# lez-s/Materialist

Measured on AMD Instinct MI355X. Metric: opt_iterations_per_sec_512x512, higher is better.
Workload: dtype f32; 1 GPU; BASELINE configs[1] synthetic: 1x512x512/GPU, --model_name pos_mlp --opt_order 'rm a' part rm, spp 64; mode=pos_mlp, height=512, width=512, spp=64, images_per_gpu=1, light=SH25, parallelism=dp1 (independent images, no data-path collective)

## Files before the change

include/matpbr.h:

```cpp
#ifndef MATPBR_H
#define MATPBR_H

#include <stddef.h>
#include <stdint.h>

#ifdef __cplusplus
extern "C" {
#endif

#define MATPBR_VERSION 311
#define MATPBR_MAX_SPP 128
#define MATPBR_NSH 25

enum {
    MATPBR_OK = 0,
    MATPBR_ERR_INVALID_ARG = -1,
    MATPBR_ERR_UNSUPPORTED = -2,
    MATPBR_ERR_LAUNCH = -3,
    MATPBR_ERR_WORKSPACE = -4,
};

enum { MATPBR_LIGHT_SH25 = 0, MATPBR_LIGHT_SH9 = 1, MATPBR_LIGHT_ENV_TEXELS = 2 };

#define MATPBR_FLAG_CLAMP_PARAMS 1u
// ... 13 lines not shown

typedef struct MatpbrCamera {
    float fov_x_deg;
} MatpbrCamera;

int matpbr_version(void);
const char* matpbr_strerror(int code);

int matpbr_shade_fwd(const float* a, const float* r, const float* m, const float* n, const float* light,
                     int light_kind, int n_light, float* out_rgb, int H, int W, int batch, int spp,
                     const MatpbrCamera* cam, uint32_t flags, void* stream);
size_t matpbr_plane9_bytes(int H, int W, int batch);
int matpbr_shade_fwd_ex(const float* a, const float* r, const float* m, const float* n, const float* light, int light_kind,
                        int n_light, const float* dcache, float* out_rgb, float* jac, int H, int W, int batch, int spp,
                        const MatpbrCamera* cam, uint32_t flags, void* stream);
int matpbr_diffuse_cache(const float* n, const float* light, int light_kind, int n_light, float* dcache, int H, int W, int batch,
                         int spp, const MatpbrCamera* cam, void* stream);
int matpbr_shade_fwd_keep(const float* a, const float* r, const float* m, const float* n, const float* light, int light_kind,
                          int n_light, const float* dcache, float* out_rgb, float* jac, float* s1, int H, int W, int batch, int spp,
                          const MatpbrCamera* cam, uint32_t flags, void* stream);
int matpbr_shade_fwd_cached(const float* a, const float* m, const float* jac, const float* s1, float* out_rgb, int H, int W, int batch,
                            uint32_t flags, void* stream);

size_t matpbr_lazy_state_bytes(int H, int W, int batch);
size_t matpbr_lazy_fold_bytes(int H, int W, int batch);
int matpbr_lazy_sums_count(int H, int W);
int matpbr_shade_fwd_lazy(const float* a, const float* r, const float* m, const float* n, const float* light, int light_kind, int n_light,
                          const float* dcache, void* lazy_state, float* out_rgb, void* jac16, const float* stats, float* sums, int H, int W,
                          int batch, int spp, const MatpbrCamera* cam, uint32_t flags, float floor, float tol, void* stream);
int matpbr_lazy_state_unpack(const void* lazy_state, float* state28, int* refreshed, int H, int W, int batch, void* stream);
int matpbr_jac16_unpack(const void* jac16, float* jac, int H, int W, int batch, void* stream);

int matpbr_shade_bwd(const float* a, const float* r, const float* m, const float* n, const float* light,
                     int light_kind, int n_light, const float* d_out_rgb, float* d_a, float* d_r, float* d_m,
                     float* d_n, float* d_light, void* workspace, size_t workspace_bytes, int H, int W, int batch,
                     int spp, const MatpbrCamera* cam, uint32_t flags, void* stream);
size_t matpbr_shade_bwd_workspace_bytes(int H, int W, int batch, int n_light);
int matpbr_shade_bwd_jac(const float* a, const float* r, const float* m, const float* jac, const float* d_out_rgb, float* d_a,
                         float* d_r, float* d_m, int H, int W, int batch, void* stream);

size_t matpbr_brdf_loss_workspace_bytes(int batch);
int matpbr_brdf_loss_stats(const float* pred, const float* gt, const float* gt_srgb, const float* pa, const float* pr,
                           const float* pm, const float* a0, const float* r0, const float* m0, float scale_delta,
                           float* stats, void* workspace, size_t workspace_bytes, int H, int W, int batch, uint32_t flags,
                           void* stream);
int matpbr_brdf_loss_stats_es(const float* pred, const float* gt, const float* gt_srgb, const float* pa, const float* pr, const float* pm,
                              const float* a0, const float* r0, const float* m0, float scale_delta, float* stats, void* workspace,
                              size_t workspace_bytes, int H, int W, int batch, uint32_t flags, int es_patience, float es_min_delta, float* history,
                              int hist_len, void* stream);
int matpbr_brdf_loss_bwd_jac(const float* pa, const float* pr, const float* pm, const float* jac, const float* pred,
                             const float* gt_srgb, const float* stats, const float* a0, const float* r0, const float* m0,
                             float scale_delta, float* d_a, float* d_r, float* d_m, float* best_a, float* best_r, float* best_m,
                             float* best_img, int H, int W, int batch, uint32_t flags, void* stream);
int matpbr_adam_step(float* p, const float* g, float* m, float* v, long n, float lr, float beta1, float beta2, float eps,
                     int step, void* stream);

typedef struct MatpbrBrdfPhase {
    float *pa, *pr, *pm;
    const float *n, *light;
    const float *gt_srgb;
    const float *a0, *r0, *m0;
    const float* dcache;
    float* pred;
    float* jac;
    float *d_a, *d_r, *d_m;
    float *adam_m[3], *adam_v[3];
    float *best_a, *best_r, *best_m, *best_img;
    float* stats;
    float* history;
    void* workspace;
    size_t workspace_bytes;
    int H, W, batch, spp;
    float fov_x_deg, scale_delta;
    uint32_t part_mask;
    int es_patience;
    float es_min_delta;
    int hist_len;
    float* s1cache;
    void* lazy_state;
    float lazy_tol;
    float* pred_next;
    uint32_t flags;
    void* lazy_fold;
} MatpbrBrdfPhase;
typedef struct MatpbrNormalStep {
    float *pa, *pr, *pm, *pn;
    float *ca, *cr, *cm, *cn;
    const float *d_a, *d_r, *d_m, *d_n;
    const float *a0, *r0, *m0, *n0;
    float *adam_m[4], *adam_v[4];
    float *best_a, *best_r, *best_m, *best_n, *best_img;
    const float *pred, *stats;
    float* ln_part;
    int H, W, batch;
    uint32_t part_mask;
    float scale_delta;
} MatpbrNormalStep;
int matpbr_brdf_loss_dpred(const float* pred, const float* gt_srgb, const float* stats, float* d_pred, int H, int W, int batch, void* stream);
int matpbr_brdf_normal_step(const MatpbrNormalStep* step, int t, float lr, void* stream);

size_t matpbr_brdf_phase_workspace_bytes(int H, int W, int batch);
int matpbr_brdf_phase_step(const MatpbrBrdfPhase* phase, int t, float lr, void* stream);
int matpbr_brdf_phase_resolve(const MatpbrBrdfPhase* phase, int t_done, void* stream);
#define MATPBR_STAGE_RENDER 1u
#define MATPBR_STAGE_STATS 2u
#define MATPBR_STAGE_BACKWARD 4u
// ... 53 lines not shown
```

include/matpbr_mlp.h:

```cpp
#ifndef MATPBR_MLP_H
#define MATPBR_MLP_H
#include <stddef.h>
#include <stdint.h>

#ifdef __cplusplus
extern "C" {
#endif

int matpbr_mlp_small_bwd_step(const float* g, int ldg, const float* w, int ldw, const float* c_prev, float* g_prev, int ldo, float* colsum_out,
                              int n_prev, const float* x, int ldx, float* d_w, int ldw_out, int K, const float* colsum_in, int colsum_stride,
                              int groups_in, float* d_bias, long M, int n_red, void* stream);

int matpbr_sin_bwd(const float* d_y, long ld_d, const float* pre, long ld_p, float* out, long M, int n, void* stream);
size_t matpbr_column_sum_workspace_bytes(int N);
int matpbr_column_sum(const float* x, float* out, long M, int N, void* workspace, size_t workspace_bytes, void* stream);

int matpbr_mlp_layer_fwd(const float* x, int ldx, const float* w, int ldw, const float* bias, float* s_out, float* c_out, int ldo, long M,
                         int N, int K, void* stream);
size_t matpbr_mlp_bwd_input_workspace_bytes(long M);
int matpbr_mlp_layer_bwd_input(const float* g, int ldg, const float* wt, int ldwt, const float* c_prev, float* g_prev, int ldo,
                               float* d_bias_prev, void* workspace, size_t workspace_bytes, long M, int n_prev, int n_red, void* stream);
size_t matpbr_mlp_bwd_weight_workspace_bytes(long M);
int matpbr_mlp_layer_bwd_weight(const float* g, int ldg, const float* x, int ldx, float* d_w, int ldw, void* workspace,
                                size_t workspace_bytes, long M, int N, int K, void* stream);
// ... 24 lines not shown
                                      int nprod, void* stream);
int matpbr_mlp_layer_bwd_weight_bx(const float* g, int ldg, const float* x, int ldx, float* d_w, int ldw, void* workspace,
                                   size_t workspace_bytes, long M, int N, int K, int nprod, void* stream);

#define MATPBR_WSPLIT_TRANSPOSED 1
#define MATPBR_WSPLIT_F16X2 2
int matpbr_mlp_split_weights_fmt(const float* w, int ldw, int N, int K, int flags, void* wsplit, void* stream);
size_t matpbr_mlp_chain_images_bytes(void);
int matpbr_mlp_chain_prep(const float* const* w, const int* ldw, const int* n, const float* const* bias, int d0, void* images, void* const* bwd_images,
                          void* zero, long zero_words, void* stream);
int matpbr_mlp_chain_fwd(const float* x0, int ldx0, const void* images, float* const* s_out, int ldo, const int* n, const float* start, int lds, float* th,
                         float* map_a, float* map_r, float* map_m, int n_head, long M, void* stream);
#define MATPBR_REDUCE_NONE (-1)
#define MATPBR_REDUCE_WGRAD 0
#define MATPBR_REDUCE_COLSUM 1
#define MATPBR_REDUCE_SKINNY 2
typedef struct MatpbrReduceJob {
    int kind, groups;
    const float *src, *src_b, *src_g;
    float *dst, *dst_b, *dst_g;
    int n0, n1, n2, n3;
    long ld_j, ld_c;
} MatpbrReduceJob;
int matpbr_mlp_reduce_jobs(const MatpbrReduceJob* jobs, int n_jobs, void* stream);
int matpbr_mlp_out_layer_bwd_tmax(const float* d_x, int ldd, const float* s_prev, const float* c_prev, int lds, const float* w_out, int ldw, float* g_prev,
                                  int ldg, void* g_tile_max, float* d_w, long ld_j, long ld_c, float* d_bias, float* d_bias_prev, void* workspace,
                                  size_t workspace_bytes, long M, int J, int n_prev, MatpbrReduceJob* defer, void* stream);
int matpbr_mlp_layer_bwd_input_blk(const float* g, int ldg, const void* g_tile_max, const void* wtsplit, const float* s_prev, float* g_prev, int ldo,
                                   void* out_tile_max, float* d_bias_prev, void* workspace, size_t workspace_bytes, long M, int n_prev, int n_red,
                                   MatpbrReduceJob* defer, void* stream);
int matpbr_mlp_first_layer_bwd_blk(const float* g, int ldg, const void* g_tile_max, const void* wtsplit, const float* s_prev, int lds, const float* x0,
                                   int ldx0, float* d_w0, long ld_j, long ld_c, int d0, float* d_bias0, void* workspace, size_t workspace_bytes,
                                   void* workspace2, size_t workspace2_bytes, long M, int n0, int n_red, MatpbrReduceJob* defer2, void* stream);
int matpbr_mlp_layer_bwd_weight_blk(const float* g, int ldg, const void* g_tile_max, const float* x, int ldx, float* d_w, int ldw, void* workspace,
                                    size_t workspace_bytes, long M, int N, int K, MatpbrReduceJob* defer, void* stream);
int matpbr_mlp_set_wgrad_kernel(int kernel);
int matpbr_mlp_split_weights_multi(const float* const* w, const int* ldw, const int* N, const int* K, const int* transposed,
                                   void* const* wsplit, int n_jobs, void* stream);
int matpbr_mlp_skinny_fwd(const float* x, int ldx, const float* w, int ldw, const float* bias, float* out, int ldo, long M, int J, int K,
                          void* stream);
int matpbr_mlp_arm_head_fwd(const float* x, int ldx, const float* w, int ldw, const float* bias, const float* start, int lds, float* th,
                            float* map_a, float* map_r, float* map_m, long M, int K, void* stream);
int matpbr_mlp_arm_head_bwd(const float* g_a, const float* g_r, const float* g_m, const float* th, float* d_x, long M, void* stream);
size_t matpbr_mlp_skinny_workspace_bytes(int J);
int matpbr_mlp_out_layer_bwd(const float* d_x, int ldd, const float* s_prev, const float* c_prev, int lds, const float* w_out, int ldw, float* g_prev,
                             int ldg, float* d_w, long ld_j, long ld_c, float* d_bias, float* d_bias_prev, void* workspace, size_t workspace_bytes,
                             long M, int J, int n_prev, void* stream);
int matpbr_mlp_skinny_bwd_weight(const float* s, int lds, const float* b, int ldb, float* d_w, long ld_j, long ld_c, float* d_bias,
                                 void* workspace, size_t workspace_bytes, long M, int J, int C, void* stream);
int matpbr_adamw_step_dev(float* p, const float* g, float* m, float* v, long n, float* hyper, float beta1, float beta2, float eps,
                          float weight_decay, void* stream);
int matpbr_adamw_step_snapshot_dev(float* p, const float* g, float* m, float* v, long n, float* hyper, float beta1, float beta2,
                                   float eps, float weight_decay, float* best, const float* stats, void* stream);

#ifdef __cplusplus
}
#endif
#endif
```

materialist_amd/_lib.py:

```python
from __future__ import annotations

import ctypes
import os
import threading

from . import build as _build

_c_f = ctypes.c_void_p


class MatpbrCamera(ctypes.Structure):
    _fields_ = [("fov_x_deg", ctypes.c_float)]


class MatpbrBrdfPhase(ctypes.Structure):
    _fields_ = ([(k, ctypes.c_void_p) for k in ("pa", "pr", "pm", "n", "light", "gt_srgb", "a0", "r0", "m0", "dcache", "pred", "jac", "d_a",
                                                "d_r", "d_m")] +
                [("adam_m", ctypes.c_void_p * 3), ("adam_v", ctypes.c_void_p * 3)] +
                [(k, ctypes.c_void_p) for k in ("best_a", "best_r", "best_m", "best_img", "stats", "history", "workspace")] +
                [("workspace_bytes", ctypes.c_size_t), ("H", ctypes.c_int), ("W", ctypes.c_int), ("batch", ctypes.c_int), ("spp", ctypes.c_int),
                 ("fov_x_deg", ctypes.c_float), ("scale_delta", ctypes.c_float), ("part_mask", ctypes.c_uint32), ("es_patience", ctypes.c_int),
                 ("es_min_delta", ctypes.c_float), ("hist_len", ctypes.c_int), ("s1cache", ctypes.c_void_p), ("lazy_state", ctypes.c_void_p),
                 ("lazy_tol", ctypes.c_float), ("pred_next", ctypes.c_void_p), ("flags", ctypes.c_uint32), ("lazy_fold", ctypes.c_void_p)])

# ... 6 lines not shown


class MatpbrError(RuntimeError):
    pass


class ReduceJob(ctypes.Structure):
    _fields_ = [("kind", ctypes.c_int), ("groups", ctypes.c_int), ("src", ctypes.c_void_p), ("src_b", ctypes.c_void_p), ("src_g", ctypes.c_void_p),
                ("dst", ctypes.c_void_p), ("dst_b", ctypes.c_void_p), ("dst_g", ctypes.c_void_p), ("n0", ctypes.c_int), ("n1", ctypes.c_int),
                ("n2", ctypes.c_int), ("n3", ctypes.c_int), ("ld_j", ctypes.c_long), ("ld_c", ctypes.c_long)]


SIGNATURES = {
    "matpbr_version": (ctypes.c_int, []),
    "matpbr_strerror": (ctypes.c_char_p, [ctypes.c_int]),
    "matpbr_shade_fwd": (ctypes.c_int, [_c_f] * 5 + [ctypes.c_int, ctypes.c_int, _c_f, ctypes.c_int, ctypes.c_int, ctypes.c_int,
                                       ctypes.c_int, ctypes.POINTER(MatpbrCamera), ctypes.c_uint32, ctypes.c_void_p]),
    "matpbr_shade_bwd": (ctypes.c_int, [_c_f] * 5 + [ctypes.c_int, ctypes.c_int] + [_c_f] * 6 + [ctypes.c_void_p, ctypes.c_size_t,
                                       ctypes.c_int, ctypes.c_int, ctypes.c_int, ctypes.c_int, ctypes.POINTER(MatpbrCamera),
                                       ctypes.c_uint32, ctypes.c_void_p]),
    "matpbr_shade_bwd_workspace_bytes": (ctypes.c_size_t, [ctypes.c_int] * 4),
    "matpbr_plane9_bytes": (ctypes.c_size_t, [ctypes.c_int] * 3),
    "matpbr_shade_fwd_ex": (ctypes.c_int, [_c_f] * 5 + [ctypes.c_int, ctypes.c_int, _c_f, _c_f, _c_f, ctypes.c_int, ctypes.c_int, ctypes.c_int,
                                          ctypes.c_int, ctypes.POINTER(MatpbrCamera), ctypes.c_uint32, ctypes.c_void_p]),
    "matpbr_shade_fwd_keep": (ctypes.c_int, [_c_f] * 5 + [ctypes.c_int, ctypes.c_int, _c_f, _c_f, _c_f, _c_f, ctypes.c_int, ctypes.c_int, ctypes.c_int,
                                            ctypes.c_int, ctypes.POINTER(MatpbrCamera), ctypes.c_uint32, ctypes.c_void_p]),
    "matpbr_shade_fwd_cached": (ctypes.c_int, [_c_f] * 5 + [ctypes.c_int, ctypes.c_int, ctypes.c_int, ctypes.c_uint32, ctypes.c_void_p]),
    "matpbr_diffuse_cache": (ctypes.c_int, [_c_f, _c_f, ctypes.c_int, ctypes.c_int, _c_f, ctypes.c_int, ctypes.c_int, ctypes.c_int, ctypes.c_int,
                                           ctypes.POINTER(MatpbrCamera), ctypes.c_void_p]),
    "matpbr_lazy_state_bytes": (ctypes.c_size_t, [ctypes.c_int] * 3),
    "matpbr_lazy_fold_bytes": (ctypes.c_size_t, [ctypes.c_int] * 3),
    "matpbr_env_texel_phase_step": (ctypes.c_int, [_c_f] * 6 + [ctypes.c_int, ctypes.c_int, ctypes.c_float, ctypes.c_void_p, ctypes.c_size_t, ctypes.c_int,
                                                   ctypes.c_int, _c_f, ctypes.c_int] + [_c_f] * 8 + [ctypes.c_float] * 3 + [ctypes.c_int, ctypes.c_int,
                                                                                                                          ctypes.c_void_p]),
    "matpbr_brdf_loss_dpred": (ctypes.c_int, [_c_f] * 4 + [ctypes.c_int, ctypes.c_int, ctypes.c_int, ctypes.c_void_p]),
    "matpbr_brdf_normal_step": (ctypes.c_int, [ctypes.POINTER(MatpbrNormalStep), ctypes.c_int, ctypes.c_float, ctypes.c_void_p]),
    "matpbr_env_mlp_phase_step": (ctypes.c_int, [_c_f] * 7 + [ctypes.c_int, ctypes.c_int, ctypes.c_float, ctypes.c_void_p, ctypes.c_size_t, ctypes.c_int,
                                                 ctypes.c_int, _c_f, ctypes.c_int] + [_c_f] * 4 + [ctypes.c_int, ctypes.c_int, ctypes.c_void_p]),
    "matpbr_brdf_phase_stages_timed": (ctypes.c_int, [ctypes.POINTER(MatpbrBrdfPhase), ctypes.c_int, ctypes.c_float, ctypes.c_uint32, ctypes.c_void_p,
                                                      ctypes.c_void_p, ctypes.c_void_p]),
    "matpbr_lazy_sums_count": (ctypes.c_int, [ctypes.c_int] * 2),
    "matpbr_shade_fwd_lazy": (ctypes.c_int, [_c_f] * 5 + [ctypes.c_int, ctypes.c_int] + [_c_f] * 6 + [ctypes.c_int, ctypes.c_int, ctypes.c_int, ctypes.c_int,
                                            ctypes.POINTER(MatpbrCamera), ctypes.c_uint32, ctypes.c_float, ctypes.c_float, ctypes.c_void_p]),
    "matpbr_lazy_state_unpack": (ctypes.c_int, [_c_f, _c_f, _c_f, ctypes.c_int, ctypes.c_int, ctypes.c_int, ctypes.c_void_p]),
    "matpbr_jac16_unpack": (ctypes.c_int, [_c_f, _c_f, ctypes.c_int, ctypes.c_int, ctypes.c_int, ctypes.c_void_p]),
    "matpbr_shade_bwd_jac": (ctypes.c_int, [_c_f] * 8 + [ctypes.c_int, ctypes.c_int, ctypes.c_int, ctypes.c_void_p]),
    "matpbr_brdf_loss_workspace_bytes": (ctypes.c_size_t, [ctypes.c_int]),
    "matpbr_brdf_loss_stats": (ctypes.c_int, [_c_f] * 9 + [ctypes.c_float, _c_f, ctypes.c_void_p, ctypes.c_size_t, ctypes.c_int, ctypes.c_int,
                                             ctypes.c_int, ctypes.c_uint32, ctypes.c_void_p]),
    "matpbr_brdf_loss_stats_es": (ctypes.c_int, [_c_f] * 9 + [ctypes.c_float, _c_f, ctypes.c_void_p, ctypes.c_size_t, ctypes.c_int, ctypes.c_int,
                                                ctypes.c_int, ctypes.c_uint32, ctypes.c_int, ctypes.c_float, _c_f, ctypes.c_int, ctypes.c_void_p]),
    "matpbr_brdf_loss_bwd_jac": (ctypes.c_int, [_c_f] * 10 + [ctypes.c_float] + [_c_f] * 7 + [ctypes.c_int, ctypes.c_int, ctypes.c_int,
                                                                                              ctypes.c_uint32, ctypes.c_void_p]),
    "matpbr_brdf_phase_workspace_bytes": (ctypes.c_size_t, [ctypes.c_int] * 3),
    "matpbr_brdf_phase_step": (ctypes.c_int, [ctypes.POINTER(MatpbrBrdfPhase), ctypes.c_int, ctypes.c_float, ctypes.c_void_p]),
    "matpbr_brdf_phase_stages": (ctypes.c_int, [ctypes.POINTER(MatpbrBrdfPhase), ctypes.c_int, ctypes.c_float, ctypes.c_uint32, ctypes.c_void_p]),
    "matpbr_brdf_phase_resolve": (ctypes.c_int, [ctypes.POINTER(MatpbrBrdfPhase), ctypes.c_int, ctypes.c_void_p]),
    "matpbr_env_phase_workspace_bytes": (ctypes.c_size_t, [ctypes.c_int] * 3),
    "matpbr_env_phase_step": (ctypes.c_int, [_c_f] * 7 + [ctypes.c_int, ctypes.c_int, ctypes.c_float, ctypes.c_void_p, ctypes.c_size_t,
                                            ctypes.c_int, ctypes.c_int, ctypes.c_int, ctypes.c_void_p]),
    "matpbr_env_project": (ctypes.c_int, [_c_f, ctypes.c_int, _c_f, _c_f, _c_f, ctypes.c_int, ctypes.c_void_p]),
    "matpbr_env_project_bwd": (ctypes.c_int, [_c_f, ctypes.c_int, _c_f, _c_f, _c_f, ctypes.c_int, ctypes.c_int, ctypes.c_void_p]),
    "matpbr_select_improved": (ctypes.c_int, [_c_f, _c_f, _c_f, ctypes.c_int, ctypes.c_long, ctypes.c_void_p]),
    "matpbr_mlp_wsplit_bytes": (ctypes.c_size_t, [ctypes.c_int]),
    "matpbr_mlp_split_weights": (ctypes.c_int, [_c_f, ctypes.c_int, ctypes.c_int, ctypes.c_int, _c_f, ctypes.c_void_p]),
    "matpbr_mlp_layer_fwd_bx": (ctypes.c_int, [_c_f, ctypes.c_int, _c_f, _c_f, _c_f, _c_f, ctypes.c_int, ctypes.c_long, ctypes.c_int, ctypes.c_int,
                                              ctypes.c_int, ctypes.c_void_p]),
    "matpbr_mlp_layer_bwd_input_bx": (ctypes.c_int, [_c_f, ctypes.c_int, _c_f, _c_f, _c_f, ctypes.c_int, _c_f, ctypes.c_void_p, ctypes.c_size_t,
                                                    ctypes.c_long, ctypes.c_int, ctypes.c_int, ctypes.c_int, ctypes.c_void_p]),
    "matpbr_sin_bwd": (ctypes.c_int, [_c_f, ctypes.c_long, _c_f, ctypes.c_long, _c_f, ctypes.c_long, ctypes.c_int, ctypes.c_void_p]),
    "matpbr_mlp_layer_fwd": (ctypes.c_int, [_c_f, ctypes.c_int, _c_f, ctypes.c_int, _c_f, _c_f, _c_f, ctypes.c_int, ctypes.c_long, ctypes.c_int,
                                           ctypes.c_int, ctypes.c_void_p]),
    "matpbr_mlp_bwd_input_workspace_bytes": (ctypes.c_size_t, [ctypes.c_long]),
    "matpbr_mlp_layer_bwd_input": (ctypes.c_int, [_c_f, ctypes.c_int, _c_f, ctypes.c_int, _c_f, _c_f, ctypes.c_int, _c_f, ctypes.c_void_p,
                                                 ctypes.c_size_t, ctypes.c_long, ctypes.c_int, ctypes.c_int, ctypes.c_void_p]),
    "matpbr_mlp_bwd_weight_workspace_bytes": (ctypes.c_size_t, [ctypes.c_long]),
    "matpbr_mlp_layer_bwd_weight": (ctypes.c_int, [_c_f, ctypes.c_int, _c_f, ctypes.c_int, _c_f, ctypes.c_int, ctypes.c_void_p, ctypes.c_size_t,
                                                  ctypes.c_long, ctypes.c_int, ctypes.c_int, ctypes.c_void_p]),
    "matpbr_mlp_layer_fwd_sgn": (ctypes.c_int, [_c_f, ctypes.c_int, _c_f, ctypes.c_int, _c_f, _c_f, ctypes.c_int, _c_f, ctypes.c_int, ctypes.c_long,
                                               ctypes.c_int, ctypes.c_int, ctypes.c_void_p]),
    "matpbr_mlp_layer_bwd_input_sgn": (ctypes.c_int, [_c_f, ctypes.c_int, _c_f, ctypes.c_int, _c_f, _c_f, ctypes.c_int, _c_f, ctypes.c_void_p,
                                                     ctypes.c_size_t, ctypes.c_long, ctypes.c_int, ctypes.c_int, ctypes.c_void_p]),
    "matpbr_mlp_layer_bwd_input_bx_sgn": (ctypes.c_int, [_c_f, ctypes.c_int, _c_f, _c_f, _c_f, ctypes.c_int, _c_f, ctypes.c_void_p, ctypes.c_size_t,
                                                        ctypes.c_long, ctypes.c_int, ctypes.c_int, ctypes.c_int, ctypes.c_void_p]),
    "matpbr_mlp_layer_bwd_weight_bx": (ctypes.c_int, [_c_f, ctypes.c_int, _c_f, ctypes.c_int, _c_f, ctypes.c_int, ctypes.c_void_p, ctypes.c_size_t,
                                                     ctypes.c_long, ctypes.c_int, ctypes.c_int, ctypes.c_int, ctypes.c_void_p]),
    "matpbr_mlp_out_layer_bwd_tmax": (ctypes.c_int, [_c_f, ctypes.c_int, _c_f, _c_f, ctypes.c_int, _c_f, ctypes.c_int, _c_f, ctypes.c_int, ctypes.c_void_p, _c_f,
                                                     ctypes.c_long, ctypes.c_long, _c_f, _c_f, ctypes.c_void_p, ctypes.c_size_t, ctypes.c_long, ctypes.c_int,
                                                     ctypes.c_int, ctypes.c_void_p, ctypes.c_void_p]),
    "matpbr_mlp_reduce_jobs": (ctypes.c_int, [ctypes.c_void_p, ctypes.c_int, ctypes.c_void_p]),
    "matpbr_mlp_layer_bwd_input_blk": (ctypes.c_int, [_c_f, ctypes.c_int, ctypes.c_void_p, ctypes.c_void_p, _c_f, _c_f, ctypes.c_int, ctypes.c_void_p, _c_f,
                                                      ctypes.c_void_p, ctypes.c_size_t, ctypes.c_long, ctypes.c_int, ctypes.c_int, ctypes.c_void_p, ctypes.c_void_p]),
    "matpbr_mlp_first_layer_bwd_blk": (ctypes.c_int, [_c_f, ctypes.c_int, ctypes.c_void_p, ctypes.c_void_p, _c_f, ctypes.c_int, _c_f, ctypes.c_int, _c_f,
                                                      ctypes.c_long, ctypes.c_long, ctypes.c_int, _c_f, ctypes.c_void_p, ctypes.c_size_t, ctypes.c_void_p,
                                                      ctypes.c_size_t, ctypes.c_long, ctypes.c_int, ctypes.c_int, ctypes.c_void_p, ctypes.c_void_p]),
    "matpbr_mlp_layer_bwd_weight_blk": (ctypes.c_int, [_c_f, ctypes.c_int, ctypes.c_void_p, _c_f, ctypes.c_int, _c_f, ctypes.c_int, ctypes.c_void_p,
                                                       ctypes.c_size_t, ctypes.c_long, ctypes.c_int, ctypes.c_int, ctypes.c_void_p, ctypes.c_void_p]),
    "matpbr_mlp_set_wgrad_kernel": (ctypes.c_int, [ctypes.c_int]),
    "matpbr_mlp_chain_images_bytes": (ctypes.c_size_t, []),
    "matpbr_mlp_chain_prep": (ctypes.c_int, [ctypes.c_void_p, ctypes.c_void_p, ctypes.c_void_p, ctypes.c_void_p, ctypes.c_int, ctypes.c_void_p, ctypes.c_void_p,
                                             ctypes.c_void_p, ctypes.c_long, ctypes.c_void_p]),
    "matpbr_mlp_chain_fwd": (ctypes.c_int, [_c_f, ctypes.c_int, ctypes.c_void_p, ctypes.c_void_p, ctypes.c_int, ctypes.c_void_p, _c_f, ctypes.c_int, _c_f, _c_f, _c_f,
                                            _c_f, ctypes.c_int, ctypes.c_long, ctypes.c_void_p]),
    "matpbr_mlp_split_weights_fmt": (ctypes.c_int, [_c_f, ctypes.c_int, ctypes.c_int, ctypes.c_int, ctypes.c_int, ctypes.c_void_p, ctypes.c_void_p]),
    "matpbr_mlp_skinny_fwd": (ctypes.c_int, [_c_f, ctypes.c_int, _c_f, ctypes.c_int, _c_f, _c_f, ctypes.c_int, ctypes.c_long, ctypes.c_int, ctypes.c_int,
                                            ctypes.c_void_p]),
    "matpbr_mlp_arm_head_fwd": (ctypes.c_int, [_c_f, ctypes.c_int, _c_f, ctypes.c_int, _c_f, _c_f, ctypes.c_int, _c_f, _c_f, _c_f, _c_f, ctypes.c_long,
                                              ctypes.c_int, ctypes.c_void_p]),
    "matpbr_mlp_arm_head_bwd": (ctypes.c_int, [_c_f, _c_f, _c_f, _c_f, _c_f, ctypes.c_long, ctypes.c_void_p]),
    "matpbr_mlp_skinny_workspace_bytes": (ctypes.c_size_t, [ctypes.c_int]),
    "matpbr_mlp_set_lds_dma": (ctypes.c_int, [ctypes.c_int]),
    "matpbr_mlp_skinny_bwd_weight": (ctypes.c_int, [_c_f, ctypes.c_int, _c_f, ctypes.c_int, _c_f, ctypes.c_long, ctypes.c_long, _c_f, ctypes.c_void_p,
                                                   ctypes.c_size_t, ctypes.c_long, ctypes.c_int, ctypes.c_int, ctypes.c_void_p]),
    "matpbr_adamw_step_dev": (ctypes.c_int, [_c_f] * 4 + [ctypes.c_long, _c_f, ctypes.c_float, ctypes.c_float, ctypes.c_float, ctypes.c_float,
                                                         ctypes.c_void_p]),
    "matpbr_light_to_sh25": (ctypes.c_int, [_c_f, ctypes.c_int, ctypes.c_int, _c_f, ctypes.c_int, ctypes.c_void_p]),
    "matpbr_light_to_sh25_bwd": (ctypes.c_int, [_c_f, ctypes.c_int, ctypes.c_int, _c_f, ctypes.c_int, ctypes.c_void_p]),
    "matpbr_mlp_split_weights_multi": (ctypes.c_int, [ctypes.c_void_p] * 6 + [ctypes.c_int, ctypes.c_void_p]),
    "matpbr_adamw_step_snapshot_dev": (ctypes.c_int, [_c_f] * 4 + [ctypes.c_long, _c_f, ctypes.c_float, ctypes.c_float, ctypes.c_float, ctypes.c_float,
                                                                  _c_f, _c_f, ctypes.c_void_p]),
    "matpbr_mlp_layer_fwd_tail": (ctypes.c_int, [_c_f, ctypes.c_int, _c_f, ctypes.c_int, _c_f, _c_f, _c_f, ctypes.c_int, _c_f, ctypes.c_int, ctypes.c_long,
                                                ctypes.c_int, ctypes.c_int, ctypes.c_void_p]),
    "matpbr_mlp_layer_fwd_bx_tail": (ctypes.c_int, [_c_f, ctypes.c_int, _c_f, _c_f, _c_f, _c_f, ctypes.c_int, _c_f, ctypes.c_int, ctypes.c_long,
                                                   ctypes.c_int, ctypes.c_int, ctypes.c_int, ctypes.c_void_p]),
    "matpbr_sample_brdf_dr": (ctypes.c_int, [_c_f] * 10 + [ctypes.c_long, ctypes.c_void_p]),
    "matpbr_mlp_layer_fwd_bx_head": (ctypes.c_int, [_c_f, ctypes.c_int, _c_f, _c_f, _c_f, _c_f, ctypes.c_int, _c_f, ctypes.c_int, _c_f, _c_f, ctypes.c_int,
                                                   _c_f, _c_f, _c_f, _c_f, ctypes.c_long, ctypes.c_int, ctypes.c_int, ctypes.c_void_p]),
    "matpbr_column_sum_workspace_bytes": (ctypes.c_size_t, [ctypes.c_int]),
    "matpbr_column_sum": (ctypes.c_int, [_c_f, _c_f, ctypes.c_long, ctypes.c_int, ctypes.c_void_p, ctypes.c_size_t, ctypes.c_void_p]),
    "matpbr_shade_transfer": (ctypes.c_int, [_c_f] * 5 + [ctypes.c_int, ctypes.c_int, ctypes.c_int, ctypes.c_int, ctypes.POINTER(MatpbrCamera),
                                            ctypes.c_uint32, ctypes.c_void_p]),
    "matpbr_transfer_bytes": (ctypes.c_size_t, [ctypes.c_int] * 3),
    "matpbr_relight": (ctypes.c_int, [_c_f] * 3 + [ctypes.c_int, ctypes.c_int, ctypes.c_int, ctypes.c_void_p]),
    "matpbr_adam_step": (ctypes.c_int, [_c_f] * 4 + [ctypes.c_long, ctypes.c_float, ctypes.c_float, ctypes.c_float, ctypes.c_float, ctypes.c_int,
                                       ctypes.c_void_p]),
    "matpbr_eval_brdf": (ctypes.c_int, [_c_f] * 8 + [ctypes.c_long, ctypes.c_void_p]),
    "matpbr_eval_brdf_bwd": (ctypes.c_int, [_c_f] * 11 + [ctypes.c_long, ctypes.c_void_p]),
    "matpbr_brdf_terms": (ctypes.c_int, [_c_f] * 5 + [ctypes.c_long, ctypes.c_void_p]),
    "matpbr_sample_brdf": (ctypes.c_int, [_c_f] * 10 + [ctypes.c_long, ctypes.c_void_p]),
    "matpbr_sh_eval": (ctypes.c_int, [_c_f] * 3 + [ctypes.c_long, ctypes.c_void_p]),
    "matpbr_depth_to_mesh_host": (ctypes.c_int, [ctypes.c_void_p, ctypes.c_int, ctypes.c_int, ctypes.c_float, ctypes.c_float] + [ctypes.c_void_p] * 6),
    "matpbr_mlp_small_bwd_step": (ctypes.c_int, [_c_f, ctypes.c_int, _c_f, ctypes.c_int, _c_f, _c_f, ctypes.c_int, _c_f, ctypes.c_int, _c_f, ctypes.c_int,
                                                 _c_f, ctypes.c_int, ctypes.c_int, _c_f, ctypes.c_int, ctypes.c_int, _c_f, ctypes.c_long, ctypes.c_int,
# ... 54 lines not shown
```

materialist_amd/armhead.py:

```python
from __future__ import annotations

import types
from typing import Dict, Optional

import torch

from . import _lib, ops
from . import loss as _loss
from . import render as _render
from .posmlp import _PosMlpHipFn

_al4 = lambda n: (n + 3) // 4 * 4


def flat_state(net: torch.nn.Module, dev) -> dict:
    L = net.n_layers
    lins = [(getattr(net, f"lin{l}").linear if l < L - 1 else getattr(net, f"lin{l}")) for l in range(L)]
    st = getattr(net, "_flat_state", None)
    if (st is not None and "spans" in st and st["flat"].device == torch.device(dev)
            and all(lin.weight.data_ptr() == wp.data_ptr() and lin.bias.data_ptr() == bp.data_ptr() for lin, (wp, bp) in zip(lins, st["views"]))):
        return st
    total = sum(lin.weight.shape[0] * _al4(lin.weight.shape[1]) + _al4(lin.weight.shape[0]) for lin in lins)
    flat = torch.zeros(total, dtype=torch.float32, device=dev)
    off, views, spans = 0, [], {}
    for l, lin in enumerate(lins):
        n, k = lin.weight.shape
        wp = flat[off:off + n * _al4(k)].view(n, _al4(k))
        wp[:, :k].copy_(lin.weight.detach())
        lin.weight.data = wp[:, :k]
        off += n * _al4(k)
        bp = flat[off:off + n]
        bp.copy_(lin.bias.detach())
        lin.bias.data = bp
        off += _al4(n)
        views.append((wp, bp))
    names = {id(p): name for name, p in net.named_parameters()}
    for lin, (wp, bp) in zip(lins, views):
        spans[names[id(lin.weight)]] = (wp, lin.weight.shape[1])
        spans[names[id(lin.bias)]] = (bp, None)
    st = net._flat_state = {"flat": flat, "views": views, "spans": spans}
    return st


class ArmMlpPhase:

    PACKED = True
    FUSED_OUT_BWD = True
    FUSED_FIRST_BWD = True
    BWD_F16 = True
    FWD_CHAIN = True
    DEFER_REDUCE = True
    FWD_PRODUCTS = 3

    @staticmethod
    def why_not(scene: _render.Scene, gt_image: torch.Tensor, net: torch.nn.Module, optimize_part: str, mask) -> Optional[str]:
        if gt_image.ndim != 3:
            return "a batch of images (the network optimises one image per process, as the reference does)"
        if not gt_image.is_cuda:
            return "the image is not on a GPU"
        if not scene.use_mesh_normal or "n" in optimize_part:
            return "predicted normals / a part that moves the normal map (the eight-output 'armn' network and the render under a normal map: loop.PosMlpNormalPhase with armhead.MlpEngine)"
        if getattr(net, "output_type", None) != "arm" or not _PosMlpHipFn.PRODUCTS:
            return "not the five-output 'arm' network on the split-operand kernels"
        M = gt_image.shape[0] * gt_image.shape[1]
        if M % 128 or M < _PosMlpHipFn.MIN_ROWS:
            return f"{M} pixels: the layer kernels take whole 128-row tiles of at least {_PosMlpHipFn.MIN_ROWS} rows"
        L = net.n_layers
        d0 = getattr(net, "lin0").linear.weight.shape[1]
        for l in range(L - 1):
            n = getattr(net, f"lin{l}").linear.weight.shape[0]
            if (n + d0 if (l + 1) in net.skip else n) != 256:
                return "hidden layers that are not 256 wide"
        if getattr(net, f"lin{L - 1}").weight.shape != (5, 256) or d0 > 16:
            return "an output layer that is not 256 -> 5, or more than 16 inputs"
        return None

    @staticmethod
    def supported(scene: _render.Scene, gt_image: torch.Tensor, net: torch.nn.Module, optimize_part: str, mask) -> bool:
        return ArmMlpPhase.why_not(scene, gt_image, net, optimize_part, mask) is None

    def __init__(self, scene: _render.Scene, gt_image: torch.Tensor, net: torch.nn.Module, start_arm: torch.Tensor, fixed: Dict[str, torch.Tensor],
                 optimize_part: str = "arm", spp: int = 64, lr: float = 3e-4, scale_delta: float = 0.1, patience: int = 0,
                 min_delta: float = 0.0, best_mse: Optional[torch.Tensor] = None, history_len: int = 5000, weight_decay: float = 0.01,
                 mask: Optional[torch.Tensor] = None):
        from .loop import _lib_ws

        if not ArmMlpPhase.supported(scene, gt_image, net, optimize_part, None):
            raise NotImplementedError("ArmMlpPhase: 'arm' network with 256-wide layers on one image of at least 8192 pixels (a multiple of 128)")
        self.ops, self.scene, self.net, self.part = ops, scene, net, optimize_part
        self.spp, self.scale_delta = int(spp), float(scale_delta)
        self.gt = gt_image.contiguous()
        dev = self.dev = self.gt.device
        H, W = self.H, self.W = self.gt.shape[0], self.gt.shape[1]
        M = self.M = H * W
        self.gt_srgb = _loss.linear_to_srgb(self.gt).contiguous()
        self.start_arm = start_arm.detach().to(dev, torch.float32).contiguous()
        self.fixed = {k: v.detach().contiguous() for k, v in fixed.items()}
        self.orig = {"albedo": self.start_arm[:, 0:3].reshape(H, W, 3).contiguous(),
                     "roughness": self.start_arm[:, 3:4].reshape(H, W, 1).contiguous(),
                     "metallic": self.start_arm[:, 4:5].reshape(H, W, 1).contiguous()}
        self.products = int(_PosMlpHipFn.PRODUCTS)
        self.fwd_products = int(self.FWD_PRODUCTS) or self.products
        self.bwd_f16 = bool(self.BWD_F16 and self.PACKED and self.FUSED_OUT_BWD and self.FUSED_FIRST_BWD)
        st = flat_state(net, dev)
# ... 82 lines not shown
        self.dcache = ops.diffuse_cache(self._n, self._light, self.spp, scene.fov)
        self.jac = ops.plane9(self.gt)
        self.s1 = None if "roughness" in self.live else torch.empty((3, 1, H, W), dtype=torch.float32, device=dev)
        self._bg_mask = scene.bg_mask
        if self._bg_mask is not None:
            self._bg_rgb = (scene.bg_basis @ self._light.reshape(25, 3)).contiguous()
            self._bg_idx = ops.background_index(self._bg_mask)
            self._bg_rows = self._bg_rgb.reshape(-1, 3)[self._bg_idx].contiguous()
            self._bg_rows_t = self._bg_rows.t().contiguous()
        self._mask_u8 = None if mask is None else mask.to(dev).reshape(H, W).to(torch.uint8).contiguous()
        self._fed = {k: E(H, W, 1) for k in ("roughness", "metallic")} if mask is not None else None
        self.t = 0

    def set_lr(self, lr: float) -> None:
        self._lr = float(lr)
        self.hyper[0:1].fill_(self._lr)
        self.opt.param_groups[0]["lr"] = self._lr

    def forward(self) -> Dict[str, torch.Tensor]:
        o, P = ops, self.fwd_products
        if self._split_args[-1] > 0:
            with torch.cuda.device(self.dev):
                _lib.check(_lib.load().matpbr_mlp_split_weights_multi(*self._split_args, o._stream(self.flat)), "matpbr_mlp_split_weights_multi")
        if self.chain:
            live = self.live
            lib, st = _lib.load(), o._stream(self.flat)
            mp = [o._ptr(self.maps[k]) if k in live else None for k in ("albedo", "roughness", "metallic")]
            with torch.cuda.device(self.dev):
                _lib.check(lib.matpbr_mlp_chain_prep(*self._chain_prep, st), "matpbr_mlp_chain_prep")
                _lib.check(lib.matpbr_mlp_chain_fwd(o._ptr(self.x0p), self.x0p.stride(0), o._ptr(self._chain_images), self._chain_out, 256, self._chain_n,
                                                    o._ptr(self.start_arm), self.start_arm.stride(0), o._ptr(self.th), *mp, self.views[-1][0].shape[0], self.M, st),
                           "matpbr_mlp_chain_fwd")
            return {k: (self.maps[k] if k in live else self.fixed[k]) for k in self.maps}
        wp, bp = self.views[0]
        tail = lambda l: self.x0p if self.ns[l] != 256 else None
        if self.packed:
            o.mlp_layer_fwd(self.x0p, wp, bp, self.bufs[0], None, self.d0, packed=True)
        else:
            o.mlp_layer_fwd(self.x0p, wp, bp, self.bufs[0], self.cbufs[0], self.d0)
        live = self.live
        maps = [self.maps[k] if k in live else None for k in ("albedo", "roughness", "metallic")]
        wo, bo = self.views[-1]
        for l in range(1, self.L - 1):
            wp, bp = self.views[l]
            if l == self.L - 2 and self.ns[l] == 256:
                o.mlp_layer_fwd_bx_head(self.bufs[l - 1], self.wsplit_f[l], bp, self.bufs[l], self.cbufs[l], 256, P, wo, bo, self.start_arm, self.th,
                                        *maps)
            else:
                o.mlp_layer_fwd_bx(self.bufs[l - 1], self.wsplit_f[l], bp, self.bufs[l], self.cbufs[l], self.ns[l], 256, P, tail=tail(l))
        if self.ns[-1] != 256:
            o.mlp_arm_head_fwd(self.bufs[-1], wo, bo, self.start_arm, self.th, *maps, 256)
        return {k: (self.maps[k] if k in live else self.fixed[k]) for k in self.maps}

    def backward(self) -> None:
        o, P, live = ops, self.products, self.live
        o.mlp_arm_head_bwd(self.g["albedo"] if "albedo" in live else None, self.g["roughness"] if "roughness" in live else None,
                           self.g["metallic"] if "metallic" in live else None, self.th, self.d_x)
        wp, _ = self.views[-1]
        gw, gb = self.gviews[-1]
        g_prev = self.gbufs[0]
        _, gb_prev = self.gviews[self.L - 2]
        f16 = self.bwd_f16
        import ctypes as _ct

        jobs, nj = (self._jobs, 0) if (f16 and self.DEFER_REDUCE) else (None, 0)
        slot = (lambda k: (_ct.cast(_ct.byref(jobs, k * _ct.sizeof(_lib.ReduceJob)), _ct.c_void_p), f"_d{k}")) if jobs is not None else (lambda k: None)
        if f16:
            if not self.prep_all:
                self.tmax.zero_()
            o.mlp_out_layer_bwd_tmax(self.d_x, self.bufs[-1], wp, g_prev, self.tmax[self.L - 2], gw, gb, gb_prev, 5, self.ns[-1], defer=slot(nj))
            nj += 1
        elif self.FUSED_OUT_BWD:
            o.mlp_out_layer_bwd(self.d_x, self.bufs[-1], None if self.packed else self.cbufs[-1], wp, g_prev, gw, gb, gb_prev, 5, self.ns[-1])
        else:
            o.mlp_skinny_bwd_weight(self.d_x, self.bufs[-1], gw, 5, 256, d_bias=gb)
            self.w_out_t[:, :5].copy_(wp.t())
            o.mlp_layer_bwd_input(self.d_x, self.w_out_t, self.bufs[-1] if self.packed else self.cbufs[-1], g_prev, self.ns[-1], 5, gb_prev,
                                  packed=self.packed)
        g, n_red = g_prev, self.ns[-1]
        for l in range(self.L - 2, 0, -1):
            wp, _ = self.views[l]
            gw, _ = self.gviews[l]
            if f16:
                o.mlp_layer_bwd_weight_blk(g, self.tmax[l], self.bufs[l - 1], n_red, 256, out=gw, defer=slot(nj))
                nj += 1
            else:
                o.mlp_layer_bwd_weight_bx(g, self.bufs[l - 1], n_red, 256, P, out=gw)
            n_prev = self.ns[l - 1]
            _, gb = self.gviews[l - 1]
            c_prev = self.bufs[l - 1] if self.packed else self.cbufs[l - 1]
            if f16:
                if l == 1:
                    o.mlp_first_layer_bwd_blk(g, self.tmax[l], self.wsplit_b[l], c_prev, self.x0p, self.gviews[0][0], self.d0, n_prev, n_red, gb, defer=slot(nj))
                    nj += 2
                    if jobs is not None:
                        o.mlp_reduce_jobs(jobs, nj, self.flat)
                    return
                g_prev = self.gbufs[0] if g is self.gbufs[1] else self.gbufs[1]
                o.mlp_layer_bwd_input_blk(g, self.tmax[l], self.wsplit_b[l], c_prev, g_prev, n_prev, n_red, gb, self.tmax[l - 1], defer=slot(nj))
                nj += 1
                g, n_red = g_prev, n_prev
                continue
            if l == 1 and self.FUSED_FIRST_BWD:
                o.mlp_first_layer_bwd_bx(g, self.wsplit_b[l], c_prev, self.x0p, self.gviews[0][0], self.d0, n_prev, n_red, gb, P, packed=self.packed)
                return
            g_prev = self.gbufs[0] if g is self.gbufs[1] else self.gbufs[1]
            o.mlp_layer_bwd_input_bx(g, self.wsplit_b[l], c_prev, g_prev, n_prev, n_red, gb, P, packed=self.packed)
            g, n_red = g_prev, n_prev
        gw, _ = self.gviews[0]
        o.mlp_skinny_bwd_weight(self.x0p, g, gw, self.d0, n_red, transposed_out=True)

    def step(self) -> None:
        o, sc = ops, self.scene
        d = self.forward()
        if self._mask_u8 is not None:
            d = dict(d)
            for k in ("roughness", "metallic"):
                lo, hi = (0.0, 1.0) if k in self.live else (-3.0e38, 3.0e38)
                d[k] = o.masked_mean_fill(d[k], self._mask_u8, out=self._fed[k], lo=lo, hi=hi)
        if self.s1 is not None and self.t > 0:
            o.shade_fwd_cached(d["albedo"], d["metallic"], self.jac, self.s1, clamp_params=True, out=self.pred)
        else:
            o.shade_fwd(d["albedo"], d["roughness"], d["metallic"], self._n, self._light, self.spp, sc.fov, clamp_params=True, out=self.pred,
                        dcache=self.dcache, jac=self.jac, s1=self.s1)
        if self._bg_mask is not None and not (self.s1 is not None and self.t > 0):
            self.pred.view(-1, 3).index_copy_(0, self._bg_idx, self._bg_rows)
            o.background_into_jac(self.jac, self.s1, self._bg_mask, self._bg_rgb, self._bg_idx, self._bg_rows_t)
        o.brdf_loss_stats(self.pred, self.gt, self.gt_srgb, d["albedo"], d["roughness"], d["metallic"], self.orig["albedo"],
                          self.orig["roughness"], self.orig["metallic"], self.scale_delta, self.stats, self.ws, optimize_part=self.part,
                          es_patience=self.patience, es_min_delta=self.min_delta, history=self.hist)
        o.brdf_loss_bwd_jac(d["albedo"], d["roughness"], d["metallic"], self.jac, self.pred, self.gt_srgb, self.stats,
                            self.orig["albedo"], self.orig["roughness"], self.orig["metallic"], self.scale_delta,
                            self.g["albedo"], self.g["roughness"], self.g["metallic"], self.best["albedo"], self.best["roughness"],
                            self.best["metallic"], self.best_img, optimize_part=self.part)
        if self._mask_u8 is not None:
            for k in ("roughness", "metallic"):
                if k in self.live:
                    o.masked_mean_fill(self.g[k], self._mask_u8, out=self.g[k], gate=self.maps[k])
        self.backward()
        lib = _lib.load()
        with torch.cuda.device(self.dev):
            _lib.check(lib.matpbr_adamw_step_snapshot_dev(o._ptr(self.flat), o._ptr(self.gflat), o._ptr(self.adam_m), o._ptr(self.adam_v),
                                                          self.flat.numel(), o._ptr(self.hyper), 0.9, 0.999, 1e-8, self.weight_decay,
                                                          o._ptr(self._best_flat), o._ptr(self.stats), o._stream(self.flat)),
                       "matpbr_adamw_step_snapshot_dev")
        if self._lr > 1.5e-4:
            self._sched_epoch += 1
            if self._sched_epoch % 100 == 0:
                self.set_lr(self._lr * 0.8)
        self.t += 1

    @property
    def best_weights(self) -> Dict[str, torch.Tensor]:
        out, off = {}, 0
        order = []
        for wp, bp in self.views:
            order += [(off, wp), (off + wp.numel(), bp)]
            off += wp.numel() + _al4(bp.numel())
        by_ptr = {t.data_ptr(): o_ for o_, t in order}
        for name, (view, k) in self._spans.items():
            o_ = by_ptr[view.data_ptr()]
            best = self._best_flat[o_:o_ + view.numel()].view_as(view)
            out[name] = (best[:, :k] if k is not None else best).clone()
        return out

    def current_maps(self) -> Dict[str, torch.Tensor]:
        d = self.forward()
        if self._mask_u8 is not None:
            d = dict(d)
            for k in ("roughness", "metallic"):
                lo, hi = (0.0, 1.0) if k in self.live else (-3.0e38, 3.0e38)
                d[k] = self.ops.masked_mean_fill(d[k], self._mask_u8, lo=lo, hi=hi)
        return {"albedo": d["albedo"].clamp(0, 1), "roughness": d["roughness"].clamp(0.07, 1), "metallic": d["metallic"].clamp(0, 1)}

    def step_and_check(self) -> bool:
        self.step()
        if self.patience <= 0 or self.t % self.sync_every:
            return False
        return bool(self.stats[0, ops.STAT_STOPPED] > 0.5)

    @property
    def iterations_run(self) -> int:
        return int(self.stats[0, ops.STAT_ITERS])

    def lr_at(self, t0: int) -> float:
        lr, k = self.base_lr, 0
        while lr > 1.5e-4 and (k + 1) * 100 <= t0:
            lr *= 0.8
            k += 1
        return lr

    def history(self) -> torch.Tensor:
        return self.hist[: self.t]


class MlpEngine:

    @staticmethod
# ... 137 lines not shown
```

materialist_amd/build.py:

```python
from __future__ import annotations

import os
import shutil
import subprocess

_HERE = os.path.dirname(os.path.abspath(__file__))
CSRC = os.path.join(_HERE, "csrc")
LIB_PATH = os.path.join(_HERE, "libmatpbr.so")
SOURCES = ["matpbr_kernels.hip", "posmlp_kernels.hip", "posmlp_chain.hip", "mesh_host.cpp"]
HEADERS = [os.path.join("..", "..", "include", "matpbr_experimental.h"), "posmlp_device.hpp", "matpbr_device.hpp", "matpbr_shade.hpp", "matpbr_lazy.hpp", "matpbr_pstep.hpp", os.path.join("..", "..", "include", "matpbr.h"), os.path.join("..", "..", "include", "matpbr_mlp.h")]
HIPCC_FLAGS = ["-O3", "--offload-arch=gfx950", "-std=c++17", "-shared", "-fPIC", "-fno-gpu-rdc", "-Wall", "-Wno-unused-function"]


def _hipcc() -> str:
    for cand in (os.environ.get("HIPCC"), shutil.which("hipcc"), "/opt/rocm/bin/hipcc"):
        if cand and os.path.exists(cand):
            return cand
    raise RuntimeError("hipcc not found: libmatpbr.so can only be built with the ROCm toolchain")


def sources_digest() -> str:
    import hashlib

    h = hashlib.sha256()
    for name in sorted(SOURCES + HEADERS):
        with open(os.path.normpath(os.path.join(CSRC, name)), "rb") as f:
            h.update(f.read())
    return h.hexdigest()[:16]


def is_stale() -> bool:
    if not os.path.exists(LIB_PATH):
        return True
    t = os.path.getmtime(LIB_PATH)
    deps = [os.path.join(CSRC, s) for s in SOURCES] + [os.path.normpath(os.path.join(CSRC, h)) for h in HEADERS]
    return any(os.path.getmtime(d) > t for d in deps)


EXTRA_FLAGS = {"posmlp_chain.hip": ["-fno-slp-vectorize"]}
OBJ_DIR = os.path.join(_HERE, "_build")


def build_library(force: bool = False, verbose: bool = False) -> str:
    if not force and not is_stale():
        return LIB_PATH
    os.makedirs(OBJ_DIR, exist_ok=True)
    hdr_t = max(os.path.getmtime(os.path.normpath(os.path.join(CSRC, h))) for h in HEADERS)
    flags = [f for f in HIPCC_FLAGS if f != "-shared"]
    objs, procs = [], []
    for src in SOURCES:
        sp = os.path.join(CSRC, src)
        obj = os.path.join(OBJ_DIR, os.path.splitext(src)[0] + ".o")
        objs.append(obj)
        if force or not os.path.exists(obj) or os.path.getmtime(obj) < max(os.path.getmtime(sp), hdr_t, os.path.getmtime(__file__)):
            cmd = [_hipcc(), *flags, *EXTRA_FLAGS.get(src, []), "-c", sp, "-o", obj]
            procs.append((cmd, subprocess.Popen(cmd, stdout=subprocess.PIPE, stderr=subprocess.PIPE, text=True)))
    for cmd, pr in procs:
        out, err = pr.communicate()
        if pr.returncode != 0:
            raise RuntimeError("hipcc failed:\n" + " ".join(cmd) + "\n" + out + err)
        if verbose:
            print(err)
    cmd = [_hipcc(), "--offload-arch=gfx950", "-shared", "-fPIC", "-fno-gpu-rdc", "-o", LIB_PATH, *objs]
# ... 37 lines not shown
```

materialist_amd/csrc/matpbr_kernels.hip:

```cpp
#include <hip/hip_runtime.h>
#include <hip/hip_ext.h>
#include <cstdlib>

#include <algorithm>
#include <cmath>
#include <cstdint>
#include <cstring>

#include "../../include/matpbr.h"
#include "../../include/matpbr_experimental.h"
#include "matpbr_device.hpp"
#include "matpbr_shade.hpp"
#include "matpbr_lazy.hpp"
#include "matpbr_pstep.hpp"

using namespace matpbr;

namespace {

constexpr int kRedBlocks = 768;

__global__ __launch_bounds__(kBlock) void loss_sums1_kernel(const float* __restrict__ pred, const float* __restrict__ gt,
                                                            float* __restrict__ part, long n3) {
    __shared__ float s_buf[4];
    const int b = blockIdx.y;
    const float* p = pred + b * n3;
    const float* q = gt + b * n3;
    float sp = 0.0f, sg = 0.0f;
    for (long i = (long)blockIdx.x * kBlock + threadIdx.x; i < n3; i += (long)gridDim.x * kBlock) { sp += p[i]; sg += q[i]; }
    sp = block_sum(sp, s_buf);
    sg = block_sum(sg, s_buf);
    if (threadIdx.x == 0) { part[((long)b * gridDim.x + blockIdx.x) * 2] = sp; part[((long)b * gridDim.x + blockIdx.x) * 2 + 1] = sg; }
}
__global__ __launch_bounds__(kBlock) void loss_final1_kernel(const float* __restrict__ part, float* __restrict__ stats, int nblk) {
    __shared__ float s_buf[4];
    const int b = blockIdx.x;
    float sp = 0.0f, sg = 0.0f;
    for (int i = threadIdx.x; i < nblk; i += kBlock) { sp += part[((long)b * nblk + i) * 2]; sg += part[((long)b * nblk + i) * 2 + 1]; }
    sp = block_sum(sp, s_buf);
    sg = block_sum(sg, s_buf);
    if (threadIdx.x == 0) stats[b * kStatsStride + 0] = sg / sp;
}
__global__ __launch_bounds__(kBlock) void step_state_init_kernel(const float* __restrict__ stats, float* __restrict__ state, int batch) {
    for (int i = threadIdx.x; i < batch * kStateStride; i += kBlock) {
        const int b = i / kStateStride, k = i - b * kStateStride;
        state[i] = k < kStatsStride ? stats[b * kStatsStride + k] : (k == kStBestRatio ? -1.0f : 0.0f);
    }
}
struct ResolveArgs {
    float *x0[3], *x1[3];
    float *p0, *p1, *best_img;
    const float* state;
    long n1;
};
__global__ __launch_bounds__(kBlock) void phase_resolve_kernel(const ResolveArgs q) {
    const int b = blockIdx.y;
    const long i = (long)blockIdx.x * kBlock + threadIdx.x;
    if (i >= q.n1) return;
    const bool swap = q.state[b * kStateStride + kStSel] > 0.5f;
    const float bratio = q.state[b * kStateStride + kStBestRatio];
    const long o1 = b * q.n1 + i, o3 = o1 * 3;
    if (swap || bratio >= 0.0f) {
#pragma unroll
        for (int z = 0; z < 3; ++z) {
            if (q.x0[z] == nullptr) continue;
            const int w = z == 0 ? 3 : 1;
            const float lo = z == 1 ? 0.07f : 0.0f;
            for (int c = 0; c < w; ++c) {
                const long o = (z == 0 ? o3 : o1) + c;
                float u = q.x0[z][o], v = q.x1[z][o];
                if (swap) { const float t = u; u = v; v = t; q.x0[z][o] = u; }
                q.x1[z][o] = bratio >= 0.0f ? fminf(fmaxf(v, lo), 1.0f) : v;
            }
        }
    }
    if (q.p0 == nullptr) return;
#pragma unroll
    for (int c = 0; c < 3; ++c) {
        float u = q.p0[o3 + c], v = q.p1[o3 + c];
        if (swap) { const float t = u; u = v; v = t; q.p0[o3 + c] = u; q.p1[o3 + c] = v; }
        if (bratio >= 0.0f && q.best_img) q.best_img[o3 + c] = pow_inv_gamma(fmaxf(v * bratio, kLossEps));
    }
}
__global__ __launch_bounds__(kBlock) void phase_resolve_done_kernel(float* __restrict__ state2, int batch) {
    for (int i = threadIdx.x; i < 2 * batch; i += kBlock) state2[(long)i * kStateStride + kStSel] = 0.0f;
}

template <int MODE>
__global__ __launch_bounds__(kBlock) void loss_sums2_kernel(const float* __restrict__ pred, const float* __restrict__ gt_srgb,
                                                            const float* __restrict__ stats, const float* __restrict__ pa,
                                                            const float* __restrict__ a0, const float* __restrict__ pr,
                                                            const float* __restrict__ r0, const float* __restrict__ pm,
                                                            const float* __restrict__ m0, float* __restrict__ part, long n3, long n1,
                                                            const float* __restrict__ fwd_sums, int n_fwd, unsigned part_mask,
                                                            const float* __restrict__ reg_sums = nullptr, const float* __restrict__ pred_alt = nullptr,
                                                            const float* __restrict__ state = nullptr, int n_reg = 0,
                                                            const long long* __restrict__ walk_fix = nullptr) {
    __shared__ float s_buf[4];
    const int b = blockIdx.y;
    float ratio = 1.0f;
    const bool vec4 = MODE == 4 && (n3 & 3) == 0 && ((reinterpret_cast<uintptr_t>(pred) | reinterpret_cast<uintptr_t>(pred_alt) | reinterpret_cast<uintptr_t>(gt_srgb)) & 15) == 0;
    const long stride4 = (long)gridDim.x * kBlock, first4 = (long)blockIdx.x * kBlock + threadIdx.x;
    float4 pre_p[2], pre_g[2];
    if (vec4) {
#pragma unroll
        for (int u = 0; u < 2; ++u) {
            const long i = first4 + u * stride4;
            pre_g[u] = reinterpret_cast<const float4*>(gt_srgb + b * n3)[i < (n3 >> 2) ? i : 0];
        }
    }
    if (MODE >= 1 && img_stopped(stats, b)) return;
    if (MODE >= 3 && state != nullptr && state[b * kStateStride + kStSel] > 0.5f) pred = pred_alt;
    if (vec4) {
#pragma unroll
        for (int u = 0; u < 2; ++u) {
            const long i = first4 + u * stride4;
            pre_p[u] = reinterpret_cast<const float4*>(pred + b * n3)[i < (n3 >> 2) ? i : 0];
        }
    }
    float sp_total = 0.0f;
    if (MODE == 1 || MODE >= 3) {
        float sp = 0.0f;
        for (int i = threadIdx.x; i < n_fwd; i += kBlock)
            sp += fwd_sums[(long)b * n_fwd + i] + (MODE == 4 && walk_fix ? (float)((double)walk_fix[(long)b * n_fwd + i] * (1.0 / kWalkFix)) : 0.0f);
        sp_total = block_sum(sp, s_buf);
        ratio = stats[b * kStatsStride + kStGtSum] / sp_total;
    } else if (MODE == 0) {
        ratio = stats[b * kStatsStride + kStRatio];
    }
    float s[5] = {0.0f, 0.0f, 0.0f, 0.0f, 0.0f};
    if (vec4) {
        const float4* p4 = reinterpret_cast<const float4*>(pred + b * n3);
        const float4* g4 = reinterpret_cast<const float4*>(gt_srgb + b * n3);
        auto word = [&](const float4 pv, const float4 gv) {
            const float px[4] = {pv.x, pv.y, pv.z, pv.w}, gx[4] = {gv.x, gv.y, gv.z, gv.w};
#pragma unroll
            for (int e = 0; e < 4; ++e) {
                const float d = pow_inv_gamma(fmaxf(px[e] * ratio, kLossEps)) - gx[e];
                s[0] = fmaf(d, d, s[0]);
                s[1] += fabsf(d);
            }
        };
#pragma unroll
        for (int u = 0; u < 2; ++u)
            if (first4 + u * stride4 < (n3 >> 2)) word(pre_p[u], pre_g[u]);
        for (long i = first4 + 2 * stride4; i < (n3 >> 2); i += stride4) word(p4[i], g4[i]);
    } else
    for (long i = (long)blockIdx.x * kBlock + threadIdx.x; i < n3; i += (long)gridDim.x * kBlock) {
        float xs = pow_inv_gamma(fmaxf(pred[b * n3 + i] * ratio, kLossEps));
        float d = xs - gt_srgb[b * n3 + i];
        s[0] = fmaf(d, d, s[0]);
        s[1] += fabsf(d);
        if (MODE != 4 && (part_mask & MATPBR_PART_A)) s[2] += fabsf(fminf(fmaxf(pa[b * n3 + i], 0.0f), 1.0f) - a0[b * n3 + i]);
    }
    if (MODE != 4 && (part_mask & (MATPBR_PART_R | MATPBR_PART_M)))
        for (long i = (long)blockIdx.x * kBlock + threadIdx.x; i < n1; i += (long)gridDim.x * kBlock) {
            if (part_mask & MATPBR_PART_R) s[3] += fabsf(fminf(fmaxf(pr[b * n1 + i], 0.07f), 1.0f) - r0[b * n1 + i]);
            if (part_mask & MATPBR_PART_M) s[4] += fabsf(fminf(fmaxf(pm[b * n1 + i], 0.0f), 1.0f) - m0[b * n1 + i]);
        }
    float* rows = part + (long)b * (MODE >= 3 ? step_part_stride((int)gridDim.x) : (long)gridDim.x * 5);
#pragma unroll
    for (int k = 0; k < 5; ++k) {
        if (MODE == 4 && k >= 2) {
            if (threadIdx.x == 0) rows[(long)blockIdx.x * 5 + k] = 0.0f;
            continue;
        }
        float v = block_sum(s[k], s_buf);
        if (threadIdx.x == 0) rows[(long)blockIdx.x * 5 + k] = v;
    }
    if (MODE >= 3 && blockIdx.x == 0 && threadIdx.x == 0) rows[(long)gridDim.x * 5] = sp_total;
    if (MODE == 4 && blockIdx.x == 0) {
        float rg[3] = {0.0f, 0.0f, 0.0f};
        for (int i = threadIdx.x; i < n_reg; i += kBlock) {
#pragma unroll
            for (int k = 0; k < 3; ++k) rg[k] += reg_sums[((long)b * n_reg + i) * 3 + k];
        }
#pragma unroll
        for (int k = 0; k < 3; ++k) {
            const float v = block_sum(rg[k], s_buf);
            if (threadIdx.x == 0) rows[(long)gridDim.x * 5 + 1 + k] = v;
        }
// ... 278 lines not shown
    float acc[kNSH][3];
#pragma unroll
    for (int k = 0; k < kNSH; ++k) acc[k][0] = acc[k][1] = acc[k][2] = 0.0f;
    for (int t = threadIdx.x; t < n_light; t += 64) {
        float Yw[kNSH];
        texel_basis(t, He, Yw);
        const float e0 = src[t * 3], e1 = src[t * 3 + 1], e2 = src[t * 3 + 2];
#pragma unroll
        for (int k = 0; k < kNSH; ++k) {
            acc[k][0] = fmaf(Yw[k], e0, acc[k][0]);
            acc[k][1] = fmaf(Yw[k], e1, acc[k][1]);
            acc[k][2] = fmaf(Yw[k], e2, acc[k][2]);
        }
    }
#pragma unroll
    for (int k = 0; k < kNSH; ++k)
#pragma unroll
        for (int c = 0; c < 3; ++c) {
            const float v = wave_sum_to_lane63(acc[k][c]);
            if (threadIdx.x == 63) dst[k * 3 + c] = v;
        }
}
__global__ __launch_bounds__(kBlock) void light_to_sh25_bwd_kernel(const float* __restrict__ d_sh25, int kind, int n_light, float* __restrict__ d_light,
                                                                   int batch) {
    const long i = (long)blockIdx.x * kBlock + threadIdx.x;
    if (i >= (long)batch * n_light) return;
    const int b = (int)(i / n_light), t = (int)(i % n_light);
    const float* g = d_sh25 + (long)b * kNL;
    float* dst = d_light + i * 3;
    if (kind == MATPBR_LIGHT_SH9) {
        dst[0] = g[t * 3]; dst[1] = g[t * 3 + 1]; dst[2] = g[t * 3 + 2];
        return;
    }
    const int He = (int)(sqrtf((float)(n_light / 2)) + 0.5f);
    float Yw[kNSH];
    texel_basis(t, He, Yw);
    float a0 = 0.0f, a1 = 0.0f, a2 = 0.0f;
#pragma unroll
    for (int k = 0; k < kNSH; ++k) {
        a0 = fmaf(Yw[k], g[k * 3], a0);
        a1 = fmaf(Yw[k], g[k * 3 + 1], a1);
        a2 = fmaf(Yw[k], g[k * 3 + 2], a2);
    }
    dst[0] = a0; dst[1] = a1; dst[2] = a2;
}
__global__ __launch_bounds__(kBlock) void select_copy_kernel(float* __restrict__ dst, const float* __restrict__ src, const float* __restrict__ stats,
                                                             int first, long n) {
    if (!(first || stats[kStImproved] > 0.5f)) return;
    for (long i = (long)blockIdx.x * kBlock + threadIdx.x; i < n; i += (long)gridDim.x * kBlock) dst[i] = src[i];
}
__global__ __launch_bounds__(kBlock) void adam_dev_kernel(float* __restrict__ p, const float* __restrict__ g, float* __restrict__ m,
                                                          float* __restrict__ v, long n, float* __restrict__ hyper, float b1, float b2,
                                                          float eps, float wd, float* __restrict__ best, const float* __restrict__ stats) {
    if (stats != nullptr && stats[kStStopped] > 1.5f) return;
    const bool snap = best != nullptr && stats[kStImproved] > 0.5f;
    const float t = stats != nullptr ? fmaxf(stats[kStIters], 1.0f) : hyper[1] + 1.0f, lr = hyper[0];
    if (stats != nullptr && blockIdx.x == 0 && threadIdx.x == 0) hyper[1] = t;
    const float keep = 1.0f - lr * wd;
    const float bc1 = 1.0f - powf(b1, t), bc2 = 1.0f - powf(b2, t);
    const float lr_over_bc1 = lr / bc1, inv_sqrt_bc2 = 1.0f / sqrtf(bc2);
    for (long i = (long)blockIdx.x * kBlock + threadIdx.x; i < n; i += (long)gridDim.x * kBlock) {
        float gi = g[i];
        float mi = fmaf(b1, m[i], (1.0f - b1) * gi);
        float vi = fmaf(b2, v[i], (1.0f - b2) * gi * gi);
        m[i] = mi; v[i] = vi;
        const float pi = p[i];
        if (snap) best[i] = pi;
        p[i] = pi * keep - lr_over_bc1 * mi / fmaf(fsqrt(vi), inv_sqrt_bc2, eps);
    }
}
__global__ void adam_dev_tick_kernel(float* __restrict__ hyper, const float* __restrict__ stats) {
    if (stats != nullptr && stats[kStStopped] > 1.5f) return;
    hyper[1] += 1.0f;
}

__global__ __launch_bounds__(kBlock) void colsum_pass1_kernel(const float* __restrict__ x, float* __restrict__ part, long M, int N,
                                                              long rows_per) {
    const long r0 = (long)blockIdx.x * rows_per, r1 = r0 + rows_per < M ? r0 + rows_per : M;
    for (int c = threadIdx.x; c < N; c += kBlock) {
        float a0 = 0.0f, a1 = 0.0f, a2 = 0.0f, a3 = 0.0f;
        long r = r0;
        for (; r + 3 < r1; r += 4) {
            a0 += x[r * N + c]; a1 += x[(r + 1) * N + c]; a2 += x[(r + 2) * N + c]; a3 += x[(r + 3) * N + c];
        }
        for (; r < r1; ++r) a0 += x[r * N + c];
        part[(long)blockIdx.x * N + c] = (a0 + a1) + (a2 + a3);
    }
}
__global__ __launch_bounds__(kBlock) void colsum_pass2_kernel(const float* __restrict__ part, float* __restrict__ out, int nblk, int N) {
    __shared__ float s_acc[8][33];
    const int cx = threadIdx.x & 31, cy = threadIdx.x >> 5;
    const int c = blockIdx.x * 32 + cx;
    float a = 0.0f;
    if (c < N)
        for (int b = cy; b < nblk; b += 8) a += part[(long)b * N + c];
    s_acc[cy][cx] = a;
    __syncthreads();
    if (cy == 0 && c < N) {
        float t = 0.0f;
#pragma unroll
        for (int k = 0; k < 8; ++k) t += s_acc[k][cx];
        out[c] = t;
    }
}

__global__ __launch_bounds__(kBlock) void colsum_small_kernel(const float* __restrict__ x, float* __restrict__ out, int M, int N) {
    const int slice = threadIdx.x & 63, cx = threadIdx.x >> 6;
    const int c = blockIdx.x * 4 + cx;
    float a = 0.0f;
    if (c < N)
        for (int r = slice; r < M; r += 64) a += x[(long)r * N + c];
    a = wave_sum_to_lane63(a);
    if (slice == 63 && c < N) out[c] = a;
}

__global__ __launch_bounds__(kBlock) void sin_bwd_kernel(const float* __restrict__ d_y, long ld_d, const float* __restrict__ pre, long ld_p,
                                                         float* __restrict__ out, long M, int n) {
    const long total = M * n;
    for (long i = (long)blockIdx.x * kBlock + threadIdx.x; i < total; i += (long)gridDim.x * kBlock) {
        const long r = i / n;
        const int c = (int)(i - r * n);
        out[i] = d_y[r * ld_d + c] * cosf(pre[r * ld_p + c]);
// ... 628 lines not shown
    else
        hipLaunchKernelGGL(lazy_refresh_kernel<8>, dim3((unsigned)lb.ngrp, (unsigned)batch), dim3(kBlock), 0, st, ra, light, g, tab);
    return launch_status();
}
static int lazy_forward(const float* a, const float* r, const float* m, const float* n, const float* light, const float* dcache, void* lazy_state,
                        float* out_rgb, void* jac16, const float* stats, float* sums, const Geom& g, const RuleTable& tab, int batch, int clamp,
                        int force, float floor_, float tol, hipStream_t st, int jac32 = 0) {
    const long P = (long)g.H * g.W;
    const LazyBuffers lb = lazy_buffers(lazy_state, P, batch);
    if (lb.nblk > kLazyMaxBlocks) return MATPBR_ERR_UNSUPPORTED;
    LazyFwdArgs fa{};
    fa.a = a; fa.r = r; fa.m = m; fa.state = lb.planes; fa.out = out_rgb; fa.jac16 = (uint32_t*)jac16; fa.stats = stats; fa.block_sums = sums;
    fa.counts = lb.counts; fa.lists = lb.lists; fa.clamp = clamp; fa.force = force; fa.n_sums = lb.nblk + lb.ngrp; fa.jac32 = jac32;
    hipLaunchKernelGGL(lazy_fwd_kernel, dim3((unsigned)lb.nblk, (unsigned)batch), dim3(kBlock), 0, st, fa, (int)P);
    return lazy_refresh(a, r, m, n, light, dcache, lazy_state, out_rgb, jac16, stats, sums, g, tab, batch, clamp, force, floor_, tol, st, jac32);
}

int matpbr_shade_fwd_lazy(const float* a, const float* r, const float* m, const float* n, const float* light, int light_kind, int n_light,
                          const float* dcache, void* lazy_state, float* out_rgb, void* jac16, const float* stats, float* sums, int H, int W,
                          int batch, int spp, const MatpbrCamera* cam, uint32_t flags, float floor_, float tol, void* stream) {
    if (!a || !r || !m || !n || !light || !dcache || !lazy_state || !out_rgb || !jac16 || batch <= 0) return MATPBR_ERR_INVALID_ARG;
    if (!sh25(light_kind, n_light)) return MATPBR_ERR_INVALID_ARG;
    if (!valid_spp(spp)) return MATPBR_ERR_UNSUPPORTED;
    if (!stats && !(floor_ > 0.0f)) return MATPBR_ERR_INVALID_ARG;
    Geom g;
    RuleTable tab;
    if (!make_geom(H, W, cam, g)) return MATPBR_ERR_INVALID_ARG;
    if (!fill_rule_table(spp, tab)) return MATPBR_ERR_UNSUPPORTED;
    return lazy_forward(a, r, m, n, light, dcache, lazy_state, out_rgb, jac16, stats, sums, g, tab, batch, (flags & MATPBR_FLAG_CLAMP_PARAMS) ? 1 : 0,
                        (flags & MATPBR_FLAG_LAZY_FORCE) ? 1 : 0, floor_, tol, (hipStream_t)stream, (flags & MATPBR_FLAG_JAC32) ? 1 : 0);
}

int matpbr_lazy_state_unpack(const void* lazy_state, float* state28, int* refreshed, int H, int W, int batch, void* stream) {
    if (!lazy_state || (!state28 && !refreshed) || H <= 0 || W <= 0 || batch <= 0) return MATPBR_ERR_INVALID_ARG;
    const long P = (long)H * W, BP = P * batch;
    const uint32_t* counts = (const uint32_t*)((const char*)lazy_state + lazy_planes_bytes(P, batch));
    const uint16_t* lists = (const uint16_t*)((const char*)counts + lazy_counts_bytes(P, batch));
    if (state28)
        hipLaunchKernelGGL(lazy_unpack_kernel, dim3((unsigned)((BP + kBlock - 1) / kBlock)), dim3(kBlock), 0, (hipStream_t)stream,
                           (const uint32_t*)lazy_state, state28, BP);
    if (refreshed)
        hipLaunchKernelGGL(lazy_refreshed_kernel, dim3((unsigned)lazy_fwd_blocks(P), (unsigned)batch), dim3(kBlock), 0, (hipStream_t)stream, counts, lists,
                           refreshed, (int)P, lazy_fwd_blocks(P));
    return launch_status();
}

int matpbr_jac16_unpack(const void* jac16, float* jac, int H, int W, int batch, void* stream) {
    if (!jac16 || !jac || H <= 0 || W <= 0 || batch <= 0) return MATPBR_ERR_INVALID_ARG;
    const long BP = (long)H * W * batch;
    hipLaunchKernelGGL(jac16_unpack_kernel, dim3((unsigned)((BP + kBlock - 1) / kBlock)), dim3(kBlock), 0, (hipStream_t)stream, (const uint32_t*)jac16, jac, BP);
    return launch_status();
}

size_t matpbr_brdf_loss_workspace_bytes(int batch) { return batch > 0 ? (size_t)batch * kRedBlocks * 5 * sizeof(float) : 0; }

static unsigned part_mask_of(uint32_t flags) {
    const unsigned all = MATPBR_PART_A | MATPBR_PART_R | MATPBR_PART_M;
    if (flags & MATPBR_PART_N) return flags & all;
    return (flags & all) ? (flags & all) : all;
}

int matpbr_brdf_loss_stats_es(const float* pred, const float* gt, const float* gt_srgb, const float* pa, const float* pr, const float* pm,
                              const float* a0, const float* r0, const float* m0, float scale_delta, float* stats, void* workspace,
                              size_t workspace_bytes, int H, int W, int batch, uint32_t flags, int es_patience, float es_min_delta, float* history,
                              int hist_len, void* stream) {
    if (!pred || !gt || !gt_srgb || !pa || !pr || !pm || !a0 || !r0 || !m0 || !stats || H <= 0 || W <= 0 || batch <= 0)
        return MATPBR_ERR_INVALID_ARG;
    if (!workspace || workspace_bytes < matpbr_brdf_loss_workspace_bytes(batch)) return MATPBR_ERR_WORKSPACE;
    const long n1 = (long)H * W, n3 = n1 * 3;
    float* part = (float*)workspace;
    hipStream_t st = (hipStream_t)stream;
    dim3 grid(kRedBlocks, (unsigned)batch);
    hipLaunchKernelGGL(loss_sums1_kernel, grid, dim3(kBlock), 0, st, pred, gt, part, n3);
    hipLaunchKernelGGL(loss_final1_kernel, dim3((unsigned)batch), dim3(kBlock), 0, st, part, stats, kRedBlocks);
    hipLaunchKernelGGL(loss_sums2_kernel<0>, grid, dim3(kBlock), 0, st, pred, gt_srgb, stats, pa, a0, pr, r0, pm, m0, part, n3, n1,
                       (const float*)nullptr, 0, part_mask_of(flags));
    hipLaunchKernelGGL(loss_final2_kernel<2>, dim3((unsigned)batch), dim3(kBlock), 0, st, part, stats, kRedBlocks, 1.0f / (float)n3,
                       1.0f / (float)n1, scale_delta, part_mask_of(flags), es_patience, es_min_delta,
                       (const float*)nullptr, 0, history, hist_len, batch);
    return launch_status();
}

int matpbr_brdf_loss_stats(const float* pred, const float* gt, const float* gt_srgb, const float* pa, const float* pr, const float* pm,
                           const float* a0, const float* r0, const float* m0, float scale_delta, float* stats, void* workspace,
                           size_t workspace_bytes, int H, int W, int batch, uint32_t flags, void* stream) {
    return matpbr_brdf_loss_stats_es(pred, gt, gt_srgb, pa, pr, pm, a0, r0, m0, scale_delta, stats, workspace, workspace_bytes, H, W, batch, flags, -1,
                                     0.0f, nullptr, 0, stream);
}


int matpbr_brdf_loss_bwd_jac(const float* pa, const float* pr, const float* pm, const float* jac, const float* pred, const float* gt_srgb,
                             const float* stats, const float* a0, const float* r0, const float* m0, float scale_delta, float* d_a,
                             float* d_r, float* d_m, float* best_a, float* best_r, float* best_m, float* best_img, int H, int W, int batch,
                             uint32_t flags, void* stream) {
    if (!pa || !pr || !pm || !jac || !pred || !gt_srgb || !stats || !a0 || !r0 || !m0 || !d_a || !d_r || !d_m || H <= 0 || W <= 0 ||
        batch <= 0)
        return MATPBR_ERR_INVALID_ARG;
    JacBwdArgs q{};
    q.a = pa; q.r = pr; q.m = pm; q.jac = jac; q.d_a = d_a; q.d_r = d_r; q.d_m = d_m;
    q.pred = pred; q.gt_srgb = gt_srgb; q.stats = stats; q.a0 = a0; q.r0 = r0; q.m0 = m0;
    q.best_a = best_a; q.best_r = best_r; q.best_m = best_m; q.best_img = best_img;
    q.scale_delta = scale_delta;
    q.inv_n3 = 1.0f / (3.0f * (float)H * (float)W);
    q.inv_n1 = 1.0f / ((float)H * (float)W);
    q.part_mask = part_mask_of(flags);
    const long P = (long)H * W;
    if (flags & MATPBR_FLAG_JAC16)
        hipLaunchKernelGGL((jac_bwd_kernel<true, true>), dim3((unsigned)((P + kBlock - 1) / kBlock), (unsigned)batch), dim3(kBlock), 0, (hipStream_t)stream, q, P);
    else
        hipLaunchKernelGGL((jac_bwd_kernel<true, false>), dim3((unsigned)((P + kBlock - 1) / kBlock), (unsigned)batch), dim3(kBlock), 0, (hipStream_t)stream, q, P);
    return launch_status();
}

namespace {
__global__ __launch_bounds__(kBlock) void loss_dpred_kernel(const float* __restrict__ pred, const float* __restrict__ gt_srgb,
                                                            const float* __restrict__ stats, float* __restrict__ d_pred, long P, float inv_n3) {
    const int b = blockIdx.y;
    if (img_stopped_before(stats, b)) return;
    const long p = (long)blockIdx.x * kBlock + threadIdx.x;
    if (p >= P) return;
    const long i = (long)b * P + p;
    const float ratio = stats[b * kStatsStride + kStRatio], sr = stats[b * kStatsStride + kStSr];
#pragma unroll
    for (int c = 0; c < 3; ++c) {
        const float x = pred[i * 3 + c] * ratio;
        const float xc = fmaxf(x, kLossEps);
        const float xs = pow_inv_gamma(xc);
        const float d = xs - gt_srgb[i * 3 + c];
        const float dxs = x > kLossEps ? xs * rcp(xc) * (1.0f / 2.2f) : 0.0f;
        d_pred[i * 3 + c] = ratio * dxs * fmaf(6.0f * sr, d, fsign(d)) * inv_n3;
    }
}
struct NormalStepArgs {
    MatpbrNormalStep s;
    float inv_n3, inv_n1, lr_over_bc1, b1, b2, eps, inv_sqrt_bc2;
};
__device__ __forceinline__ float adam_one(float p, float gi, float* m, float* v, long i, const NormalStepArgs& q) {
    const float mi = fmaf(q.b1, m[i], (1.0f - q.b1) * gi);
    const float vi = fmaf(q.b2, v[i], (1.0f - q.b2) * gi * gi);
    m[i] = mi; v[i] = vi;
    return p - q.lr_over_bc1 * mi / fmaf(fsqrt(vi), q.inv_sqrt_bc2, q.eps);
}
__global__ __launch_bounds__(kBlock) void normal_step_kernel(const NormalStepArgs q, long P) {
    __shared__ float s_buf[4];
    const MatpbrNormalStep& s = q.s;
    const int b = blockIdx.y;
    if (img_stopped_before(s.stats, b)) return;
    const long p = (long)blockIdx.x * kBlock + threadIdx.x;
    const bool live = p < P;
    const long i = (long)b * P + (live ? p : P - 1);
    const bool improved = s.stats[b * kStatsStride + kStImproved] > 0.5f;
    const float ratio = s.stats[b * kStatsStride + kStRatio];
    const unsigned part = s.part_mask;
    float ln = 0.0f;
    if (live) {
#pragma unroll
        for (int c = 0; c < 3; ++c) {
            const float ra = s.pa[i * 3 + c], a = fminf(fmaxf(ra, 0.0f), 1.0f);
            if (improved && s.best_a) s.best_a[i * 3 + c] = a;
            if (improved && s.best_img) s.best_img[i * 3 + c] = pow_inv_gamma(fmaxf(s.pred[i * 3 + c] * ratio, kLossEps));
            if ((part & MATPBR_PART_A) && s.d_a) {
                float g = s.d_a[i * 3 + c] + s.scale_delta * q.inv_n3 * fsign(a - s.a0[i * 3 + c]);
                g = (ra >= 0.0f && ra <= 1.0f) ? g : 0.0f;
                const float pn = adam_one(ra, g, s.adam_m[0], s.adam_v[0], i * 3 + c, q);
// ... 565 lines not shown
```

materialist_amd/csrc/matpbr_shade.hpp:

```cpp
#pragma once
#include <hip/hip_runtime.h>

#include <cmath>
#include <cstdint>
#include <cstring>

#include "matpbr_device.hpp"

namespace matpbr {

constexpr int kBlock = 256;
constexpr int kNL = kNSH * 3;

constexpr int kMaxRings = 8, kMaxAz = 8;
struct RuleTable {
    int nu_d, nphi_d, nu_s, nphi_s;
    float4 dring[kMaxRings];
    float4 dring2[kMaxRings];
    float2 daz[kMaxRings][kMaxAz];
    float4 sring[kMaxRings];
    float2 saz[kMaxRings][kMaxAz];
};

struct RuleRegs { float2 daz, saz; };
__device__ __forceinline__ void load_rule_regs(const RuleTable& tab, RuleRegs& rr) {
    static_assert(kMaxRings * kMaxAz == 64, "one table entry per lane of a wave64");
    const int lane = threadIdx.x & 63;
    rr.daz = (&tab.daz[0][0])[lane];
    rr.saz = (&tab.saz[0][0])[lane];
}
__device__ __forceinline__ float2 rule_entry(float2 v, int idx) {
    return make_float2(__builtin_bit_cast(float, __builtin_amdgcn_readlane(__builtin_bit_cast(int, v.x), idx)),
                       __builtin_bit_cast(float, __builtin_amdgcn_readlane(__builtin_bit_cast(int, v.y), idx)));
}

inline double vdc2_host(uint32_t i) {
    i = (i << 16) | (i >> 16);
    i = ((i & 0x55555555u) << 1) | ((i & 0xAAAAAAAAu) >> 1);
    i = ((i & 0x33333333u) << 2) | ((i & 0xCCCCCCCCu) >> 2);
    i = ((i & 0x0F0F0F0Fu) << 4) | ((i & 0xF0F0F0F0u) >> 4);
    i = ((i & 0x00FF00FFu) << 8) | ((i & 0xFF00FF00u) >> 8);
    return (double)i * 2.3283064365386963e-10;
}
inline void gauss_legendre01(int n, double* x, double* w) {
    for (int i = 0; i < n; ++i) {
        double z = std::cos(M_PI * (i + 0.75) / (n + 0.5)), pp = 1.0;
        for (int it = 0; it < 100; ++it) {
            double p1 = 1.0, p2 = 0.0;
            for (int j = 0; j < n; ++j) {
                double p3 = p2;
                p2 = p1;
                p1 = ((2.0 * j + 1.0) * z * p2 - j * p3) / (j + 1.0);
            }
            pp = n * (z * p1 - p2) / (z * z - 1.0);
            double z1 = z;
            z = z1 - p1 / pp;
            if (std::fabs(z - z1) < 1e-15) break;
        }
        x[n - 1 - i] = 0.5 * (z + 1.0);
        w[n - 1 - i] = 1.0 / ((1.0 - z * z) * pp * pp);
// ... 261 lines not shown
    const f2 d2 = sm.d + sm.d;
    sm.wlx = vfma(d2, sm.whx, -px.vx); sm.wly = vfma(d2, sm.why, -px.vy); sm.wlz = vfma(d2, R.ct, -px.vz);
    to_world(px.s, px.t, px.n, sm.wlx, sm.wly, sm.wlz, sm.wi);
    sm.NoL = vmax(sm.wlz, 0.0f);
    sm.dpos = vmax(sm.d, 0.0f);
    sm.g1l = rcp(vfma(sm.NoL, px.omk, px.kpe));
    sm.x5 = pow5(1.0f - sm.dpos);
}

template <bool JAC>
struct SpecAcc { f2 S0[3], S1[3], dS0[JAC ? 3 : 1], dS1[JAC ? 3 : 1]; };

template <bool JAC>
__device__ __forceinline__ void spec_accumulate(const Pixel& px, const LightRegs& lr, const RuleTable& tab, const RuleRegs& rr,
                                                SpecAcc<JAC>& A) {
#pragma unroll
    for (int c = 0; c < 3; ++c) {
        A.S0[c] = A.S1[c] = f2{0.0f, 0.0f};
        if (JAC) A.dS0[c] = A.dS1[c] = f2{0.0f, 0.0f};
    }
    const f2 four_over_r = 4.0f * rcp(px.r);
    const f2 cv = px.dk_dr * px.g1v * (1.0f - px.NoV);
    for (int k = 0; k < tab.nu_s; ++k) {
        const float4 rg = tab.sring[k];
        SpecRing R;
        spec_ring<JAC>(px, rg, R);
        f2 lam0 = f2{0.0f, 0.0f};
        if (JAC) lam0 = vfma(four_over_r, vfma(R.q * R.idq, -2.0f * rg.y, 1.0f), -cv);
        for (int j = 0; j < tab.nphi_s; ++j) {
            SpecSample sm;
            spec_sample(px, R, rule_entry(rr.saz, k * kMaxAz + j), sm);
            const f2 wgt = (R.ringw * sm.g1l) * (sm.NoL * sm.dpos);
            f2 L[3];
            sh_radiance(lr, sm.wi, L);
            const f2 wx = wgt * sm.x5;
#pragma unroll
            for (int c = 0; c < 3; ++c) {
                A.S0[c] = vfma(wgt, L[c], A.S0[c]);
                A.S1[c] = vfma(wx, L[c], A.S1[c]);
            }
            if (JAC) {
                const f2 lam = vfma(px.dk_dr * sm.g1l, sm.NoL - 1.0f, lam0);
                const f2 wl = wgt * lam, wlx = wl * sm.x5;
#pragma unroll
                for (int c = 0; c < 3; ++c) {
                    A.dS0[c] = vfma(wl, L[c], A.dS0[c]);
                    A.dS1[c] = vfma(wlx, L[c], A.dS1[c]);
                }
            }
        }
    }
}

constexpr int kStatsStride = 16;
enum { kStRatio = 0, kStMse, kStL1, kStSr, kStLa, kStLr, kStLm, kStLoss, kStImproved, kStBest, kStEsCounter, kStEsBest, kStEsHas,
       kStStopped, kStIters, kStGtSum };
constexpr int kStateStride = 20;
enum { kStSel = 16, kStBestRatio = 17, kStSelOld = 18  };
__device__ __forceinline__ bool img_stopped(const float* stats, int b) { return stats[b * kStatsStride + kStStopped] > 0.5f; }
__device__ __forceinline__ bool img_stopped_before(const float* stats, int b) { return stats[b * kStatsStride + kStStopped] > 1.5f; }

__device__ __forceinline__ bool stats_enter(float* st) {
    if (st[kStStopped] > 0.5f) {
        st[kStStopped] = 2.0f;
        st[kStImproved] = 0.0f;
        return true;
    }
    return false;
}
__device__ __forceinline__ void stats_commit(float* st, float mse, float l1, float sr, float la, float lr, float lm, float scale_delta,
                                             int es_patience, float es_min_delta, float* history, int hist_len, int batch, int b) {
    st[kStMse] = mse; st[kStL1] = l1; st[kStSr] = sr; st[kStLa] = la; st[kStLr] = lr; st[kStLm] = lm;
    st[kStLoss] = 3.0f * sr * mse + l1 + scale_delta * (la + lr + lm);
    float best = st[kStBest];
    bool improved = mse < best;
    st[kStImproved] = improved ? 1.0f : 0.0f;
    st[kStBest] = improved ? mse : best;
    const int it = (int)st[kStIters];
    if (history && it < hist_len) history[(long)it * batch + b] = mse;
    st[kStIters] = (float)(it + 1);
    if (es_patience > 0) {
        if (st[kStEsHas] < 0.5f) { st[kStEsBest] = mse; st[kStEsHas] = 1.0f; }
        else if (mse > st[kStEsBest] * (1.0f - es_min_delta)) {
            float cnt = st[kStEsCounter] + 1.0f;
            st[kStEsCounter] = cnt;
            if (cnt >= (float)es_patience) st[kStStopped] = 1.0f;
        } else { st[kStEsBest] = mse; st[kStEsCounter] = 0.0f; }
    }
}
constexpr int kStepRows = 384;
__host__ __device__ inline long step_part_stride(int rows) { return (long)rows * 5 + 4; }

struct ShadeArgs {
    const float *a, *r, *m, *n;
    const float* dcache;
    float* out;
    float* jac;
    const float* d_out;
    float *d_a, *d_r, *d_m;
    const float* stats;
    float* block_sums;
    int clamp;
    float* s1;
};

template <bool JAC>
__global__ __launch_bounds__(kBlock, 2) void shade_kernel(const ShadeArgs q, const float* __restrict__ light, const Geom g,
                                                          const RuleTable tab) {
    __shared__ float s_sum[4];
// ... 117 lines not shown
}

__global__ __launch_bounds__(kBlock, 2) void diffuse_cache_kernel(const float* __restrict__ n, const float* __restrict__ light,
                                                                  float* __restrict__ dcache, const Geom g, const RuleTable tab) {
    RuleRegs rr;
    load_rule_regs(tab, rr);
    const int b = blockIdx.y;
    const int P = g.H * g.W;
    const long BP = (long)gridDim.y * P;
    const int q0 = 2 * (blockIdx.x * kBlock + threadIdx.x);
    const bool act0 = q0 < P, two = q0 + 1 < P;
    const int p0 = act0 ? q0 : P - 1, p1 = two ? q0 + 1 : p0;
    const long i0 = (long)b * P + p0, i1 = (long)b * P + p1;
    Pixel px;
    f2 nv[3];
#pragma unroll
    for (int c = 0; c < 3; ++c) nv[c] = f2{n[i0 * 3 + c], n[i1 * 3 + c]};
    px.inv_len = rsq(vmax(dot3v(nv, nv), 1e-30f));
#pragma unroll
    for (int c = 0; c < 3; ++c) px.n[c] = nv[c] * px.inv_len;
    f2 fi = f2{(float)(p0 / g.W), (float)(p1 / g.W)}, fj = f2{(float)(p0 % g.W), (float)(p1 % g.W)};
    f2 x = (g.cx - fj) * g.inv_f, y = (fi - g.cy) * g.inv_f;
    f2 il = rsq(vfma(x, x, vfma(y, y, 1.0f)));
    f2 wo[3] = {x * il, y * il, il};
    frame(px.n, px.s, px.t);
    px.vx = dot3v(px.s, wo); px.vy = dot3v(px.t, wo); px.vz = dot3v(px.n, wo);
    px.NoV = vmax(px.vz, 0.0f);
    px.po = pow5(1.0f - px.NoV);
    LightRegs lr;
    load_light_regs(lr, light + (long)b * kNL);
    DiffuseCoef A;
    diffuse_coef(px, lr, tab, rr, A);
#pragma unroll
    for (int c = 0; c < 3; ++c) {
        if (act0) { dcache[c * BP + i0] = A.A0[c].x; dcache[(3 + c) * BP + i0] = A.A1[c].x; dcache[(6 + c) * BP + i0] = A.A2[c].x; }
        if (two) { dcache[c * BP + i1] = A.A0[c].y; dcache[(3 + c) * BP + i1] = A.A1[c].y; dcache[(6 + c) * BP + i1] = A.A2[c].y; }
    }
}

struct JacBwdArgs {
    const float *a, *r, *m;
    const float* jac;
    const float* d_out;
    float *d_a, *d_r, *d_m;
    const float *pred, *gt_srgb, *stats;
    const float *a0, *r0, *m0;
    float *best_a, *best_r, *best_m, *best_img;
    float *pa, *pr, *pm;
    float *am[3], *av[3];
    float scale_delta, inv_n3, inv_n1;
    unsigned part_mask;
    float lr_over_bc1, b1, b2, eps, inv_sqrt_bc2;
    int check_stop;
};
constexpr float kLossEps = 1e-8f;
__device__ __forceinline__ float fsign(float x) { return x > 0.0f ? 1.0f : (x < 0.0f ? -1.0f : 0.0f); }
__device__ __forceinline__ float pow_inv_gamma(float x) { return __builtin_amdgcn_exp2f(__builtin_amdgcn_logf(x) * (1.0f / 2.2f)); }
__device__ __forceinline__ float adam_update(float p, float gi, float* m, float* v, long i, const JacBwdArgs& q) {
    const unsigned off = (unsigned)i * 4u;
    float* mp = (float*)((char*)m + off);
    float* vp = (float*)((char*)v + off);
    const float mi = fmaf(q.b1, *mp, (1.0f - q.b1) * gi);
    const float vi = fmaf(q.b2, *vp, (1.0f - q.b2) * gi * gi);
    *mp = mi; *vp = vi;
    return p - q.lr_over_bc1 * mi / fmaf(fsqrt(vi), q.inv_sqrt_bc2, q.eps);
}

typedef _Float16 jac_h2 __attribute__((ext_vector_type(2)));
template <bool FUSED, bool J16 = false>
__global__ __launch_bounds__(kBlock) void jac_bwd_kernel(const JacBwdArgs q, long P) {
    const int b = blockIdx.y;
    if (FUSED && q.check_stop && img_stopped_before(q.stats, b)) return;
    const long p = (long)blockIdx.x * kBlock + threadIdx.x;
    if (p >= P) return;
    const long BP = (long)gridDim.y * P, i = (long)b * P + p;
    float a[3] = {q.a[i * 3], q.a[i * 3 + 1], q.a[i * 3 + 2]}, r = q.r[i], m = q.m[i];
    float ra[3] = {a[0], a[1], a[2]}, rr = r, rm = m;
    if (FUSED) {
#pragma unroll
        for (int c = 0; c < 3; ++c) a[c] = fminf(fmaxf(a[c], 0.0f), 1.0f);
        r = fminf(fmaxf(r, 0.07f), 1.0f);
        m = fminf(fmaxf(m, 0.0f), 1.0f);
    }
    float go[3], xs_keep[3];
    if (FUSED) {
        const float ratio = q.stats[b * kStatsStride + kStRatio], sr = q.stats[b * kStatsStride + kStSr];
#pragma unroll
        for (int c = 0; c < 3; ++c) {
            const float x = q.pred[i * 3 + c] * ratio;
            const float xc = fmaxf(x, kLossEps);
            const float xs = pow_inv_gamma(xc);
            const float d = xs - q.gt_srgb[i * 3 + c];
            const float dxs = x > kLossEps ? xs * rcp(xc) * (1.0f / 2.2f) : 0.0f;
            go[c] = ratio * dxs * fmaf(6.0f * sr, d, fsign(d)) * q.inv_n3;
            xs_keep[c] = xs;
        }
    } else {
#pragma unroll
        for (int c = 0; c < 3; ++c) go[c] = q.d_out[i * 3 + c];
    }
    float da[3], dr = 0.0f, dm = 0.0f;
    const float omm = 1.0f - m;
    float jrv[3] = {0.0f, 0.0f, 0.0f};
    if (J16) {
        const jac_h2 u3 = __builtin_bit_cast(jac_h2, q.jac[3 * BP + i]), u4 = __builtin_bit_cast(jac_h2, q.jac[4 * BP + i]);
        jrv[0] = (float)u3.x; jrv[1] = (float)u3.y; jrv[2] = (float)u4.x;
    }
#pragma unroll
    for (int c = 0; c < 3; ++c) {
        float Pc, SD, JR;
        if (J16) {
            const jac_h2 u = __builtin_bit_cast(jac_h2, q.jac[c * BP + i]);
            Pc = (float)u.x; SD = (float)u.y; JR = jrv[c];
        } else {
            Pc = q.jac[c * BP + i]; SD = q.jac[(3 + c) * BP + i]; JR = q.jac[(6 + c) * BP + i];
        }
        da[c] = go[c] * fmaf(m, SD, omm * Pc);
        dm = fmaf(go[c], fmaf(a[c] - 0.04f, SD, -(a[c] * Pc)), dm);
        dr = fmaf(go[c], JR, dr);
    }
    if (!FUSED) {
#pragma unroll
        for (int c = 0; c < 3; ++c) q.d_a[i * 3 + c] = da[c];
        q.d_r[i] = dr;
        q.d_m[i] = dm;
        return;
    }
    const bool improved = q.stats[b * kStatsStride + kStImproved] > 0.5f;
#pragma unroll
    for (int c = 0; c < 3; ++c) {
        float gsum = da[c] + ((q.part_mask & MATPBR_PART_A) ? q.scale_delta * q.inv_n3 * fsign(a[c] - q.a0[i * 3 + c]) : 0.0f);
        gsum = (ra[c] >= 0.0f && ra[c] <= 1.0f) ? gsum : 0.0f;
        if (q.d_a) q.d_a[i * 3 + c] = gsum;
        if (improved && q.best_a) q.best_a[i * 3 + c] = a[c];
        if (improved && q.best_img) q.best_img[i * 3 + c] = xs_keep[c];
        if ((q.part_mask & MATPBR_PART_A) && q.am[0]) q.pa[i * 3 + c] = adam_update(ra[c], gsum, q.am[0], q.av[0], i * 3 + c, q);
    }
    float gr = dr + ((q.part_mask & MATPBR_PART_R) ? q.scale_delta * q.inv_n1 * fsign(r - q.r0[i]) : 0.0f);
    float gm = dm + ((q.part_mask & MATPBR_PART_M) ? q.scale_delta * q.inv_n1 * fsign(m - q.m0[i]) : 0.0f);
    gr = (rr >= 0.07f && rr <= 1.0f) ? gr : 0.0f;
    gm = (rm >= 0.0f && rm <= 1.0f) ? gm : 0.0f;
    if (q.d_r) q.d_r[i] = gr;
    if (q.d_m) q.d_m[i] = gm;
    if (improved && q.best_r) q.best_r[i] = r;
    if (improved && q.best_m) q.best_m[i] = m;
    if ((q.part_mask & MATPBR_PART_R) && q.am[1]) q.pr[i] = adam_update(rr, gr, q.am[1], q.av[1], i, q);
    if ((q.part_mask & MATPBR_PART_M) && q.am[2]) q.pm[i] = adam_update(rm, gm, q.am[2], q.av[2], i, q);
}

struct LightGradUse {
    const f2* gw;
    float* dc;
    template <int K> __device__ __forceinline__ void operator()(f2 Bk) {
#pragma unroll
        for (int c = 0; c < 3; ++c) dc[K * 3 + c] = fmaf(gw[c].y, Bk.y, fmaf(gw[c].x, Bk.x, dc[K * 3 + c]));
    }
};
template <int K0, int K1>
struct TransferUse {
    const f2* w;
    f2* acc;
    template <int K> __device__ __forceinline__ void operator()(f2 Bk) {
        if (K >= K0 && K < K1) {
#pragma unroll
            for (int c = 0; c < 3; ++c) acc[(K - K0) * 3 + c] = vfma(w[c], Bk, acc[(K - K0) * 3 + c]);
        }
    }
};

template <bool WANT_N, bool WANT_W, class Use>
__device__ __forceinline__ void walk_samples(const Pixel& px, const LightRegs& lr, const RuleTable& tab, const RuleRegs& rr, const f2 go[3],
                                             Use&& use, f2& dnx, f2& dny) {
    const f2 omm = 1.0f - px.m;
    f2 kd[3], C0[3], ga[3], gC[3], gD[3];
#pragma unroll
    for (int c = 0; c < 3; ++c) {
        kd[c] = px.a[c] * omm;
        C0[c] = vfma(px.m, px.a[c], omm * 0.04f);
        if (WANT_N) { ga[c] = go[c] * kd[c]; gC[c] = go[c] * C0[c]; gD[c] = go[c] - gC[c]; }
    }
    f2 gvd = f2{0.0f, 0.0f}, scs = f2{0.0f, 0.0f};
    for (int k = 0; k < tab.nu_d; ++k) {
        const float4 rg = tab.dring[k];
        const float4 rg2 = tab.dring2[k];
        for (int j = 0; j < tab.nphi_d; ++j) {
            const float2 az = rule_entry(rr.daz, k * kMaxAz + j);
            f2 wi[3];
            to_world(px.s, px.t, px.n, az.x, az.y, rg.x, wi);
            const f2 u = vfma(px.vz, rg.x, vfma(px.vy, az.y, vfma(px.vx, az.x, 1.0f)));
            const f2 qq = vfma(px.r, u, -0.5f);
            const f2 Fo = vfma(qq, px.po, 1.0f), Fi = vfma(qq, rg2.x, 1.0f);
            if (WANT_W) {
                const f2 wff = (Fo * Fi) * rg.y;
                f2 wc[3] = {kd[0] * wff, kd[1] * wff, kd[2] * wff};
                use(wi, wc);
            }
// ... 287 lines not shown
```

materialist_amd/csrc/posmlp_kernels.hip:

```cpp
#include <hip/hip_runtime.h>
#include <stdint.h>
#include <atomic>
#include <type_traits>

#include "../../include/matpbr.h"
#include "../../include/matpbr_experimental.h"
#include "posmlp_device.hpp"

namespace {


constexpr int kBM = 128, kBN = 128, kBK = 32;
constexpr int kPersistent = 512;
constexpr int EPI_SINCOS = 0, EPI_MULC = 1, EPI_BIAS = 2;

struct HeadArgs {
  const float* w;
  int ldw;
  const float* bias;
  ArmHead h;
};

__global__ __launch_bounds__(256) void mlp_tail_copy_kernel(float* __restrict__ out, int ldo, const float* __restrict__ tail, int ldt, long M, int N) {
  const int w = 256 - N;
  const long total = M * w;
  for (long i = (long)blockIdx.x * 256 + threadIdx.x; i < total; i += (long)gridDim.x * 256) {
    const long m = i / w;
    const int j = (int)(i - m * w);
    out[m * ldo + N + j] = tail[m * ldt + j];
  }
}
__device__ __forceinline__ void store4_upto(float* dst, float4 v, int valid, bool all) {
  if (all) {
    *reinterpret_cast<float4*>(dst) = v;
    return;
  }
  if (valid >= 4) {
    *reinterpret_cast<float4*>(dst) = v;
  } else {
    if (valid > 0) dst[0] = v.x;
    if (valid > 1) dst[1] = v.y;
    if (valid > 2) dst[2] = v.z;
  }
}

struct NtArgs {
  const float* A;
  const float* B;
  const float* bias;
  const float* cmul;
  float* out0;
  float* out1;
  float* colsum;
  int M;
  int N, K, lda, ldb, ldo;
  const float* tail;
  int ldt;
  int cmul_sin;
  const float* x0;
  int ldx0;
// ... 610 lines not shown
#pragma unroll
    for (int q = 0; q < 8; ++q) *reinterpret_cast<float4*>(sX + (tid + 256 * q) * 4) = rx[q];
  };

  f32x16 acc[2][4];
#pragma unroll
  for (int mi = 0; mi < 2; ++mi)
#pragma unroll
    for (int ni = 0; ni < 4; ++ni)
#pragma unroll
      for (int r = 0; r < 16; ++r) acc[mi][ni][r] = 0.f;

  if (m_begin < m_end) {
    gload(m_begin);
    sstore();
    __syncthreads();
    const float* pa = sG + lh * 128 + wm * 64 + li;
    const float* pb = sX + lh * 256 + wn * 128 + li;
    for (long m0 = m_begin; m0 < m_end; m0 += kWM) {
      const bool more = m0 + kWM < m_end;
      if (more) gload(m0 + kWM);
#pragma unroll
      for (int kk = 0; kk < kWM / 2; ++kk) {
        float a[2], b[4];
#pragma unroll
        for (int mi = 0; mi < 2; ++mi) a[mi] = pa[2 * kk * 128 + mi * 32];
#pragma unroll
        for (int ni = 0; ni < 4; ++ni) b[ni] = pb[2 * kk * 256 + ni * 32];
#pragma unroll
        for (int mi = 0; mi < 2; ++mi)
#pragma unroll
          for (int ni = 0; ni < 4; ++ni) acc[mi][ni] = __builtin_amdgcn_mfma_f32_32x32x2f32(a[mi], b[ni], acc[mi][ni], 0, 0, 0);
      }
      __syncthreads();
      if (more) {
        sstore();
        __syncthreads();
      }
    }
  }
  float* out = partial + (long)blockIdx.x * 256 * 256;
#pragma unroll
  for (int mi = 0; mi < 2; ++mi)
#pragma unroll
    for (int ni = 0; ni < 4; ++ni)
#pragma unroll
      for (int r = 0; r < 16; ++r) {
        const int n = n0 + wm * 64 + mi * 32 + (r & 3) + 8 * (r >> 2) + 4 * lh;
        const int k = wn * 128 + ni * 32 + li;
        out[n * 256 + k] = acc[mi][ni][r];
      }
}

__device__ __forceinline__ void wgrad_reduce_body(float* red, const float* __restrict__ partial, int slabs, float* __restrict__ dW, int N, int K, int ldw,
                                                  int block) {
  const int t = threadIdx.x & 255, sl = threadIdx.x >> 8;
  const int idx = block * 256 + t;
  const int per = (slabs + 3) / 4, c0 = sl * per, c1 = c0 + per < slabs ? c0 + per : slabs;
  float s0 = 0.f, s1 = 0.f, s2 = 0.f, s3 = 0.f;
  int c = c0;
  for (; c + 3 < c1; c += 4) {
    s0 += partial[(long)(c + 0) * 65536 + idx];
    s1 += partial[(long)(c + 1) * 65536 + idx];
    s2 += partial[(long)(c + 2) * 65536 + idx];
    s3 += partial[(long)(c + 3) * 65536 + idx];
  }
  for (; c < c1; ++c) s0 += partial[(long)c * 65536 + idx];
  red[sl * 256 + t] = (s0 + s1) + (s2 + s3);
  __syncthreads();
  const int n = idx >> 8, k = idx & 255;
  if (sl == 0 && n < N && k < K) dW[(long)n * ldw + k] = (red[t] + red[256 + t]) + (red[512 + t] + red[768 + t]);
}
__global__ __launch_bounds__(1024) void mlp_wgrad_reduce(const float* __restrict__ partial, int slabs, float* __restrict__ dW, int N, int K,
                                                         int ldw) {
  __shared__ float red[1024];
  wgrad_reduce_body(red, partial, slabs, dW, N, K, ldw, (int)blockIdx.x);
}

__device__ __forceinline__ void colsum_reduce_body(float* red, const float* __restrict__ part, int groups, float* __restrict__ out, int col) {
  const bool act = threadIdx.x < 256;
  float s = 0.f;
  if (act) {
    for (int g = threadIdx.x; g < groups; g += 256) s += part[(long)g * 256 + col];
    red[threadIdx.x] = s;
  }
  __syncthreads();
#pragma unroll
  for (int w = 128; w > 0; w >>= 1) {
    if ((int)threadIdx.x < w) red[threadIdx.x] += red[threadIdx.x + w];
    __syncthreads();
  }
  if (threadIdx.x == 0) out[col] = red[0];
}
__global__ __launch_bounds__(256) void mlp_colsum_reduce(const float* __restrict__ part, int groups, float* __restrict__ out) {
  __shared__ float red[256];
  colsum_reduce_body(red, part, groups, out, (int)blockIdx.x);
}



constexpr long kSmallM = 1024;

__device__ __forceinline__ float4 ld4_masked(const float* p, int k, int K) {
  float4 v = *reinterpret_cast<const float4*>(p);
  v.x = k < K ? v.x : 0.f;
  v.y = k + 1 < K ? v.y : 0.f;
  v.z = k + 2 < K ? v.z : 0.f;
  v.w = k + 3 < K ? v.w : 0.f;
  return v;
}

template <int EPI, bool BKN = false>
__device__ __forceinline__ void small_nt_body(const NtArgs& p, int block) {
  __shared__ float s_part[4][16 * 64];
  __shared__ float s_col[4][32];
  const int wave = threadIdx.x >> 6, lane = threadIdx.x & 63, li = lane & 31, lh = lane >> 5;
  const int tiles_n = (p.N + 31) >> 5;
  const int tm = block / tiles_n, tn = block - tm * tiles_n;
  const int row = min(tm * 32 + li, p.M - 1), col = min(tn * 32 + li, p.N - 1);
  const float* pa = p.A + (size_t)row * p.lda;
  const float* pb = BKN ? p.B + col : p.B + (size_t)col * p.ldb;
  const int kpad = (p.K + 3) & ~3;
  const int kq = (((p.K + 3) / 4) + 7) & ~7;
  const int k_begin = wave * kq;
  f32x16 acc;
#pragma unroll
  for (int r = 0; r < 16; ++r) acc[r] = 0.f;
  {
    float4 a[8], b[8];
#pragma unroll
    for (int j = 0; j < 8; ++j) {
      const int k = k_begin + 8 * j + 4 * lh;
      const int kc = k < kpad ? k : kpad - 4;
      const bool mine = 8 * j < kq;
      a[j] = ld4_masked(pa + kc, k, mine ? p.K : 0);
      if (BKN) {
        const int K_ = mine ? p.K : 0;
        b[j].x = k < K_ ? pb[(size_t)min(k, p.K - 1) * p.ldb] : 0.f;
        b[j].y = k + 1 < K_ ? pb[(size_t)min(k + 1, p.K - 1) * p.ldb] : 0.f;
        b[j].z = k + 2 < K_ ? pb[(size_t)min(k + 2, p.K - 1) * p.ldb] : 0.f;
        b[j].w = k + 3 < K_ ? pb[(size_t)min(k + 3, p.K - 1) * p.ldb] : 0.f;
      } else {
        b[j] = ld4_masked(pb + kc, k, mine ? p.K : 0);
      }
    }
#pragma unroll
    for (int j = 0; j < 8; ++j) {
      if (8 * j < kq && k_begin + 8 * j < p.K) {
        acc = __builtin_amdgcn_mfma_f32_32x32x2f32(a[j].x, b[j].x, acc, 0, 0, 0);
// ... 1387 lines not shown
    float mine[J];
#pragma unroll
    for (int j = 0; j < J; ++j) mine[j] = 0.f;
    float4 x[R];
    auto load_rows = [&](int g) {
#pragma unroll
      for (int r = 0; r < R; ++r) {
        long m = row0 + g * R + r;
        m = m < M ? m : M - 1;
        x[r] = in ? *reinterpret_cast<const float4*>(X + m * ldx + k0) : make_float4(0.f, 0.f, 0.f, 0.f);
      }
    };
    load_rows(0);
    for (int g = 0; g < 64 / R; ++g) {
      float4 cur[R];
#pragma unroll
      for (int r = 0; r < R; ++r) cur[r] = x[r];
      if (g + 1 < 64 / R) load_rows(g + 1);
#pragma unroll
      for (int r = 0; r < R; ++r) {
        const int row = g * R + r;
#pragma unroll
        for (int j = 0; j < J; ++j) {
          const float t = wave_sum_lane63(fmaf(cur[r].x, w[j].x, fmaf(cur[r].y, w[j].y, fmaf(cur[r].z, w[j].z, cur[r].w * w[j].w))));
          const float total = __builtin_bit_cast(float, __builtin_amdgcn_readlane(__builtin_bit_cast(int, t), 63));
          mine[j] = lane == row ? total : mine[j];
        }
      }
    }
    const long m = row0 + lane;
    if (m < M) {
      float v[J];
#pragma unroll
      for (int j = 0; j < J; ++j) v[j] = mine[j] + bias[j];
      if (out != nullptr) {
#pragma unroll
        for (int j = 0; j < J; ++j) out[m * ldo + j] = v[j];
      }
      if (HEAD) arm_head_store(h, m, v);
    }
  }
}

template <int J, bool HEAD>
void launch_skinny_nt(const float* x, int ldx, const float* w, int ldw, const float* bias, float* out, int ldo, long M, int K, const ArmHead& h,
                      hipStream_t stream) {
  const long tiles = (M + 63) / 64;
  const unsigned grid = (unsigned)((tiles + 3) / 4 < 2048 ? (tiles + 3) / 4 : 2048);
  hipLaunchKernelGGL((mlp_skinny_nt_kernel<J, HEAD>), dim3(grid), dim3(256), 0, stream, x, ldx, w, ldw, bias, out, ldo, M, K, h);
}

__global__ __launch_bounds__(256) void arm_head_bwd_kernel(const float* __restrict__ g_a, const float* __restrict__ g_r, const float* __restrict__ g_m,
                                                           const float* __restrict__ th, float* __restrict__ d_x, long M) {
  for (long m = (long)blockIdx.x * 256 + threadIdx.x; m < M; m += (long)gridDim.x * 256) {
    const float4 t0 = *reinterpret_cast<const float4*>(th + m * 8);
    const float t4 = th[m * 8 + 4];
    float4 o = make_float4(0.f, 0.f, 0.f, 0.f);
    float o4 = 0.f;
    if (g_a) {
      o.x = (g_a[m * 3 + 0] * 1.3f) * (1.f - t0.x * t0.x);
      o.y = (g_a[m * 3 + 1] * 1.3f) * (1.f - t0.y * t0.y);
      o.z = (g_a[m * 3 + 2] * 1.3f) * (1.f - t0.z * t0.z);
    }
    if (g_r) o.w = ((g_r[m] * 0.93f) * 1.3f) * (1.f - t0.w * t0.w);
    if (g_m) o4 = (g_m[m] * 1.3f) * (1.f - t4 * t4);
    *reinterpret_cast<float4*>(d_x + m * 8) = o;
    *reinterpret_cast<float4*>(d_x + m * 8 + 4) = make_float4(o4, 0.f, 0.f, 0.f);
  }
}

constexpr int kSkinnySlabs = 1024;
constexpr int kOutJ = 5;
struct SkinnyDgrad {
  const float* W;
  int ldw, Jv;
  const float* cmul;
  float* G;
  int ldg;
  float* gsum_part;
  unsigned* tmax;
};
template <int J, bool DGRAD = false, int JV = kOutJ>
__global__ __launch_bounds__(256) void mlp_skinny_tn_kernel(const float* __restrict__ S, int lds, const float* __restrict__ B, int ldb,
                                                            float* __restrict__ partial, float* __restrict__ bpart, long M, long rows_per_slab,
                                                            const SkinnyDgrad dg) {
  __shared__ float red[3][8][256];
  __shared__ float bred[4][J];
  const int cq = threadIdx.x & 63, rs = __builtin_amdgcn_readfirstlane(threadIdx.x >> 6);
  const long m_begin = (long)blockIdx.x * rows_per_slab;
  const long m_end = (m_begin + rows_per_slab < M) ? m_begin + rows_per_slab : M;
  float4 acc[J];
  float bs[J];
#pragma unroll
  for (int j = 0; j < J; ++j) { acc[j] = make_float4(0.f, 0.f, 0.f, 0.f); bs[j] = 0.f; }
  float4 wv[DGRAD ? JV : 1], gsum = make_float4(0.f, 0.f, 0.f, 0.f);
  if (DGRAD) {
#pragma unroll
    for (int j = 0; j < JV; ++j) wv[j] = j < dg.Jv ? *reinterpret_cast<const float4*>(dg.W + (size_t)j * dg.ldw + 4 * cq) : make_float4(0.f, 0.f, 0.f, 0.f);
  }
  constexpr int U = 4;
  float tmx = 0.f;
  long tmx_tile = m_begin / kBM;
  auto tmx_flush = [&]() {
    if (DGRAD && dg.tmax != nullptr) {
      const float wmx = wave_max_lane63(tmx);
      if (cq == 63) atomicMax(dg.tmax + tmx_tile, __float_as_uint(wmx));
    }
    tmx = 0.f;
  };
  for (long m0 = m_begin + rs; m0 < m_end; m0 += 4 * U) {
    float4 b[U];
#pragma unroll
    for (int u = 0; u < U; ++u) {
      const long m = m0 + 4 * u;
      b[u] = m < m_end ? *reinterpret_cast<const float4*>(B + m * ldb + 4 * cq) : make_float4(0.f, 0.f, 0.f, 0.f);
    }
#pragma unroll
    for (int u = 0; u < U; ++u) {
      const long m = m0 + 4 * u < m_end ? m0 + 4 * u : m_end - 1;
      const float* srow = S + m * lds;
      const bool live = m0 + 4 * u < m_end;
// ... 19 lines not shown
        if (m / kBM != tmx_tile) {
          tmx_flush();
          tmx_tile = m / kBM;
        }
        tmx = __builtin_fmaxf(__builtin_fmaxf(tmx, __builtin_fmaxf(__builtin_fabsf(gv.x), __builtin_fabsf(gv.y))), __builtin_fmaxf(__builtin_fabsf(gv.z), __builtin_fabsf(gv.w)));
      }
    }
  }
  if (DGRAD) tmx_flush();
  if (DGRAD) {
    if (rs > 0) *reinterpret_cast<float4*>(&red[rs - 1][0][4 * cq]) = gsum;
    __syncthreads();
    if (rs == 0) {
#pragma unroll
      for (int q = 0; q < 3; ++q) {
        const float4 o = *reinterpret_cast<const float4*>(&red[q][0][4 * cq]);
        gsum.x += o.x; gsum.y += o.y; gsum.z += o.z; gsum.w += o.w;
      }
      *reinterpret_cast<float4*>(dg.gsum_part + (size_t)blockIdx.x * 256 + 4 * cq) = gsum;
    }
    __syncthreads();
  }
  if (cq == 0) {
#pragma unroll
    for (int j = 0; j < J; ++j) bred[rs][j] = bs[j];
  }
#pragma unroll
  for (int j0 = 0; j0 < J; j0 += 8) {
    if (j0 > 0) __syncthreads();
    if (rs > 0) {
#pragma unroll
      for (int j = 0; j < 8; ++j) *reinterpret_cast<float4*>(&red[rs - 1][j][4 * cq]) = acc[j0 + j];
    }
    __syncthreads();
    if (rs == 0) {
#pragma unroll
      for (int j = 0; j < 8; ++j) {
        float4 t = acc[j0 + j];
#pragma unroll
        for (int q = 0; q < 3; ++q) {
          const float4 o = *reinterpret_cast<const float4*>(&red[q][j][4 * cq]);
          t.x += o.x; t.y += o.y; t.z += o.z; t.w += o.w;
        }
        *reinterpret_cast<float4*>(partial + ((size_t)blockIdx.x * J + j0 + j) * 256 + 4 * cq) = t;
      }
    }
  }
  if (rs == 0 && bpart != nullptr && threadIdx.x < J)
    bpart[(size_t)blockIdx.x * J + threadIdx.x] = (bred[0][threadIdx.x] + bred[1][threadIdx.x]) + (bred[2][threadIdx.x] + bred[3][threadIdx.x]);
}

__device__ __forceinline__ void skinny_reduce_body(float* red_, int block, const float* __restrict__ partial, const float* __restrict__ bpart, int slabs, int J, int Jv,
                                                             int C, float* __restrict__ out, long ld_j, long ld_c, float* __restrict__ d_b,
                                                             const float* __restrict__ gsum_part, int C2, float* __restrict__ d_b2) {
  float (*red)[64] = reinterpret_cast<float (*)[64]>(red_);
  int j = block >> 2;
  const int cl = threadIdx.x & 63, c = (block & 3) * 64 + cl, sl = threadIdx.x >> 6;
  if (j == J) {
    partial = gsum_part; J = 1; j = 0; Jv = 1; C = C2; out = d_b2; ld_j = 0; ld_c = 1; d_b = nullptr;
  }
  if (j >= Jv) return;
  float a0 = 0.f, a1 = 0.f, a2 = 0.f, a3 = 0.f;
  int q = sl;
  for (; q + 48 < slabs; q += 64) {
    a0 += partial[((size_t)q * J + j) * 256 + c];
    a1 += partial[((size_t)(q + 16) * J + j) * 256 + c];
    a2 += partial[((size_t)(q + 32) * J + j) * 256 + c];
    a3 += partial[((size_t)(q + 48) * J + j) * 256 + c];
  }
  for (; q < slabs; q += 16) a0 += partial[((size_t)q * J + j) * 256 + c];
  red[sl][cl] = (a0 + a1) + (a2 + a3);
  __syncthreads();
  if (sl == 0 && c < C) {
    float t = 0.f;
#pragma unroll
    for (int u = 0; u < 16; ++u) t += red[u][cl];
    out[j * ld_j + c * ld_c] = t;
  }
  if (d_b != nullptr && bpart != nullptr && (block & 3) == 0) {
    __syncthreads();
    float t = 0.f;
    for (int q2 = threadIdx.x; q2 < slabs; q2 += 1024) t += bpart[(size_t)q2 * J + j];
    red[sl][cl] = t;
    __syncthreads();
    if (sl == 0) {
      float u = 0.f;
#pragma unroll
      for (int r = 0; r < 16; ++r) u += red[r][cl];
      red[0][cl] = u;
    }
    __syncthreads();
    if (threadIdx.x == 0) {
      float u = 0.f;
      for (int r = 0; r < 64; ++r) u += red[0][r];
      d_b[j] = u;
    }
  }
}
__global__ __launch_bounds__(1024) void mlp_skinny_tn_reduce(const float* __restrict__ partial, const float* __restrict__ bpart, int slabs, int J, int Jv,
                                                             int C, float* __restrict__ out, long ld_j, long ld_c, float* __restrict__ d_b,
                                                             const float* __restrict__ gsum_part, int C2, float* __restrict__ d_b2) {
  __shared__ float red[1024];
  skinny_reduce_body(red, (int)blockIdx.x, partial, bpart, slabs, J, Jv, C, out, ld_j, ld_c, d_b, gsum_part, C2, d_b2);
}

constexpr int kMaxReduceJobs = 16;
struct ReduceJobs {
  MatpbrReduceJob j[kMaxReduceJobs];
  int first[kMaxReduceJobs + 1];
  int n;
};
__global__ __launch_bounds__(1024) void mlp_reduce_jobs_kernel(const ReduceJobs js) {
  __shared__ float red[1024];
  int k = 0;
  while (k + 1 < js.n && (int)blockIdx.x >= js.first[k + 1]) ++k;
  const MatpbrReduceJob& q = js.j[k];
  const int block = (int)blockIdx.x - js.first[k];
  if (q.kind == MATPBR_REDUCE_WGRAD) wgrad_reduce_body(red, q.src, q.groups, q.dst, q.n0, q.n1, q.n2, block);
  else if (q.kind == MATPBR_REDUCE_COLSUM) colsum_reduce_body(red, q.src, q.groups, q.dst, block);
  else skinny_reduce_body(red, block, q.src, q.src_b, q.groups, q.n0, q.n1, q.n2, q.dst, q.ld_j, q.ld_c, q.dst_b, q.src_g, q.n3, q.dst_g);
}
inline int reduce_job_blocks(const MatpbrReduceJob& q) {
  if (q.kind == MATPBR_REDUCE_WGRAD) return 256;
  if (q.kind == MATPBR_REDUCE_COLSUM) return q.n0;
  return q.n0 * 4 + (q.dst_g ? 4 : 0);
}
inline void launch_reduce_job(const MatpbrReduceJob& q, hipStream_t st) {
  if (q.kind == MATPBR_REDUCE_WGRAD) hipLaunchKernelGGL(mlp_wgrad_reduce, dim3(256), dim3(1024), 0, st, q.src, q.groups, q.dst, q.n0, q.n1, q.n2);
  else if (q.kind == MATPBR_REDUCE_COLSUM) hipLaunchKernelGGL(mlp_colsum_reduce, dim3(q.n0), dim3(256), 0, st, q.src, q.groups, q.dst);
  else hipLaunchKernelGGL(mlp_skinny_tn_reduce, dim3(reduce_job_blocks(q)), dim3(1024), 0, st, q.src, q.src_b, q.groups, q.n0, q.n1, q.n2, q.dst, q.ld_j, q.ld_c,
                          q.dst_b, q.src_g, q.n3, q.dst_g);
}
inline void reduce_or_defer(const MatpbrReduceJob& q, MatpbrReduceJob* defer, hipStream_t st) {
  if (defer) *defer = q;
  else launch_reduce_job(q, st);
}

}

extern "C" {

int matpbr_mlp_set_wgrad_kernel(int kernel) { return g_wg_hx.exchange(kernel != 0 ? 1 : 0, std::memory_order_relaxed); }

int matpbr_mlp_set_lds_dma(int mode) {
  g_nt_w0_gx.store(mode == 3 ? 1 : 0, std::memory_order_relaxed);
  const int was = g_nt_gl.exchange(mode < 0 ? 0 : (mode > 2 ? 2 : mode), std::memory_order_relaxed);
  return was;
}

int matpbr_mlp_layer_fwd_tail(const float* x, int ldx, const float* w, int ldw, const float* bias, float* s_out, float* c_out, int ldo,
                              const float* tail, int ldt, long M, int N, int K, void* stream) {
  if (!x || !w || !bias || !s_out || M <= 0 || M > 0x7fffff00L || N <= 0 || N > 256 || K <= 0 || K > 256) return MATPBR_ERR_INVALID_ARG;
  if ((ldx & 3) || (ldw & 3) || ldx < ((K + 3) & ~3) || ldw < ((K + 3) & ~3) || ldo < N || !aligned16(x) || !aligned16(w))
    return MATPBR_ERR_INVALID_ARG;
  if (tail && (ldo < 256 || ldt < 256 - N || !c_out)) return MATPBR_ERR_INVALID_ARG;
  NtArgs p{x, w, bias, nullptr, s_out, c_out, nullptr, 0, N, K, ldx, ldw, ldo};
  p.tail = tail; p.ldt = ldt;
  const bool thin = M > kSmallM && K <= 16 && ldx >= thin_pad(K) && ldw >= ((K + 3) & ~3) && ldo >= 256 && !(ldo & 3) && aligned16(s_out) &&
                    (!c_out || aligned16(c_out));
  if (M <= kSmallM) {
    if (c_out) launch_small_nt<EPI_SINCOS>(p, M, (hipStream_t)stream);
    else launch_small_nt<EPI_BIAS>(p, M, (hipStream_t)stream);
  } else if (thin) {
    p.M = (int)M;
    if (c_out) launch_thin_k<EPI_SINCOS>(p, (hipStream_t)stream);
    else launch_thin_k<EPI_BIAS>(p, (hipStream_t)stream);
  } else if (c_out)
    launch_nt<EPI_SINCOS>(p, M, (hipStream_t)stream);
  else
    launch_nt<EPI_BIAS>(p, M, (hipStream_t)stream);
  if (tail && N < 256)
    hipLaunchKernelGGL(mlp_tail_copy_kernel, dim3((unsigned)((M * (256 - N) + 255) / 256 < 2048 ? (M * (256 - N) + 255) / 256 : 2048)), dim3(256), 0,
                       (hipStream_t)stream, s_out, ldo, tail, ldt, M, N);
  return hipGetLastError() == hipSuccess ? MATPBR_OK : MATPBR_ERR_LAUNCH;
}

int matpbr_mlp_layer_fwd_sgn(const float* x, int ldx, const float* w, int ldw, const float* bias, float* s_out, int ldo, const float* tail, int ldt,
                             long M, int N, int K, void* stream) {
  if (!x || !w || !bias || !s_out || M <= 0 || M > 0x7fffff00L || N <= 0 || N > 256 || K <= 0 || K > 16) return MATPBR_ERR_INVALID_ARG;
  if (M <= kSmallM || (ldx & 3) || (ldw & 3) || ldx < thin_pad(K) || ldw < ((K + 3) & ~3) || ldo < 256 || (ldo & 3) || !aligned16(x) || !aligned16(w) ||
      !aligned16(s_out))
// ... 226 lines not shown
  reduce_or_defer(q2, defer ? defer + 1 : nullptr, (hipStream_t)stream);
  return hipGetLastError() == hipSuccess ? MATPBR_OK : MATPBR_ERR_LAUNCH;
}

int matpbr_mlp_first_layer_bwd_bx(const float* g, int ldg, const void* wtsplit, const float* c_prev, int ldc, int sgn, const float* x0, int ldx0,
                                  float* d_w0, long ld_j, long ld_c, int d0, float* d_bias0, void* workspace, size_t workspace_bytes, void* workspace2,
                                  size_t workspace2_bytes, long M, int n0, int n_red, int nprod, void* stream) {
  if (nprod == 3) return MATPBR_ERR_INVALID_ARG;
  return mlp_first_layer_bwd_impl(g, ldg, wtsplit, c_prev, ldc, sgn, x0, ldx0, d_w0, ld_j, ld_c, d0, d_bias0, workspace, workspace_bytes, workspace2,
                                  workspace2_bytes, M, n0, n_red, nprod, nullptr, stream);
}
int matpbr_mlp_first_layer_bwd_blk(const float* g, int ldg, const void* g_tile_max, const void* wtsplit, const float* s_prev, int lds, const float* x0, int ldx0,
                                   float* d_w0, long ld_j, long ld_c, int d0, float* d_bias0, void* workspace, size_t workspace_bytes, void* workspace2,
                                   size_t workspace2_bytes, long M, int n0, int n_red, MatpbrReduceJob* defer2, void* stream) {
  return mlp_first_layer_bwd_impl(g, ldg, wtsplit, s_prev, lds, 1, x0, ldx0, d_w0, ld_j, ld_c, d0, d_bias0, workspace, workspace_bytes, workspace2,
                                  workspace2_bytes, M, n0, n_red, 3, (const unsigned*)g_tile_max, stream, defer2);
}
int matpbr_mlp_layer_bwd_input_blk(const float* g, int ldg, const void* g_tile_max, const void* wtsplit, const float* s_prev, float* g_prev, int ldo,
                                   void* out_tile_max, float* d_bias_prev, void* workspace, size_t workspace_bytes, long M, int n_prev, int n_red,
                                   MatpbrReduceJob* defer, void* stream) {
  return mlp_layer_bwd_input_bx_impl(g, ldg, wtsplit, s_prev, g_prev, ldo, d_bias_prev, workspace, workspace_bytes, M, n_prev, n_red, 3, 1, stream,
                                     (const unsigned*)g_tile_max, (unsigned*)out_tile_max, defer);
}

int matpbr_mlp_layer_bwd_input_bx(const float* g, int ldg, const void* wtsplit, const float* c_prev, float* g_prev, int ldo, float* d_bias_prev,
                                  void* workspace, size_t workspace_bytes, long M, int n_prev, int n_red, int nprod, void* stream) {
  if (nprod == 3) return MATPBR_ERR_INVALID_ARG;
  return mlp_layer_bwd_input_bx_impl(g, ldg, wtsplit, c_prev, g_prev, ldo, d_bias_prev, workspace, workspace_bytes, M, n_prev, n_red, nprod, 0, stream);
}
int matpbr_mlp_layer_bwd_input_bx_sgn(const float* g, int ldg, const void* wtsplit, const float* s_prev, float* g_prev, int ldo, float* d_bias_prev,
                                      void* workspace, size_t workspace_bytes, long M, int n_prev, int n_red, int nprod, void* stream) {
  if (nprod == 3) return MATPBR_ERR_INVALID_ARG;
  return mlp_layer_bwd_input_bx_impl(g, ldg, wtsplit, s_prev, g_prev, ldo, d_bias_prev, workspace, workspace_bytes, M, n_prev, n_red, nprod, 1, stream);
}

static int wgrad_slabs(long M) {
  long s = (M + 255) / 256;
  if (s > 256) s = 256;
  if (s < 1) s = 1;
  return (int)s;
}

size_t matpbr_mlp_bwd_weight_workspace_bytes(long M) { return (size_t)wgrad_slabs(M) * 256 * 256 * sizeof(float); }

int matpbr_mlp_layer_bwd_weight(const float* g, int ldg, const float* x, int ldx, float* d_w, int ldw, void* workspace,
                                size_t workspace_bytes, long M, int N, int K, void* stream) {
  if (!g || !x || !d_w || M <= 0 || N <= 0 || N > 256 || K <= 0 || K > 256) return MATPBR_ERR_INVALID_ARG;
  if ((ldg & 3) || (ldx & 3) || ldg < N || ldx < ((K + 3) & ~3) || ldw < K || !aligned16(g) || !aligned16(x)) return MATPBR_ERR_INVALID_ARG;
  if (M <= kSmallM) {
    const int tiles = ((N + 31) / 32) * ((K + 31) / 32);
    hipLaunchKernelGGL(mlp_small_tn, dim3((unsigned)tiles), dim3(256), 0, (hipStream_t)stream, g, ldg, x, ldx, d_w, ldw, (int)M, N, K);
    return hipGetLastError() == hipSuccess ? MATPBR_OK : MATPBR_ERR_LAUNCH;
  }
  if (!workspace || workspace_bytes < matpbr_mlp_bwd_weight_workspace_bytes(M)) return MATPBR_ERR_WORKSPACE;
  const int slabs = wgrad_slabs(M);
  long rows = (M + slabs - 1) / slabs;
  rows = (rows + kWM - 1) / kWM * kWM;
  hipLaunchKernelGGL(mlp_wgrad_tn, dim3(slabs, (N + 127) / 128), dim3(256), 0, (hipStream_t)stream, g, ldg, x, ldx, (float*)workspace, M, rows, K);
  hipLaunchKernelGGL(mlp_wgrad_reduce, dim3(256), dim3(1024), 0, (hipStream_t)stream, (const float*)workspace, slabs, d_w, N, K, ldw);
  return hipGetLastError() == hipSuccess ? MATPBR_OK : MATPBR_ERR_LAUNCH;
}

static int mlp_layer_bwd_weight_bx_impl(const float* g, int ldg, const float* x, int ldx, float* d_w, int ldw, void* workspace,
                                        size_t workspace_bytes, long M, int N, int K, int nprod, const unsigned* g_tile_max, void* stream,
                                        MatpbrReduceJob* defer = nullptr) {
  if (!g || !x || !d_w || M <= 0 || N <= 0 || N > 256 || K <= 0 || K > 256) return MATPBR_ERR_INVALID_ARG;
  if (nprod == 3 && (!g_tile_max || (M % kBM))) return MATPBR_ERR_INVALID_ARG;
  if ((nprod != 3 && nprod != 6 && nprod != 9) || (M & 15) || ldg < 256 || ldx < 256 || (ldg & 3) || (ldx & 3) || ldw < K || !aligned16(g) || !aligned16(x))
    return MATPBR_ERR_UNSUPPORTED;
  if (!workspace || workspace_bytes < matpbr_mlp_bwd_weight_workspace_bytes(M)) return MATPBR_ERR_WORKSPACE;
  int slabs = wgrad_slabs(M);
  long rows = ((M + slabs - 1) / slabs + 15) / 16 * 16;
  slabs = (int)((M + rows - 1) / rows);
  if (nprod == 3 && g_wg_hx.load(std::memory_order_relaxed) != 0 && (long)ldg * 4 >= 1024 && (long)ldx * 4 >= 1024 && (long)3 * ldg * 4 + 1024 < (1l << 31) && (long)3 * ldx * 4 + 1024 < (1l << 31)) {
    if (!lds_opt_in<&mlp_wgrad_hx>(kHxSmem)) return MATPBR_ERR_LAUNCH;
    hipLaunchKernelGGL(mlp_wgrad_hx, dim3(slabs), dim3(kWgThreads), kHxSmem, (hipStream_t)stream, g, ldg, x, ldx, (float*)workspace, M, rows, g_tile_max);
  } else if (nprod == 3) {
    if (!lds_opt_in<&mlp_wgrad_bx<3>>(kWgSmem)) return MATPBR_ERR_LAUNCH;
    hipLaunchKernelGGL(mlp_wgrad_bx<3>, dim3(slabs), dim3(kWgThreads), kWgSmem, (hipStream_t)stream, g, ldg, x, ldx, (float*)workspace, M, rows, g_tile_max);
  } else if (nprod == 6) {
    if (!lds_opt_in<&mlp_wgrad_bx<6>>(kWgSmem)) return MATPBR_ERR_LAUNCH;
    hipLaunchKernelGGL(mlp_wgrad_bx<6>, dim3(slabs), dim3(kWgThreads), kWgSmem, (hipStream_t)stream, g, ldg, x, ldx, (float*)workspace, M, rows, (const unsigned*)nullptr);
  } else {
    if (!lds_opt_in<&mlp_wgrad_bx<9>>(kWgSmem)) return MATPBR_ERR_LAUNCH;
    hipLaunchKernelGGL(mlp_wgrad_bx<9>, dim3(slabs), dim3(kWgThreads), kWgSmem, (hipStream_t)stream, g, ldg, x, ldx, (float*)workspace, M, rows, (const unsigned*)nullptr);
  }
  MatpbrReduceJob q{};
  q.kind = MATPBR_REDUCE_WGRAD; q.groups = slabs; q.src = (const float*)workspace; q.dst = d_w; q.n0 = N; q.n1 = K; q.n2 = ldw;
  reduce_or_defer(q, defer, (hipStream_t)stream);
  return hipGetLastError() == hipSuccess ? MATPBR_OK : MATPBR_ERR_LAUNCH;
}
int matpbr_mlp_layer_bwd_weight_bx(const float* g, int ldg, const float* x, int ldx, float* d_w, int ldw, void* workspace,
                                   size_t workspace_bytes, long M, int N, int K, int nprod, void* stream) {
  if (nprod == 3) return MATPBR_ERR_INVALID_ARG;
  return mlp_layer_bwd_weight_bx_impl(g, ldg, x, ldx, d_w, ldw, workspace, workspace_bytes, M, N, K, nprod, nullptr, stream);
}
int matpbr_mlp_layer_bwd_weight_blk(const float* g, int ldg, const void* g_tile_max, const float* x, int ldx, float* d_w, int ldw, void* workspace,
                                    size_t workspace_bytes, long M, int N, int K, MatpbrReduceJob* defer, void* stream) {
  return mlp_layer_bwd_weight_bx_impl(g, ldg, x, ldx, d_w, ldw, workspace, workspace_bytes, M, N, K, 3, (const unsigned*)g_tile_max, stream, defer);
}

int matpbr_mlp_skinny_fwd(const float* x, int ldx, const float* w, int ldw, const float* bias, float* out, int ldo, long M, int J, int K,
                          void* stream) {
  if (!x || !w || !bias || !out || M <= 0 || (J != 3 && J != 5 && J != 8) || K <= 0 || K > 256 || (K & 3)) return MATPBR_ERR_INVALID_ARG;
  if ((ldx & 3) || ldx < K || (ldw & 3) || ldw < K || ldo < J || !aligned16(x) || !aligned16(w)) return MATPBR_ERR_INVALID_ARG;
  const ArmHead none{nullptr, 0, nullptr, nullptr, nullptr, nullptr};
  if (J == 3) launch_skinny_nt<3, false>(x, ldx, w, ldw, bias, out, ldo, M, K, none, (hipStream_t)stream);
  else if (J == 5) launch_skinny_nt<5, false>(x, ldx, w, ldw, bias, out, ldo, M, K, none, (hipStream_t)stream);
  else launch_skinny_nt<8, false>(x, ldx, w, ldw, bias, out, ldo, M, K, none, (hipStream_t)stream);
  return hipGetLastError() == hipSuccess ? MATPBR_OK : MATPBR_ERR_LAUNCH;
}

int matpbr_mlp_arm_head_fwd(const float* x, int ldx, const float* w, int ldw, const float* bias, const float* start, int lds, float* th,
                            float* map_a, float* map_r, float* map_m, long M, int K, void* stream) {
  if (!x || !w || !bias || !start || !th || M <= 0 || K <= 0 || K > 256 || (K & 3) || lds < 5) return MATPBR_ERR_INVALID_ARG;
  if ((ldx & 3) || ldx < K || (ldw & 3) || ldw < K || !aligned16(x) || !aligned16(w) || !aligned16(th)) return MATPBR_ERR_INVALID_ARG;
  const ArmHead h{start, lds, th, map_a, map_r, map_m};
  launch_skinny_nt<5, true>(x, ldx, w, ldw, bias, nullptr, 0, M, K, h, (hipStream_t)stream);
  return hipGetLastError() == hipSuccess ? MATPBR_OK : MATPBR_ERR_LAUNCH;
}

int matpbr_mlp_arm_head_bwd(const float* g_a, const float* g_r, const float* g_m, const float* th, float* d_x, long M, void* stream) {
  if (!th || !d_x || M <= 0 || !aligned16(th) || !aligned16(d_x)) return MATPBR_ERR_INVALID_ARG;
// ... 12 lines not shown
  const int JP = (J + 7) / 8 * 8;
  if (lds < JP || ldb < 256 || (ldb & 3) || !aligned16(b)) return MATPBR_ERR_INVALID_ARG;
  if (!workspace || workspace_bytes < matpbr_mlp_skinny_workspace_bytes(J)) return MATPBR_ERR_WORKSPACE;
  long rows = (M + kSkinnySlabs - 1) / kSkinnySlabs;
  rows = (rows + 3) / 4 * 4;
  const int slabs = (int)((M + rows - 1) / rows);
  float* partial = (float*)workspace;
  float* bpart = partial + (size_t)kSkinnySlabs * JP * 256;
  if (JP == 8) hipLaunchKernelGGL((mlp_skinny_tn_kernel<8>), dim3(slabs), dim3(256), 0, (hipStream_t)stream, s, lds, b, ldb, partial, bpart, M, rows, SkinnyDgrad{});
  else hipLaunchKernelGGL((mlp_skinny_tn_kernel<16>), dim3(slabs), dim3(256), 0, (hipStream_t)stream, s, lds, b, ldb, partial, bpart, M, rows, SkinnyDgrad{});
  hipLaunchKernelGGL(mlp_skinny_tn_reduce, dim3(JP * 4), dim3(1024), 0, (hipStream_t)stream, (const float*)partial, (const float*)bpart, slabs, JP, J, C, d_w,
                     ld_j, ld_c, d_bias, (const float*)nullptr, 0, (float*)nullptr);
  return hipGetLastError() == hipSuccess ? MATPBR_OK : MATPBR_ERR_LAUNCH;
}

static int mlp_out_layer_bwd_impl(const float* d_x, int ldd, const float* s_prev, const float* c_prev, int lds, const float* w_out, int ldw, float* g_prev,
                                  int ldg, float* d_w, long ld_j, long ld_c, float* d_bias, float* d_bias_prev, void* workspace, size_t workspace_bytes,
                                  long M, int J, int n_prev, unsigned* g_tile_max, void* stream, MatpbrReduceJob* defer = nullptr) {
  if (!d_x || !s_prev || !w_out || !g_prev || !d_w || M <= 0 || J <= 0 || J > 8 || n_prev <= 0 || n_prev > 256) return MATPBR_ERR_INVALID_ARG;
  if (ldd < 8 || lds < 256 || (lds & 3) || ldg < 256 || (ldg & 3) || ldw < 256 || (ldw & 3) || !aligned16(s_prev) || !aligned16(g_prev) || !aligned16(w_out) ||
      (c_prev && !aligned16(c_prev)))
    return MATPBR_ERR_INVALID_ARG;
  if (!workspace || workspace_bytes < matpbr_mlp_skinny_workspace_bytes(J)) return MATPBR_ERR_WORKSPACE;
  long rows = (M + kSkinnySlabs - 1) / kSkinnySlabs;
  rows = (rows + 3) / 4 * 4;
  const int slabs = (int)((M + rows - 1) / rows);
  float* partial = (float*)workspace;
  float* bpart = partial + (size_t)kSkinnySlabs * 8 * 256;
  float* gsum_part = bpart + (size_t)kSkinnySlabs * 8;
  SkinnyDgrad dg{w_out, ldw, J, c_prev, g_prev, ldg, gsum_part, g_tile_max};
  if (J <= kOutJ) hipLaunchKernelGGL((mlp_skinny_tn_kernel<8, true>), dim3(slabs), dim3(256), 0, (hipStream_t)stream, d_x, ldd, s_prev, lds, partial, bpart, M, rows, dg);
  else hipLaunchKernelGGL((mlp_skinny_tn_kernel<8, true, 8>), dim3(slabs), dim3(256), 0, (hipStream_t)stream, d_x, ldd, s_prev, lds, partial, bpart, M, rows, dg);
  MatpbrReduceJob q{};
  q.kind = MATPBR_REDUCE_SKINNY; q.groups = slabs; q.src = partial; q.src_b = bpart; q.src_g = gsum_part; q.dst = d_w; q.dst_b = d_bias; q.dst_g = d_bias_prev;
  q.n0 = 8; q.n1 = J; q.n2 = 256; q.n3 = n_prev; q.ld_j = ld_j; q.ld_c = ld_c;
  reduce_or_defer(q, defer, (hipStream_t)stream);
  return hipGetLastError() == hipSuccess ? MATPBR_OK : MATPBR_ERR_LAUNCH;
}

int matpbr_mlp_out_layer_bwd(const float* d_x, int ldd, const float* s_prev, const float* c_prev, int lds, const float* w_out, int ldw, float* g_prev,
                             int ldg, float* d_w, long ld_j, long ld_c, float* d_bias, float* d_bias_prev, void* workspace, size_t workspace_bytes,
                             long M, int J, int n_prev, void* stream) {
  return mlp_out_layer_bwd_impl(d_x, ldd, s_prev, c_prev, lds, w_out, ldw, g_prev, ldg, d_w, ld_j, ld_c, d_bias, d_bias_prev, workspace, workspace_bytes, M, J,
                                n_prev, nullptr, stream);
}
int matpbr_mlp_out_layer_bwd_tmax(const float* d_x, int ldd, const float* s_prev, const float* c_prev, int lds, const float* w_out, int ldw, float* g_prev,
                                  int ldg, void* g_tile_max, float* d_w, long ld_j, long ld_c, float* d_bias, float* d_bias_prev, void* workspace,
                                  size_t workspace_bytes, long M, int J, int n_prev, MatpbrReduceJob* defer, void* stream) {
  if (!g_tile_max) return MATPBR_ERR_INVALID_ARG;
  return mlp_out_layer_bwd_impl(d_x, ldd, s_prev, c_prev, lds, w_out, ldw, g_prev, ldg, d_w, ld_j, ld_c, d_bias, d_bias_prev, workspace, workspace_bytes, M, J,
                                n_prev, (unsigned*)g_tile_max, stream, defer);
}

int matpbr_mlp_reduce_jobs(const MatpbrReduceJob* jobs, int n_jobs, void* stream) {
  if (!jobs || n_jobs <= 0 || n_jobs > kMaxReduceJobs) return MATPBR_ERR_INVALID_ARG;
  ReduceJobs js{};
  int blocks = 0;
  for (int i = 0; i < n_jobs; ++i) {
    const MatpbrReduceJob& q = jobs[i];
    if (q.kind == MATPBR_REDUCE_NONE) continue;
    if ((q.kind != MATPBR_REDUCE_WGRAD && q.kind != MATPBR_REDUCE_COLSUM && q.kind != MATPBR_REDUCE_SKINNY) || !q.src || !q.dst || q.groups <= 0 || q.n0 <= 0)
      return MATPBR_ERR_INVALID_ARG;
    js.j[js.n] = q;
    js.first[js.n] = blocks;
    blocks += reduce_job_blocks(q);
    ++js.n;
  }
  if (js.n == 0) return MATPBR_OK;
  js.first[js.n] = blocks;
  hipLaunchKernelGGL(mlp_reduce_jobs_kernel, dim3((unsigned)blocks), dim3(1024), 0, (hipStream_t)stream, js);
  return hipGetLastError() == hipSuccess ? MATPBR_OK : MATPBR_ERR_LAUNCH;
}

}
```

materialist_amd/ops.py:

```python
from __future__ import annotations

import ctypes
from typing import Dict, Optional

import torch

from . import _lib
from ._lib import MatpbrCamera, MatpbrError

LIGHT_SH25 = 0
NSH = 25
MAX_SPP = 128
FLAG_CLAMP_PARAMS = 1
FLAG_ATTACHED_SAMPLING = 2
FLAG_LAZY_FORCE = 16
FLAG_JAC16 = 32
FLAG_MODELS_READY = 64
FLAG_ROTATE_BEST = 128
FLAG_GENERIC_STEP = 256
FLAG_JAC32 = 512
FLAG_SHARE_GPU = 2048
LAZY_NSTATE = 28
LAZY_PLANES = 30
STATS_STRIDE = 16
# ... 408 lines not shown
        B, (H, W) = 1, depth.shape
    elif depth.ndim == 3:
        B, H, W = depth.shape
    else:
        raise ValueError("depth must be [H,W] or [B,H,W]")
    out = torch.empty(tuple(depth.shape) + (3,), dtype=torch.float32, device=depth.device)
    cam = MatpbrCamera(float(fov_x_deg))
    with torch.cuda.device(depth.device):
        code = lib.matpbr_normals_from_depth(_ptr(depth), _ptr(out), H, W, B, ctypes.byref(cam), _stream(depth))
    _lib.check(code, "matpbr_normals_from_depth")
    return out


def new_loss_stats(batch: int, device) -> torch.Tensor:
    st = torch.zeros((batch, STATS_STRIDE), dtype=torch.float32, device=device)
    st[:, STAT_BEST] = float("inf")
    return st


def part_mask(optimize_part: str) -> int:
    return sum({"a": PART_A, "r": PART_R, "m": PART_M, "n": PART_N}.get(ch, 0) for ch in optimize_part)


def brdf_loss_stats(pred, gt, gt_srgb, pa, pr, pm, a0, r0, m0, scale_delta: float, stats: torch.Tensor,
                    workspace: Optional[torch.Tensor] = None, optimize_part: str = "arm", es_patience: int = -1, es_min_delta: float = 0.0,
                    history: Optional[torch.Tensor] = None) -> torch.Tensor:
    lib = _lib.load()
    pred = _dev(pred, "pred", (3,))
    B, H, W = _bhw(pred)
    ts = [_dev(t, k) for t, k in ((gt, "gt"), (gt_srgb, "gt_srgb"), (pa, "pa"), (pr, "pr"), (pm, "pm"), (a0, "a0"), (r0, "r0"), (m0, "m0"))]
    need = int(lib.matpbr_brdf_loss_workspace_bytes(B))
    if workspace is None or workspace.numel() * 4 < need:
        workspace = torch.empty(need // 4, dtype=torch.float32, device=pred.device)
    with torch.cuda.device(pred.device):
        code = lib.matpbr_brdf_loss_stats_es(_ptr(pred), *[_ptr(t) for t in ts], float(scale_delta), _ptr(stats), _ptr(workspace),
                                             workspace.numel() * 4, H, W, B, part_mask(optimize_part), int(es_patience), float(es_min_delta),
                                             _ptr(history), 0 if history is None else int(history.shape[0]), _stream(pred))
    _lib.check(code, "matpbr_brdf_loss_stats")
    return stats


def brdf_loss_dpred(pred, gt_srgb, stats, d_pred) -> torch.Tensor:
    lib = _lib.load()
    pred = _dev(pred, "pred", (3,))
    B, H, W = _bhw(pred)
    with torch.cuda.device(pred.device):
        code = lib.matpbr_brdf_loss_dpred(_ptr(pred), _ptr(_dev(gt_srgb, "gt_srgb", (3,))), _ptr(stats), _ptr(_dev(d_pred, "d_pred", (3,))), H, W, B,
                                          _stream(pred))
    _lib.check(code, "matpbr_brdf_loss_dpred")
    return d_pred


def brdf_loss_bwd_jac(pa, pr, pm, jac, pred, gt_srgb, stats, a0, r0, m0, scale_delta: float, d_a, d_r, d_m,
                      best_a=None, best_r=None, best_m=None, best_img=None, optimize_part: str = "arm", jac16: bool = False) -> None:
    lib = _lib.load()
    pa = _dev(pa, "pa", (3,))
    B, H, W = _bhw(pa)
    with torch.cuda.device(pa.device), _timed("shade_bwd"):
        code = lib.matpbr_brdf_loss_bwd_jac(_ptr(pa), _ptr(pr), _ptr(pm), _ptr(jac), _ptr(pred), _ptr(gt_srgb), _ptr(stats), _ptr(a0), _ptr(r0),
                                            _ptr(m0), float(scale_delta), _ptr(d_a), _ptr(d_r), _ptr(d_m), _ptr(best_a), _ptr(best_r),
                                            _ptr(best_m), _ptr(best_img), H, W, B, part_mask(optimize_part) | (FLAG_JAC16 if jac16 else 0), _stream(pa))
    _lib.check(code, "matpbr_brdf_loss_bwd_jac")


def adam_step(p, g, m, v, lr: float, step: int, beta1: float = 0.9, beta2: float = 0.999, eps: float = 1e-8) -> None:
    lib = _lib.load()
    with torch.cuda.device(p.device):
        code = lib.matpbr_adam_step(_ptr(p), _ptr(g), _ptr(m), _ptr(v), p.numel(), float(lr), float(beta1), float(beta2), float(eps),
                                    int(step), _stream(p))
    _lib.check(code, "matpbr_adam_step")


_colsum_ws = {}


def column_sum(x: torch.Tensor) -> torch.Tensor:
    lib = _lib.load()
    x = _dev(x, "x")
    if x.ndim != 2:
        raise ValueError("column_sum expects [M, N]")
    M, N = x.shape
    key = (x.device, N)
    if key not in _colsum_ws:
        _colsum_ws[key] = torch.empty(int(lib.matpbr_column_sum_workspace_bytes(N)) // 4, dtype=torch.float32, device=x.device)
    ws = _colsum_ws[key]
    out = torch.empty(N, dtype=torch.float32, device=x.device)
    with torch.cuda.device(x.device):
        code = lib.matpbr_column_sum(_ptr(x), _ptr(out), M, N, _ptr(ws), ws.numel() * 4, _stream(x))
    _lib.check(code, "matpbr_column_sum")
    return out


def shade_transfer(a, r, m, n, spp: int, fov_x_deg: float = 35.0) -> torch.Tensor:
    lib = _lib.load()
    a = _dev(a, "albedo", (3,))
    B, H, W = _bhw(a)
    r, m, n = _dev(r, "roughness").reshape(B, H, W, 1), _dev(m, "metallic").reshape(B, H, W, 1), _dev(n, "normal", (3,))
    T = torch.empty(int(lib.matpbr_transfer_bytes(H, W, B)) // 4, dtype=torch.float32, device=a.device)
    cam = MatpbrCamera(float(fov_x_deg))
    with torch.cuda.device(a.device):
        code = lib.matpbr_shade_transfer(_ptr(a), _ptr(r), _ptr(m), _ptr(n), _ptr(T), H, W, B, check_spp(spp), ctypes.byref(cam), 0, _stream(a))
    _lib.check(code, "matpbr_shade_transfer")
    return T


def relight(T, lights, H: int, W: int, out: Optional[torch.Tensor] = None) -> torch.Tensor:
    lib = _lib.load()
    T = _dev(T, "T")
    lights = _dev(lights, "lights", (NSH, 3)).reshape(-1, NSH, 3)
    if T.numel() * 4 < int(lib.matpbr_transfer_bytes(H, W, 1)):
        raise ValueError("relight: T is smaller than matpbr_transfer_bytes(H, W, 1)")
    F_ = lights.shape[0]
    if out is None:
        out = torch.empty((F_, H, W, 3), dtype=torch.float32, device=T.device)
# ... 239 lines not shown
                                                 _ptr(g_prev), g_prev.stride(0), _ptr(g_tile_max), _ptr(d_w), d_w.stride(0), 1, _ptr(d_bias),
                                                 _ptr(d_bias_prev), _ptr(ws), ws.numel() * 4, M, int(J), int(n_prev), defer[0] if defer else None, _stream(s_prev))
    _lib.check(code, "matpbr_mlp_out_layer_bwd_tmax")


def mlp_layer_bwd_input_blk(g: torch.Tensor, g_tile_max: torch.Tensor, wtsplit: torch.Tensor, s_prev: torch.Tensor, g_prev: torch.Tensor, n_prev: int,
                            n_red: int, d_bias_prev: Optional[torch.Tensor], out_tile_max: Optional[torch.Tensor], defer=None) -> None:
    lib = _lib.load()
    g = _mat2(g, "g")
    M = g.shape[0]
    if s_prev.stride(0) != g_prev.stride(0):
        raise ValueError("s_prev and g_prev must share their row stride")
    ws = _mlp_workspace("bwd_input" + (defer[1] if defer else ""), M, g.device, lib.matpbr_mlp_bwd_input_workspace_bytes(M))
    with torch.cuda.device(g.device):
        code = lib.matpbr_mlp_layer_bwd_input_blk(_ptr(g), g.stride(0), _ptr(g_tile_max), _ptr(wtsplit), _ptr(s_prev), _ptr(g_prev), g_prev.stride(0),
                                                  _ptr(out_tile_max) if out_tile_max is not None else None,
                                                  _ptr(d_bias_prev) if d_bias_prev is not None else None, _ptr(ws), ws.numel() * 4, M, n_prev, n_red,
                                                  defer[0] if defer else None, _stream(g))
    _lib.check(code, "matpbr_mlp_layer_bwd_input_blk")


def mlp_first_layer_bwd_blk(g: torch.Tensor, g_tile_max: torch.Tensor, wtsplit: torch.Tensor, s_prev: torch.Tensor, x0: torch.Tensor, d_w0: torch.Tensor,
                            d0: int, n0: int, n_red: int, d_bias0: Optional[torch.Tensor], defer=None) -> None:
    lib = _lib.load()
    g, s_prev, x0 = _mat2(g, "g"), _mat2(s_prev, "s_prev"), _mat2(x0, "x0")
    M = g.shape[0]
    ws = _mlp_workspace("bwd_input" + (defer[1] if defer else ""), M, g.device, lib.matpbr_mlp_bwd_input_workspace_bytes(M))
    ws2 = _mlp_workspace("skinny2" + (defer[1] if defer else ""), 0, g.device, lib.matpbr_mlp_skinny_workspace_bytes(16))
    with torch.cuda.device(g.device):
        code = lib.matpbr_mlp_first_layer_bwd_blk(_ptr(g), g.stride(0), _ptr(g_tile_max), _ptr(wtsplit), _ptr(s_prev), s_prev.stride(0), _ptr(x0), x0.stride(0),
                                                  _ptr(d_w0), 1, d_w0.stride(0), int(d0), _ptr(d_bias0), _ptr(ws), ws.numel() * 4, _ptr(ws2), ws2.numel() * 4,
                                                  M, int(n0), int(n_red), defer[0] if defer else None, _stream(g))
    _lib.check(code, "matpbr_mlp_first_layer_bwd_blk")


def mlp_layer_bwd_weight_blk(g: torch.Tensor, g_tile_max: torch.Tensor, x: torch.Tensor, N: int, K: int, out: Optional[torch.Tensor] = None,
                             defer=None) -> torch.Tensor:
    lib = _lib.load()
    g, x = _mat2(g, "g"), _mat2(x, "x")
    M = g.shape[0]
    ws = _mlp_workspace("bwd_weight" + (defer[1] if defer else ""), M, g.device, lib.matpbr_mlp_bwd_weight_workspace_bytes(M))
    d_w = out if out is not None else torch.empty((N, K), dtype=torch.float32, device=g.device)
    with torch.cuda.device(g.device):
        code = lib.matpbr_mlp_layer_bwd_weight_blk(_ptr(g), g.stride(0), _ptr(g_tile_max), _ptr(x), x.stride(0), _ptr(d_w), d_w.stride(0), _ptr(ws),
                                                   ws.numel() * 4, M, N, K, defer[0] if defer else None, _stream(g))
    _lib.check(code, "matpbr_mlp_layer_bwd_weight_blk")
    return d_w


def mlp_set_wgrad_kernel(kernel: int) -> int:
    return int(_lib.load().matpbr_mlp_set_wgrad_kernel(int(kernel)))


def mlp_reduce_jobs(jobs, n: int, like: torch.Tensor) -> None:
    with torch.cuda.device(like.device):
        code = _lib.load().matpbr_mlp_reduce_jobs(ctypes.byref(jobs), int(n), _stream(like))
    _lib.check(code, "matpbr_mlp_reduce_jobs")


LIGHT_SH9, LIGHT_ENV_TEXELS = 1, 2


class _LightToSh25(torch.autograd.Function):
    @staticmethod
    def forward(ctx, light, kind):
        lib = _lib.load()
        light = _dev(light, "light")
        B, n = light.shape[0], light.shape[1]
        out = torch.empty((B, NSH, 3), dtype=torch.float32, device=light.device)
        with torch.cuda.device(light.device):
            code = lib.matpbr_light_to_sh25(_ptr(light), int(kind), n, _ptr(out), B, _stream(light))
        _lib.check(code, "matpbr_light_to_sh25")
        ctx.kind, ctx.n = int(kind), n
        return out

    @staticmethod
    def backward(ctx, d_out):
        lib = _lib.load()
        d_out = d_out.contiguous()
        B = d_out.shape[0]
        d_light = torch.empty((B, ctx.n, 3), dtype=torch.float32, device=d_out.device)
        with torch.cuda.device(d_out.device):
            code = lib.matpbr_light_to_sh25_bwd(_ptr(d_out), ctx.kind, ctx.n, _ptr(d_light), B, _stream(d_out))
        _lib.check(code, "matpbr_light_to_sh25_bwd")
        return d_light, None


def light_to_sh25(light: torch.Tensor, kind: int) -> torch.Tensor:
    squeeze = light.ndim == 2
    out = _LightToSh25.apply(light.reshape((1,) + tuple(light.shape)) if squeeze else light, kind)
    return out[0] if squeeze else out


def adamw_step_dev(p: torch.Tensor, g: torch.Tensor, m: torch.Tensor, v: torch.Tensor, hyper: torch.Tensor, weight_decay: float = 0.01,
                   beta1: float = 0.9, beta2: float = 0.999, eps: float = 1e-8) -> None:
    lib = _lib.load()
    with torch.cuda.device(p.device):
        code = lib.matpbr_adamw_step_dev(_ptr(p), _ptr(g), _ptr(m), _ptr(v), p.numel(), _ptr(hyper), float(beta1), float(beta2), float(eps),
                                         float(weight_decay), _stream(p))
    _lib.check(code, "matpbr_adamw_step_dev")


def brdf_terms(cos1, cos2, r, f0) -> torch.Tensor:
    lib = _lib.load()
    cos1, cos2, r, f0 = (_dev(t, k).reshape(-1) for t, k in ((cos1, "cos1"), (cos2, "cos2"), (r, "r"), (f0, "f0")))
    N = cos1.numel()
# ... 6 lines not shown
```

Before: 663.5 it/s.

## Fuse loss ratio, arm head backward, and AdamW into neighbouring kernels

Removes the separate loss_final1 kernel by having the second loss-sum kernel fold the per-block partial sums into the ratio itself. The arm head backward moves into the loss-backward kernel through a new _head entry point. The AdamW snapshot step moves into the deferred reduce-jobs kernel, which now validates that every destination lies inside the flat gradient. The goal is fewer kernel launches and global round-trips per optimisation step. The cost is redundant ratio reduction in every block and more complex ordering inside the reduce kernel.

After: 663.5 it/s (median of 2 runs). No clear change (-0.0%).

```diff
diff --git a/include/matpbr.h b/include/matpbr.h
--- a/include/matpbr.h
+++ b/include/matpbr.h
@@ -89,6 +89,10 @@
                              const float* gt_srgb, const float* stats, const float* a0, const float* r0, const float* m0,
                              float scale_delta, float* d_a, float* d_r, float* d_m, float* best_a, float* best_r, float* best_m,
                              float* best_img, int H, int W, int batch, uint32_t flags, void* stream);
+int matpbr_brdf_loss_bwd_jac_head(const float* pa, const float* pr, const float* pm, const float* jac, const float* pred,
+                                  const float* gt_srgb, const float* stats, const float* a0, const float* r0, const float* m0,
+                                  float scale_delta, float* d_a, float* d_r, float* d_m, float* best_a, float* best_r, float* best_m,
+                                  float* best_img, const float* th, float* d_x, int H, int W, int batch, uint32_t flags, void* stream);
 int matpbr_adam_step(float* p, const float* g, float* m, float* v, long n, float lr, float beta1, float beta2, float eps,
                      int step, void* stream);
 
diff --git a/include/matpbr_mlp.h b/include/matpbr_mlp.h
--- a/include/matpbr_mlp.h
+++ b/include/matpbr_mlp.h
@@ -100,6 +100,8 @@
                           float weight_decay, void* stream);
 int matpbr_adamw_step_snapshot_dev(float* p, const float* g, float* m, float* v, long n, float* hyper, float beta1, float beta2,
                                    float eps, float weight_decay, float* best, const float* stats, void* stream);
+int matpbr_mlp_reduce_jobs_adamw(const MatpbrReduceJob* jobs, int n_jobs, float* p, float* g, float* m, float* v, long n, float* hyper, float beta1,
+                                 float beta2, float eps, float weight_decay, float* best, const float* stats, void* stream);
 
 #ifdef __cplusplus
 }
diff --git a/materialist_amd/_lib.py b/materialist_amd/_lib.py
--- a/materialist_amd/_lib.py
+++ b/materialist_amd/_lib.py
@@ -82,6 +82,8 @@
                                                 ctypes.c_int, ctypes.c_uint32, ctypes.c_int, ctypes.c_float, _c_f, ctypes.c_int, ctypes.c_void_p]),
     "matpbr_brdf_loss_bwd_jac": (ctypes.c_int, [_c_f] * 10 + [ctypes.c_float] + [_c_f] * 7 + [ctypes.c_int, ctypes.c_int, ctypes.c_int,
                                                                                               ctypes.c_uint32, ctypes.c_void_p]),
+    "matpbr_brdf_loss_bwd_jac_head": (ctypes.c_int, [_c_f] * 10 + [ctypes.c_float] + [_c_f] * 9 + [ctypes.c_int, ctypes.c_int, ctypes.c_int,
+                                                                                                   ctypes.c_uint32, ctypes.c_void_p]),
     "matpbr_brdf_phase_workspace_bytes": (ctypes.c_size_t, [ctypes.c_int] * 3),
     "matpbr_brdf_phase_step": (ctypes.c_int, [ctypes.POINTER(MatpbrBrdfPhase), ctypes.c_int, ctypes.c_float, ctypes.c_void_p]),
     "matpbr_brdf_phase_stages": (ctypes.c_int, [ctypes.POINTER(MatpbrBrdfPhase), ctypes.c_int, ctypes.c_float, ctypes.c_uint32, ctypes.c_void_p]),
@@ -119,6 +121,8 @@
                                                      ctypes.c_long, ctypes.c_long, _c_f, _c_f, ctypes.c_void_p, ctypes.c_size_t, ctypes.c_long, ctypes.c_int,
                                                      ctypes.c_int, ctypes.c_void_p, ctypes.c_void_p]),
     "matpbr_mlp_reduce_jobs": (ctypes.c_int, [ctypes.c_void_p, ctypes.c_int, ctypes.c_void_p]),
+    "matpbr_mlp_reduce_jobs_adamw": (ctypes.c_int, [ctypes.c_void_p, ctypes.c_int] + [_c_f] * 4 + [ctypes.c_long, _c_f, ctypes.c_float, ctypes.c_float,
+                                                                                                 ctypes.c_float, ctypes.c_float, _c_f, _c_f, ctypes.c_void_p]),
     "matpbr_mlp_layer_bwd_input_blk": (ctypes.c_int, [_c_f, ctypes.c_int, ctypes.c_void_p, ctypes.c_void_p, _c_f, _c_f, ctypes.c_int, ctypes.c_void_p, _c_f,
                                                       ctypes.c_void_p, ctypes.c_size_t, ctypes.c_long, ctypes.c_int, ctypes.c_int, ctypes.c_void_p, ctypes.c_void_p]),
     "matpbr_mlp_first_layer_bwd_blk": (ctypes.c_int, [_c_f, ctypes.c_int, ctypes.c_void_p, ctypes.c_void_p, _c_f, ctypes.c_int, _c_f, ctypes.c_int, _c_f,
diff --git a/materialist_amd/armhead.py b/materialist_amd/armhead.py
--- a/materialist_amd/armhead.py
+++ b/materialist_amd/armhead.py
@@ -50,6 +50,8 @@
     BWD_F16 = True
     FWD_CHAIN = True
     DEFER_REDUCE = True
+    ADAM_IN_FOLD = True
+    HEAD_IN_LOSS_BWD = True
     FWD_PRODUCTS = 3
 
     @staticmethod
@@ -238,10 +240,11 @@
             o.mlp_arm_head_fwd(self.bufs[-1], wo, bo, self.start_arm, self.th, *maps, 256)
         return {k: (self.maps[k] if k in live else self.fixed[k]) for k in self.maps}
 
-    def backward(self) -> None:
+    def backward(self, head_done: bool = False, adam: bool = False) -> bool:
         o, P, live = ops, self.products, self.live
-        o.mlp_arm_head_bwd(self.g["albedo"] if "albedo" in live else None, self.g["roughness"] if "roughness" in live else None,
-                           self.g["metallic"] if "metallic" in live else None, self.th, self.d_x)
+        if not head_done:
+            o.mlp_arm_head_bwd(self.g["albedo"] if "albedo" in live else None, self.g["roughness"] if "roughness" in live else None,
+                               self.g["metallic"] if "metallic" in live else None, self.th, self.d_x)
         wp, _ = self.views[-1]
         gw, gb = self.gviews[-1]
         g_prev = self.gbufs[0]
@@ -279,9 +282,13 @@
                 if l == 1:
                     o.mlp_first_layer_bwd_blk(g, self.tmax[l], self.wsplit_b[l], c_prev, self.x0p, self.gviews[0][0], self.d0, n_prev, n_red, gb, defer=slot(nj))
                     nj += 2
+                    if jobs is not None and adam:
+                        o.mlp_reduce_jobs_adamw(jobs, nj, self.flat, self.gflat, self.adam_m, self.adam_v, self.hyper, self.stats, best=self._best_flat,
+                                                weight_decay=self.weight_decay)
+                        return True
                     if jobs is not None:
                         o.mlp_reduce_jobs(jobs, nj, self.flat)
-                    return
+                    return False
                 g_prev = self.gbufs[0] if g is self.gbufs[1] else self.gbufs[1]
                 o.mlp_layer_bwd_input_blk(g, self.tmax[l], self.wsplit_b[l], c_prev, g_prev, n_prev, n_red, gb, self.tmax[l - 1], defer=slot(nj))
                 nj += 1
@@ -289,12 +296,13 @@
                 continue
             if l == 1 and self.FUSED_FIRST_BWD:
                 o.mlp_first_layer_bwd_bx(g, self.wsplit_b[l], c_prev, self.x0p, self.gviews[0][0], self.d0, n_prev, n_red, gb, P, packed=self.packed)
-                return
+                return False
             g_prev = self.gbufs[0] if g is self.gbufs[1] else self.gbufs[1]
             o.mlp_layer_bwd_input_bx(g, self.wsplit_b[l], c_prev, g_prev, n_prev, n_red, gb, P, packed=self.packed)
             g, n_red = g_prev, n_prev
         gw, _ = self.gviews[0]
         o.mlp_skinny_bwd_weight(self.x0p, g, gw, self.d0, n_red, transposed_out=True)
+        return False
 
     def step(self) -> None:
         o, sc = ops, self.scene
@@ -315,21 +323,22 @@
         o.brdf_loss_stats(self.pred, self.gt, self.gt_srgb, d["albedo"], d["roughness"], d["metallic"], self.orig["albedo"],
                           self.orig["roughness"], self.orig["metallic"], self.scale_delta, self.stats, self.ws, optimize_part=self.part,
                           es_patience=self.patience, es_min_delta=self.min_delta, history=self.hist)
+        head = bool(self.HEAD_IN_LOSS_BWD and self._mask_u8 is None)
         o.brdf_loss_bwd_jac(d["albedo"], d["roughness"], d["metallic"], self.jac, self.pred, self.gt_srgb, self.stats,
                             self.orig["albedo"], self.orig["roughness"], self.orig["metallic"], self.scale_delta,
                             self.g["albedo"], self.g["roughness"], self.g["metallic"], self.best["albedo"], self.best["roughness"],
-                            self.best["metallic"], self.best_img, optimize_part=self.part)
+                            self.best["metallic"], self.best_img, optimize_part=self.part, th=self.th if head else None,
+                            d_x=self.d_x if head else None)
         if self._mask_u8 is not None:
             for k in ("roughness", "metallic"):
                 if k in self.live:
                     o.masked_mean_fill(self.g[k], self._mask_u8, out=self.g[k], gate=self.maps[k])
-        self.backward()
-        lib = _lib.load()
-        with torch.cuda.device(self.dev):
-            _lib.check(lib.matpbr_adamw_step_snapshot_dev(o._ptr(self.flat), o._ptr(self.gflat), o._ptr(self.adam_m), o._ptr(self.adam_v),
-                                                          self.flat.numel(), o._ptr(self.hyper), 0.9, 0.999, 1e-8, self.weight_decay,
-                                                          o._ptr(self._best_flat), o._ptr(self.stats), o._stream(self.flat)),
-                       "matpbr_adamw_step_snapshot_dev")
+        if not self.backward(head_done=head, adam=bool(self.ADAM_IN_FOLD and self.DEFER_REDUCE and self.bwd_f16)):
+            with torch.cuda.device(self.dev):
+                _lib.check(_lib.load().matpbr_adamw_step_snapshot_dev(o._ptr(self.flat), o._ptr(self.gflat), o._ptr(self.adam_m), o._ptr(self.adam_v),
+                                                                      self.flat.numel(), o._ptr(self.hyper), 0.9, 0.999, 1e-8, self.weight_decay,
+                                                                      o._ptr(self._best_flat), o._ptr(self.stats), o._stream(self.flat)),
+                           "matpbr_adamw_step_snapshot_dev")
         if self._lr > 1.5e-4:
             self._sched_epoch += 1
             if self._sched_epoch % 100 == 0:
diff --git a/materialist_amd/build.py b/materialist_amd/build.py
--- a/materialist_amd/build.py
+++ b/materialist_amd/build.py
@@ -8,7 +8,7 @@
 CSRC = os.path.join(_HERE, "csrc")
 LIB_PATH = os.path.join(_HERE, "libmatpbr.so")
 SOURCES = ["matpbr_kernels.hip", "posmlp_kernels.hip", "posmlp_chain.hip", "mesh_host.cpp"]
-HEADERS = [os.path.join("..", "..", "include", "matpbr_experimental.h"), "posmlp_device.hpp", "matpbr_device.hpp", "matpbr_shade.hpp", "matpbr_lazy.hpp", "matpbr_pstep.hpp", os.path.join("..", "..", "include", "matpbr.h"), os.path.join("..", "..", "include", "matpbr_mlp.h")]
+HEADERS = [os.path.join("..", "..", "include", "matpbr_experimental.h"), "posmlp_device.hpp", "matpbr_device.hpp", "matpbr_tail.hpp", "matpbr_shade.hpp", "matpbr_lazy.hpp", "matpbr_pstep.hpp", os.path.join("..", "..", "include", "matpbr.h"), os.path.join("..", "..", "include", "matpbr_mlp.h")]
 HIPCC_FLAGS = ["-O3", "--offload-arch=gfx950", "-std=c++17", "-shared", "-fPIC", "-fno-gpu-rdc", "-Wall", "-Wno-unused-function"]
 
 
diff --git a/materialist_amd/csrc/matpbr_kernels.hip b/materialist_amd/csrc/matpbr_kernels.hip
--- a/materialist_amd/csrc/matpbr_kernels.hip
+++ b/materialist_amd/csrc/matpbr_kernels.hip
@@ -32,14 +32,12 @@
     sg = block_sum(sg, s_buf);
     if (threadIdx.x == 0) { part[((long)b * gridDim.x + blockIdx.x) * 2] = sp; part[((long)b * gridDim.x + blockIdx.x) * 2 + 1] = sg; }
 }
-__global__ __launch_bounds__(kBlock) void loss_final1_kernel(const float* __restrict__ part, float* __restrict__ stats, int nblk) {
-    __shared__ float s_buf[4];
-    const int b = blockIdx.x;
+__device__ __forceinline__ float loss_ratio_fold(const float* __restrict__ part, int b, int nblk, float* s_buf) {
     float sp = 0.0f, sg = 0.0f;
     for (int i = threadIdx.x; i < nblk; i += kBlock) { sp += part[((long)b * nblk + i) * 2]; sg += part[((long)b * nblk + i) * 2 + 1]; }
     sp = block_sum(sp, s_buf);
     sg = block_sum(sg, s_buf);
-    if (threadIdx.x == 0) stats[b * kStatsStride + 0] = sg / sp;
+    return sg / sp;
 }
 __global__ __launch_bounds__(kBlock) void step_state_init_kernel(const float* __restrict__ stats, float* __restrict__ state, int batch) {
     for (int i = threadIdx.x; i < batch * kStateStride; i += kBlock) {
@@ -95,7 +93,7 @@
                                                             const float* __restrict__ fwd_sums, int n_fwd, unsigned part_mask,
                                                             const float* __restrict__ reg_sums = nullptr, const float* __restrict__ pred_alt = nullptr,
                                                             const float* __restrict__ state = nullptr, int n_reg = 0,
-                                                            const long long* __restrict__ walk_fix = nullptr) {
+                                                            const long long* __restrict__ walk_fix = nullptr, float* __restrict__ ratio_out = nullptr) {
     __shared__ float s_buf[4];
     const int b = blockIdx.y;
     float ratio = 1.0f;
@@ -126,7 +124,8 @@
         sp_total = block_sum(sp, s_buf);
         ratio = stats[b * kStatsStride + kStGtSum] / sp_total;
     } else if (MODE == 0) {
-        ratio = stats[b * kStatsStride + kStRatio];
+        ratio = loss_ratio_fold(fwd_sums, b, n_fwd, s_buf);
+        if (blockIdx.x == 0 && threadIdx.x == 0) ratio_out[b * kStatsStride + kStRatio] = ratio;
     }
     float s[5] = {0.0f, 0.0f, 0.0f, 0.0f, 0.0f};
     if (vec4) {
@@ -511,22 +510,10 @@
 __global__ __launch_bounds__(kBlock) void adam_dev_kernel(float* __restrict__ p, const float* __restrict__ g, float* __restrict__ m,
                                                           float* __restrict__ v, long n, float* __restrict__ hyper, float b1, float b2,
                                                           float eps, float wd, float* __restrict__ best, const float* __restrict__ stats) {
-    if (stats != nullptr && stats[kStStopped] > 1.5f) return;
-    const bool snap = best != nullptr && stats[kStImproved] > 0.5f;
-    const float t = stats != nullptr ? fmaxf(stats[kStIters], 1.0f) : hyper[1] + 1.0f, lr = hyper[0];
-    if (stats != nullptr && blockIdx.x == 0 && threadIdx.x == 0) hyper[1] = t;
-    const float keep = 1.0f - lr * wd;
-    const float bc1 = 1.0f - powf(b1, t), bc2 = 1.0f - powf(b2, t);
-    const float lr_over_bc1 = lr / bc1, inv_sqrt_bc2 = 1.0f / sqrtf(bc2);
-    for (long i = (long)blockIdx.x * kBlock + threadIdx.x; i < n; i += (long)gridDim.x * kBlock) {
-        float gi = g[i];
-        float mi = fmaf(b1, m[i], (1.0f - b1) * gi);
-        float vi = fmaf(b2, v[i], (1.0f - b2) * gi * gi);
-        m[i] = mi; v[i] = vi;
-        const float pi = p[i];
-        if (snap) best[i] = pi;
-        p[i] = pi * keep - lr_over_bc1 * mi / fmaf(fsqrt(vi), inv_sqrt_bc2, eps);
-    }
+    AdamDevScalars s;
+    if (!adam_dev_scalars(hyper, b1, b2, wd, best, stats, s)) return;
+    if (stats != nullptr && blockIdx.x == 0 && threadIdx.x == 0) hyper[1] = s.t;
+    for (long i = (long)blockIdx.x * kBlock + threadIdx.x; i < n; i += (long)gridDim.x * kBlock) adam_dev_element(p, m, v, best, i, g[i], b1, b2, eps, s);
 }
 __global__ void adam_dev_tick_kernel(float* __restrict__ hyper, const float* __restrict__ stats) {
     if (stats != nullptr && stats[kStStopped] > 1.5f) return;
@@ -1261,7 +1248,7 @@
     return launch_status();
 }
 
-size_t matpbr_brdf_loss_workspace_bytes(int batch) { return batch > 0 ? (size_t)batch * kRedBlocks * 5 * sizeof(float) : 0; }
+size_t matpbr_brdf_loss_workspace_bytes(int batch) { return batch > 0 ? (size_t)batch * kRedBlocks * 7 * sizeof(float) : 0; }
 
 static unsigned part_mask_of(uint32_t flags) {
     const unsigned all = MATPBR_PART_A | MATPBR_PART_R | MATPBR_PART_M;
@@ -1280,10 +1267,11 @@
     float* part = (float*)workspace;
     hipStream_t st = (hipStream_t)stream;
     dim3 grid(kRedBlocks, (unsigned)batch);
-    hipLaunchKernelGGL(loss_sums1_kernel, grid, dim3(kBlock), 0, st, pred, gt, part, n3);
-    hipLaunchKernelGGL(loss_final1_kernel, dim3((unsigned)batch), dim3(kBlock), 0, st, part, stats, kRedBlocks);
-    hipLaunchKernelGGL(loss_sums2_kernel<0>, grid, dim3(kBlock), 0, st, pred, gt_srgb, stats, pa, a0, pr, r0, pm, m0, part, n3, n1,
-                       (const float*)nullptr, 0, part_mask_of(flags));
+    float* part1 = part + (size_t)batch * kRedBlocks * 5;
+    hipLaunchKernelGGL(loss_sums1_kernel, grid, dim3(kBlock), 0, st, pred, gt, part1, n3);
+    hipLaunchKernelGGL(loss_sums2_kernel<0>, grid, dim3(kBlock), 0, st, pred, gt_srgb, (const float*)nullptr, pa, a0, pr, r0, pm, m0, part, n3, n1,
+                       (const float*)part1, kRedBlocks, part_mask_of(flags), (const float*)nullptr, (const float*)nullptr, (const float*)nullptr, 0,
+                       (const long long*)nullptr, stats);
     hipLaunchKernelGGL(loss_final2_kernel<2>, dim3((unsigned)batch), dim3(kBlock), 0, st, part, stats, kRedBlocks, 1.0f / (float)n3,
                        1.0f / (float)n1, scale_delta, part_mask_of(flags), es_patience, es_min_delta,
                        (const float*)nullptr, 0, history, hist_len, batch);
@@ -1298,12 +1286,14 @@
 }
 
 
-int matpbr_brdf_loss_bwd_jac(const float* pa, const float* pr, const float* pm, const float* jac, const float* pred, const float* gt_srgb,
-                             const float* stats, const float* a0, const float* r0, const float* m0, float scale_delta, float* d_a,
-                             float* d_r, float* d_m, float* best_a, float* best_r, float* best_m, float* best_img, int H, int W, int batch,
-                             uint32_t flags, void* stream) {
+int matpbr_brdf_loss_bwd_jac_head(const float* pa, const float* pr, const float* pm, const float* jac, const float* pred, const float* gt_srgb,
+                                  const float* stats, const float* a0, const float* r0, const float* m0, float scale_delta, float* d_a,
+                                  float* d_r, float* d_m, float* best_a, float* best_r, float* best_m, float* best_img, const float* th, float* d_x,
+                                  int H, int W, int batch, uint32_t flags, void* stream) {
     if (!pa || !pr || !pm || !jac || !pred || !gt_srgb || !stats || !a0 || !r0 || !m0 || !d_a || !d_r || !d_m || H <= 0 || W <= 0 ||
         batch <= 0)
+        return MATPBR_ERR_INVALID_ARG;
+    if ((d_x != nullptr) != (th != nullptr) || (d_x && ((flags & MATPBR_FLAG_JAC16) || ((reinterpret_cast<uintptr_t>(th) | reinterpret_cast<uintptr_t>(d_x)) & 15))))
         return MATPBR_ERR_INVALID_ARG;
     JacBwdArgs q{};
     q.a = pa; q.r = pr; q.m = pm; q.jac = jac; q.d_a = d_a; q.d_r = d_r; q.d_m = d_m;
@@ -1313,12 +1303,21 @@
     q.inv_n3 = 1.0f / (3.0f * (float)H * (float)W);
     q.inv_n1 = 1.0f / ((float)H * (float)W);
     q.part_mask = part_mask_of(flags);
+    q.th = th; q.d_x = d_x;
     const long P = (long)H * W;
     if (flags & MATPBR_FLAG_JAC16)
         hipLaunchKernelGGL((jac_bwd_kernel<true, true>), dim3((unsigned)((P + kBlock - 1) / kBlock), (unsigned)batch), dim3(kBlock), 0, (hipStream_t)stream, q, P);
     else
         hipLaunchKernelGGL((jac_bwd_kernel<true, false>), dim3((unsigned)((P + kBlock - 1) / kBlock), (unsigned)batch), dim3(kBlock), 0, (hipStream_t)stream, q, P);
     return launch_status();
+}
+
+int matpbr_brdf_loss_bwd_jac(const float* pa, const float* pr, const float* pm, const float* jac, const float* pred, const float* gt_srgb,
+                             const float* stats, const float* a0, const float* r0, const float* m0, float scale_delta, float* d_a,
+                             float* d_r, float* d_m, float* best_a, float* best_r, float* best_m, float* best_img, int H, int W, int batch,
+                             uint32_t flags, void* stream) {
+    return matpbr_brdf_loss_bwd_jac_head(pa, pr, pm, jac, pred, gt_srgb, stats, a0, r0, m0, scale_delta, d_a, d_r, d_m, best_a, best_r, best_m, best_img,
+                                         nullptr, nullptr, H, W, batch, flags, stream);
 }
 
 namespace {
diff --git a/materialist_amd/csrc/matpbr_shade.hpp b/materialist_amd/csrc/matpbr_shade.hpp
--- a/materialist_amd/csrc/matpbr_shade.hpp
+++ b/materialist_amd/csrc/matpbr_shade.hpp
@@ -6,6 +6,7 @@
 #include <cstring>
 
 #include "matpbr_device.hpp"
+#include "matpbr_tail.hpp"
 
 namespace matpbr {
 
@@ -373,9 +374,6 @@
     }
 }
 
-constexpr int kStatsStride = 16;
-enum { kStRatio = 0, kStMse, kStL1, kStSr, kStLa, kStLr, kStLm, kStLoss, kStImproved, kStBest, kStEsCounter, kStEsBest, kStEsHas,
-       kStStopped, kStIters, kStGtSum };
 constexpr int kStateStride = 20;
 enum { kStSel = 16, kStBestRatio = 17, kStSelOld = 18  };
 __device__ __forceinline__ bool img_stopped(const float* stats, int b) { return stats[b * kStatsStride + kStStopped] > 0.5f; }
@@ -599,6 +597,8 @@
     unsigned part_mask;
     float lr_over_bc1, b1, b2, eps, inv_sqrt_bc2;
     int check_stop;
+    const float* th;
+    float* d_x;
 };
 constexpr float kLossEps = 1e-8f;
 __device__ __forceinline__ float fsign(float x) { return x > 0.0f ? 1.0f : (x < 0.0f ? -1.0f : 0.0f); }
@@ -674,11 +674,13 @@
         return;
     }
     const bool improved = q.stats[b * kStatsStride + kStImproved] > 0.5f;
+    float gsum_keep[3];
 #pragma unroll
     for (int c = 0; c < 3; ++c) {
         float gsum = da[c] + ((q.part_mask & MATPBR_PART_A) ? q.scale_delta * q.inv_n3 * fsign(a[c] - q.a0[i * 3 + c]) : 0.0f);
         gsum = (ra[c] >= 0.0f && ra[c] <= 1.0f) ? gsum : 0.0f;
         if (q.d_a) q.d_a[i * 3 + c] = gsum;
+        gsum_keep[c] = gsum;
         if (improved && q.best_a) q.best_a[i * 3 + c] = a[c];
         if (improved && q.best_img) q.best_img[i * 3 + c] = xs_keep[c];
         if ((q.part_mask & MATPBR_PART_A) && q.am[0]) q.pa[i * 3 + c] = adam_update(ra[c], gsum, q.am[0], q.av[0], i * 3 + c, q);
@@ -689,6 +691,8 @@
     gm = (rm >= 0.0f && rm <= 1.0f) ? gm : 0.0f;
     if (q.d_r) q.d_r[i] = gr;
     if (q.d_m) q.d_m[i] = gm;
+    if (!J16 && q.d_x) arm_head_bwd_row(q.part_mask & MATPBR_PART_A, gsum_keep[0], gsum_keep[1], gsum_keep[2], q.part_mask & MATPBR_PART_R, gr,
+                                        q.part_mask & MATPBR_PART_M, gm, q.th + i * 8, q.d_x + i * 8);
     if (improved && q.best_r) q.best_r[i] = r;
     if (improved && q.best_m) q.best_m[i] = m;
     if ((q.part_mask & MATPBR_PART_R) && q.am[1]) q.pr[i] = adam_update(rr, gr, q.am[1], q.av[1], i, q);
diff --git a/materialist_amd/csrc/matpbr_tail.hpp b/materialist_amd/csrc/matpbr_tail.hpp
--- /dev/null
+++ b/materialist_amd/csrc/matpbr_tail.hpp
@@ -0,0 +1,55 @@
+#pragma once
+#include <hip/hip_runtime.h>
+
+#include "matpbr_device.hpp"
+
+namespace matpbr {
+
+constexpr int kStatsStride = 16;
+enum { kStRatio = 0, kStMse, kStL1, kStSr, kStLa, kStLr, kStLm, kStLoss, kStImproved, kStBest, kStEsCounter, kStEsBest, kStEsHas,
+       kStStopped, kStIters, kStGtSum };
+
+struct AdamDevScalars {
+    bool snap;
+    float t, lr, keep, lr_over_bc1, inv_sqrt_bc2;
+};
+__device__ __forceinline__ bool adam_dev_scalars(const float* __restrict__ hyper, float b1, float b2, float wd, const float* best,
+                                                 const float* __restrict__ stats, AdamDevScalars& s) {
+    if (stats != nullptr && stats[kStStopped] > 1.5f) return false;
+    s.snap = best != nullptr && stats[kStImproved] > 0.5f;
+    s.t = stats != nullptr ? fmaxf(stats[kStIters], 1.0f) : hyper[1] + 1.0f;
+    s.lr = hyper[0];
+    s.keep = 1.0f - s.lr * wd;
+    const float bc1 = 1.0f - powf(b1, s.t), bc2 = 1.0f - powf(b2, s.t);
+    s.lr_over_bc1 = s.lr / bc1;
+    s.inv_sqrt_bc2 = 1.0f / sqrtf(bc2);
+    return true;
+}
+__device__ __forceinline__ void adam_dev_element(float* __restrict__ p, float* __restrict__ m, float* __restrict__ v, float* __restrict__ best,
+                                                 long i, float gi, float b1, float b2, float eps, const AdamDevScalars& s) {
+    float mi = fmaf(b1, m[i], (1.0f - b1) * gi);
+    float vi = fmaf(b2, v[i], (1.0f - b2) * gi * gi);
+    m[i] = mi; v[i] = vi;
+    const float pi = p[i];
+    if (s.snap) best[i] = pi;
+    p[i] = pi * s.keep - s.lr_over_bc1 * mi / fmaf(fsqrt(vi), s.inv_sqrt_bc2, eps);
+}
+
+__device__ __forceinline__ void arm_head_bwd_row(bool has_a, float ga0, float ga1, float ga2, bool has_r, float gr, bool has_m, float gm,
+                                                 const float* __restrict__ th, float* __restrict__ d_x) {
+    const float4 t0 = *reinterpret_cast<const float4*>(th);
+    const float t4 = th[4];
+    float4 o = make_float4(0.f, 0.f, 0.f, 0.f);
+    float o4 = 0.f;
+    if (has_a) {
+        o.x = (ga0 * 1.3f) * fmaf(-t0.x, t0.x, 1.f);
+        o.y = (ga1 * 1.3f) * fmaf(-t0.y, t0.y, 1.f);
+        o.z = (ga2 * 1.3f) * fmaf(-t0.z, t0.z, 1.f);
+    }
+    if (has_r) o.w = ((gr * 0.93f) * 1.3f) * fmaf(-t0.w, t0.w, 1.f);
+    if (has_m) o4 = (gm * 1.3f) * fmaf(-t4, t4, 1.f);
+    *reinterpret_cast<float4*>(d_x) = o;
+    *reinterpret_cast<float4*>(d_x + 4) = make_float4(o4, 0.f, 0.f, 0.f);
+}
+
+}
diff --git a/materialist_amd/csrc/posmlp_kernels.hip b/materialist_amd/csrc/posmlp_kernels.hip
--- a/materialist_amd/csrc/posmlp_kernels.hip
+++ b/materialist_amd/csrc/posmlp_kernels.hip
@@ -6,6 +6,7 @@
 #include "../../include/matpbr.h"
 #include "../../include/matpbr_experimental.h"
 #include "posmlp_device.hpp"
+#include "matpbr_tail.hpp"
 
 namespace {
 
@@ -722,32 +723,64 @@
       }
 }
 
+struct FoldAdam {
+  float *g, *p, *m, *v, *best;
+  float b1, b2, eps;
+  bool on;
+  matpbr::AdamDevScalars s;
+};
+__device__ __forceinline__ void fold_store(float* dst, float val, const FoldAdam& A) {
+  *dst = val;
+  if (A.on) matpbr::adam_dev_element(A.p, A.m, A.v, A.best, (long)(dst - A.g), val, A.b1, A.b2, A.eps, A.s);
+}
+__device__ __forceinline__ float4 add4(float4 a, float4 b) { return make_float4(a.x + b.x, a.y + b.y, a.z + b.z, a.w + b.w); }
+
+constexpr int kFoldLds = 4096;
+constexpr int kWgradFoldBlocks = 64;
 __device__ __forceinline__ void wgrad_reduce_body(float* red, const float* __restrict__ partial, int slabs, float* __restrict__ dW, int N, int K, int ldw,
-                                                  int block) {
-  const int t = threadIdx.x & 255, sl = threadIdx.x >> 8;
-  const int idx = block * 256 + t;
+                                                  int block, const FoldAdam& A) {
+  const int t = threadIdx.x & 255, sl = __builtin_amdgcn_readfirstlane(threadIdx.x >> 8);
+  const int idx = (block * 256 + t) * 4;
   const int per = (slabs + 3) / 4, c0 = sl * per, c1 = c0 + per < slabs ? c0 + per : slabs;
-  float s0 = 0.f, s1 = 0.f, s2 = 0.f, s3 = 0.f;
+  const unsigned off = (unsigned)idx * 4u;
+  auto slab = [&](int c) { return *reinterpret_cast<const float4*>(reinterpret_cast<const char*>(partial + (size_t)c * 65536) + off); };
+  const float4 z = make_float4(0.f, 0.f, 0.f, 0.f);
+  float4 s0 = z, s1 = z, s2 = z, s3 = z;
   int c = c0;
+  for (; c + 7 < c1; c += 8) {
+    float4 v[8];
+#pragma unroll
+    for (int u = 0; u < 8; ++u) v[u] = slab(c + u);
+    s0 = add4(s0, v[0]); s1 = add4(s1, v[1]); s2 = add4(s2, v[2]); s3 = add4(s3, v[3]);
+    s0 = add4(s0, v[4]); s1 = add4(s1, v[5]); s2 = add4(s2, v[6]); s3 = add4(s3, v[7]);
+  }
   for (; c + 3 < c1; c += 4) {
-    s0 += partial[(long)(c + 0) * 65536 + idx];
-    s1 += partial[(long)(c + 1) * 65536 + idx];
-    s2 += partial[(long)(c + 2) * 65536 + idx];
-    s3 += partial[(long)(c + 3) * 65536 + idx];
-  }
-  for (; c < c1; ++c) s0 += partial[(long)c * 65536 + idx];
-  red[sl * 256 + t] = (s0 + s1) + (s2 + s3);
+    float4 v[4];
+#pragma unroll
+    for (int u = 0; u < 4; ++u) v[u] = slab(c + u);
+    s0 = add4(s0, v[0]); s1 = add4(s1, v[1]); s2 = add4(s2, v[2]); s3 = add4(s3, v[3]);
+  }
+  for (; c < c1; ++c) s0 = add4(s0, slab(c));
+  float4* red4 = reinterpret_cast<float4*>(red);
+  red4[sl * 256 + t] = add4(add4(s0, s1), add4(s2, s3));
   __syncthreads();
+  if (sl != 0) return;
+  const float4 r = add4(add4(red4[t], red4[256 + t]), add4(red4[512 + t], red4[768 + t]));
+  const float rv[4] = {r.x, r.y, r.z, r.w};
   const int n = idx >> 8, k = idx & 255;
-  if (sl == 0 && n < N && k < K) dW[(long)n * ldw + k] = (red[t] + red[256 + t]) + (red[512 + t] + red[768 + t]);
+  if (n >= N) return;
+#pragma unroll
+  for (int e = 0; e < 4; ++e)
+    if (k + e < K) fold_store(dW + (long)n * ldw + k + e, rv[e], A);
 }
 __global__ __launch_bounds__(1024) void mlp_wgrad_reduce(const float* __restrict__ partial, int slabs, float* __restrict__ dW, int N, int K,
                                                          int ldw) {
-  __shared__ float red[1024];
-  wgrad_reduce_body(red, partial, slabs, dW, N, K, ldw, (int)blockIdx.x);
-}
-
-__device__ __forceinline__ void colsum_reduce_body(float* red, const float* __restrict__ part, int groups, float* __restrict__ out, int col) {
+  __shared__ __attribute__((aligned(16))) float red[kFoldLds];
+  wgrad_reduce_body(red, partial, slabs, dW, N, K, ldw, (int)blockIdx.x, FoldAdam{});
+}
+
+__device__ __forceinline__ void colsum_reduce_body(float* red, const float* __restrict__ part, int groups, float* __restrict__ out, int col,
+                                                   const FoldAdam& A) {
   const bool act = threadIdx.x < 256;
   float s = 0.f;
   if (act) {
@@ -760,11 +793,11 @@
     if ((int)threadIdx.x < w) red[threadIdx.x] += red[threadIdx.x + w];
     __syncthreads();
   }
-  if (threadIdx.x == 0) out[col] = red[0];
+  if (threadIdx.x == 0) fold_store(out + col, red[0], A);
 }
 __global__ __launch_bounds__(256) void mlp_colsum_reduce(const float* __restrict__ part, int groups, float* __restrict__ out) {
   __shared__ float red[256];
-  colsum_reduce_body(red, part, groups, out, (int)blockIdx.x);
+  colsum_reduce_body(red, part, groups, out, (int)blockIdx.x, FoldAdam{});
 }
 
 
@@ -2258,21 +2291,9 @@
 
 __global__ __launch_bounds__(256) void arm_head_bwd_kernel(const float* __restrict__ g_a, const float* __restrict__ g_r, const float* __restrict__ g_m,
                                                            const float* __restrict__ th, float* __restrict__ d_x, long M) {
-  for (long m = (long)blockIdx.x * 256 + threadIdx.x; m < M; m += (long)gridDim.x * 256) {
-    const float4 t0 = *reinterpret_cast<const float4*>(th + m * 8);
-    const float t4 = th[m * 8 + 4];
-    float4 o = make_float4(0.f, 0.f, 0.f, 0.f);
-    float o4 = 0.f;
-    if (g_a) {
-      o.x = (g_a[m * 3 + 0] * 1.3f) * (1.f - t0.x * t0.x);
-      o.y = (g_a[m * 3 + 1] * 1.3f) * (1.f - t0.y * t0.y);
-      o.z = (g_a[m * 3 + 2] * 1.3f) * (1.f - t0.z * t0.z);
-    }
-    if (g_r) o.w = ((g_r[m] * 0.93f) * 1.3f) * (1.f - t0.w * t0.w);
-    if (g_m) o4 = (g_m[m] * 1.3f) * (1.f - t4 * t4);
-    *reinterpret_cast<float4*>(d_x + m * 8) = o;
-    *reinterpret_cast<float4*>(d_x + m * 8 + 4) = make_float4(o4, 0.f, 0.f, 0.f);
-  }
+  for (long m = (long)blockIdx.x * 256 + threadIdx.x; m < M; m += (long)gridDim.x * 256)
+    matpbr::arm_head_bwd_row(g_a != nullptr, g_a ? g_a[m * 3 + 0] : 0.f, g_a ? g_a[m * 3 + 1] : 0.f, g_a ? g_a[m * 3 + 2] : 0.f, g_r != nullptr,
+                             g_r ? g_r[m] : 0.f, g_m != nullptr, g_m ? g_m[m] : 0.f, th + m * 8, d_x + m * 8);
 }
 
 constexpr int kSkinnySlabs = 1024;
@@ -2398,7 +2419,7 @@
 
 __device__ __forceinline__ void skinny_reduce_body(float* red_, int block, const float* __restrict__ partial, const float* __restrict__ bpart, int slabs, int J, int Jv,
                                                              int C, float* __restrict__ out, long ld_j, long ld_c, float* __restrict__ d_b,
-                                                             const float* __restrict__ gsum_part, int C2, float* __restrict__ d_b2) {
+                                                             const float* __restrict__ gsum_part, int C2, float* __restrict__ d_b2, const FoldAdam& A) {
   float (*red)[64] = reinterpret_cast<float (*)[64]>(red_);
   int j = block >> 2;
   const int cl = threadIdx.x & 63, c = (block & 3) * 64 + cl, sl = threadIdx.x >> 6;
@@ -2421,7 +2442,7 @@
     float t = 0.f;
 #pragma unroll
     for (int u = 0; u < 16; ++u) t += red[u][cl];
-    out[j * ld_j + c * ld_c] = t;
+    fold_store(out + (j * ld_j + c * ld_c), t, A);
   }
   if (d_b != nullptr && bpart != nullptr && (block & 3) == 0) {
     __syncthreads();
@@ -2439,7 +2460,7 @@
     if (threadIdx.x == 0) {
       float u = 0.f;
       for (int r = 0; r < 64; ++r) u += red[0][r];
-      d_b[j] = u;
+      fold_store(d_b + j, u, A);
     }
   }
 }
@@ -2447,7 +2468,7 @@
                                                              int C, float* __restrict__ out, long ld_j, long ld_c, float* __restrict__ d_b,
                                                              const float* __restrict__ gsum_part, int C2, float* __restrict__ d_b2) {
   __shared__ float red[1024];
-  skinny_reduce_body(red, (int)blockIdx.x, partial, bpart, slabs, J, Jv, C, out, ld_j, ld_c, d_b, gsum_part, C2, d_b2);
+  skinny_reduce_body(red, (int)blockIdx.x, partial, bpart, slabs, J, Jv, C, out, ld_j, ld_c, d_b, gsum_part, C2, d_b2, FoldAdam{});
 }
 
 constexpr int kMaxReduceJobs = 16;
@@ -2456,23 +2477,34 @@
   int first[kMaxReduceJobs + 1];
   int n;
 };
-__global__ __launch_bounds__(1024) void mlp_reduce_jobs_kernel(const ReduceJobs js) {
-  __shared__ float red[1024];
+struct FoldAdamArgs {
+  float *g, *p, *m, *v, *hyper, *best;
+  const float* stats;
+  float b1, b2, eps, wd;
+};
+__global__ __launch_bounds__(1024, 8) void mlp_reduce_jobs_kernel(const ReduceJobs js, const FoldAdamArgs a) {
+  __shared__ __attribute__((aligned(16))) float red[kFoldLds];
+  FoldAdam A{};
+  if (a.g != nullptr) {
+    A.g = a.g; A.p = a.p; A.m = a.m; A.v = a.v; A.best = a.best; A.b1 = a.b1; A.b2 = a.b2; A.eps = a.eps;
+    A.on = matpbr::adam_dev_scalars(a.hyper, a.b1, a.b2, a.wd, a.best, a.stats, A.s);
+    if (A.on && blockIdx.x == 0 && threadIdx.x == 0) a.hyper[1] = A.s.t;
+  }
   int k = 0;
   while (k + 1 < js.n && (int)blockIdx.x >= js.first[k + 1]) ++k;
   const MatpbrReduceJob& q = js.j[k];
   const int block = (int)blockIdx.x - js.first[k];
-  if (q.kind == MATPBR_REDUCE_WGRAD) wgrad_reduce_body(red, q.src, q.groups, q.dst, q.n0, q.n1, q.n2, block);
-  else if (q.kind == MATPBR_REDUCE_COLSUM) colsum_reduce_body(red, q.src, q.groups, q.dst, block);
-  else skinny_reduce_body(red, block, q.src, q.src_b, q.groups, q.n0, q.n1, q.n2, q.dst, q.ld_j, q.ld_c, q.dst_b, q.src_g, q.n3, q.dst_g);
+  if (q.kind == MATPBR_REDUCE_WGRAD) wgrad_reduce_body(red, q.src, q.groups, q.dst, q.n0, q.n1, q.n2, block, A);
+  else if (q.kind == MATPBR_REDUCE_COLSUM) colsum_reduce_body(red, q.src, q.groups, q.dst, block, A);
+  else skinny_reduce_body(red, block, q.src, q.src_b, q.groups, q.n0, q.n1, q.n2, q.dst, q.ld_j, q.ld_c, q.dst_b, q.src_g, q.n3, q.dst_g, A);
 }
 inline int reduce_job_blocks(const MatpbrReduceJob& q) {
-  if (q.kind == MATPBR_REDUCE_WGRAD) return 256;
+  if (q.kind == MATPBR_REDUCE_WGRAD) return kWgradFoldBlocks;
   if (q.kind == MATPBR_REDUCE_COLSUM) return q.n0;
   return q.n0 * 4 + (q.dst_g ? 4 : 0);
 }
 inline void launch_reduce_job(const MatpbrReduceJob& q, hipStream_t st) {
-  if (q.kind == MATPBR_REDUCE_WGRAD) hipLaunchKernelGGL(mlp_wgrad_reduce, dim3(256), dim3(1024), 0, st, q.src, q.groups, q.dst, q.n0, q.n1, q.n2);
+  if (q.kind == MATPBR_REDUCE_WGRAD) hipLaunchKernelGGL(mlp_wgrad_reduce, dim3(kWgradFoldBlocks), dim3(1024), 0, st, q.src, q.groups, q.dst, q.n0, q.n1, q.n2);
   else if (q.kind == MATPBR_REDUCE_COLSUM) hipLaunchKernelGGL(mlp_colsum_reduce, dim3(q.n0), dim3(256), 0, st, q.src, q.groups, q.dst);
   else hipLaunchKernelGGL(mlp_skinny_tn_reduce, dim3(reduce_job_blocks(q)), dim3(1024), 0, st, q.src, q.src_b, q.groups, q.n0, q.n1, q.n2, q.dst, q.ld_j, q.ld_c,
                           q.dst_b, q.src_g, q.n3, q.dst_g);
@@ -2805,12 +2837,12 @@
     hipLaunchKernelGGL(mlp_small_tn, dim3((unsigned)tiles), dim3(256), 0, (hipStream_t)stream, g, ldg, x, ldx, d_w, ldw, (int)M, N, K);
     return hipGetLastError() == hipSuccess ? MATPBR_OK : MATPBR_ERR_LAUNCH;
   }
-  if (!workspace || workspace_bytes < matpbr_mlp_bwd_weight_workspace_bytes(M)) return MATPBR_ERR_WORKSPACE;
+  if (!workspace || !aligned16(workspace) || workspace_bytes < matpbr_mlp_bwd_weight_workspace_bytes(M)) return MATPBR_ERR_WORKSPACE;
   const int slabs = wgrad_slabs(M);
   long rows = (M + slabs - 1) / slabs;
   rows = (rows + kWM - 1) / kWM * kWM;
   hipLaunchKernelGGL(mlp_wgrad_tn, dim3(slabs, (N + 127) / 128), dim3(256), 0, (hipStream_t)stream, g, ldg, x, ldx, (float*)workspace, M, rows, K);
-  hipLaunchKernelGGL(mlp_wgrad_reduce, dim3(256), dim3(1024), 0, (hipStream_t)stream, (const float*)workspace, slabs, d_w, N, K, ldw);
+  hipLaunchKernelGGL(mlp_wgrad_reduce, dim3(kWgradFoldBlocks), dim3(1024), 0, (hipStream_t)stream, (const float*)workspace, slabs, d_w, N, K, ldw);
   return hipGetLastError() == hipSuccess ? MATPBR_OK : MATPBR_ERR_LAUNCH;
 }
 
@@ -2821,7 +2853,7 @@
   if (nprod == 3 && (!g_tile_max || (M % kBM))) return MATPBR_ERR_INVALID_ARG;
   if ((nprod != 3 && nprod != 6 && nprod != 9) || (M & 15) || ldg < 256 || ldx < 256 || (ldg & 3) || (ldx & 3) || ldw < K || !aligned16(g) || !aligned16(x))
     return MATPBR_ERR_UNSUPPORTED;
-  if (!workspace || workspace_bytes < matpbr_mlp_bwd_weight_workspace_bytes(M)) return MATPBR_ERR_WORKSPACE;
+  if (!workspace || !aligned16(workspace) || workspace_bytes < matpbr_mlp_bwd_weight_workspace_bytes(M)) return MATPBR_ERR_WORKSPACE;
   int slabs = wgrad_slabs(M);
   long rows = ((M + slabs - 1) / slabs + 15) / 16 * 16;
   slabs = (int)((M + rows - 1) / rows);
@@ -2940,24 +2972,49 @@
                                 n_prev, (unsigned*)g_tile_max, stream, defer);
 }
 
-int matpbr_mlp_reduce_jobs(const MatpbrReduceJob* jobs, int n_jobs, void* stream) {
+static bool fold_dst_inside(const float* dst, long last, const float* g, long n) { return dst >= g && last >= 0 && dst + last < g + n; }
+
+static int mlp_reduce_jobs_impl(const MatpbrReduceJob* jobs, int n_jobs, const FoldAdamArgs& a, long n, void* stream) {
   if (!jobs || n_jobs <= 0 || n_jobs > kMaxReduceJobs) return MATPBR_ERR_INVALID_ARG;
   ReduceJobs js{};
   int blocks = 0;
-  for (int i = 0; i < n_jobs; ++i) {
-    const MatpbrReduceJob& q = jobs[i];
-    if (q.kind == MATPBR_REDUCE_NONE) continue;
-    if ((q.kind != MATPBR_REDUCE_WGRAD && q.kind != MATPBR_REDUCE_COLSUM && q.kind != MATPBR_REDUCE_SKINNY) || !q.src || !q.dst || q.groups <= 0 || q.n0 <= 0)
-      return MATPBR_ERR_INVALID_ARG;
-    js.j[js.n] = q;
-    js.first[js.n] = blocks;
-    blocks += reduce_job_blocks(q);
-    ++js.n;
-  }
-  if (js.n == 0) return MATPBR_OK;
+  for (int pass = 0; pass < 2; ++pass)
+    for (int i = 0; i < n_jobs; ++i) {
+      const MatpbrReduceJob& q = jobs[i];
+      if (q.kind == MATPBR_REDUCE_NONE || (q.kind == MATPBR_REDUCE_WGRAD) != (pass == 0)) continue;
+      if ((q.kind != MATPBR_REDUCE_WGRAD && q.kind != MATPBR_REDUCE_COLSUM && q.kind != MATPBR_REDUCE_SKINNY) || !q.src || !q.dst || q.groups <= 0 || q.n0 <= 0)
+        return MATPBR_ERR_INVALID_ARG;
+      if (q.kind == MATPBR_REDUCE_WGRAD && !aligned16(q.src)) return MATPBR_ERR_INVALID_ARG;
+      if (a.g) {
+        bool in = true;
+        if (q.kind == MATPBR_REDUCE_WGRAD) in = q.n1 > 0 && fold_dst_inside(q.dst, (long)(q.n0 - 1) * q.n2 + q.n1 - 1, a.g, n);
+        else if (q.kind == MATPBR_REDUCE_COLSUM) in = fold_dst_inside(q.dst, q.n0 - 1, a.g, n);
+        else {
+          in = q.n1 > 0 && q.n2 > 0 && q.ld_j >= 0 && q.ld_c >= 0 && fold_dst_inside(q.dst, (q.n1 - 1) * q.ld_j + (q.n2 - 1) * q.ld_c, a.g, n);
+          if (q.dst_b) in = in && fold_dst_inside(q.dst_b, q.n1 - 1, a.g, n);
+          if (q.dst_g) in = in && q.n3 > 0 && fold_dst_inside(q.dst_g, q.n3 - 1, a.g, n);
+        }
+        if (!in) return MATPBR_ERR_INVALID_ARG;
+      }
+      js.j[js.n] = q;
+      js.first[js.n] = blocks;
+      blocks += reduce_job_blocks(q);
+      ++js.n;
+    }
+  if (js.n == 0 && !a.g) return MATPBR_OK;
+  if (js.n == 0) return MATPBR_ERR_INVALID_ARG;
   js.first[js.n] = blocks;
-  hipLaunchKernelGGL(mlp_reduce_jobs_kernel, dim3((unsigned)blocks), dim3(1024), 0, (hipStream_t)stream, js);
+  hipLaunchKernelGGL(mlp_reduce_jobs_kernel, dim3((unsigned)blocks), dim3(1024), 0, (hipStream_t)stream, js, a);
   return hipGetLastError() == hipSuccess ? MATPBR_OK : MATPBR_ERR_LAUNCH;
 }
 
-}
+int matpbr_mlp_reduce_jobs(const MatpbrReduceJob* jobs, int n_jobs, void* stream) { return mlp_reduce_jobs_impl(jobs, n_jobs, FoldAdamArgs{}, 0, stream); }
+
+int matpbr_mlp_reduce_jobs_adamw(const MatpbrReduceJob* jobs, int n_jobs, float* p, float* g, float* m, float* v, long n, float* hyper, float beta1,
+                                 float beta2, float eps, float weight_decay, float* best, const float* stats, void* stream) {
+  if (!p || !g || !m || !v || !hyper || !stats || n <= 0) return MATPBR_ERR_INVALID_ARG;
+  const FoldAdamArgs a{g, p, m, v, hyper, best, stats, beta1, beta2, eps, weight_decay};
+  return mlp_reduce_jobs_impl(jobs, n_jobs, a, n, stream);
+}
+
+}
diff --git a/materialist_amd/ops.py b/materialist_amd/ops.py
--- a/materialist_amd/ops.py
+++ b/materialist_amd/ops.py
@@ -484,14 +484,21 @@
 
 
 def brdf_loss_bwd_jac(pa, pr, pm, jac, pred, gt_srgb, stats, a0, r0, m0, scale_delta: float, d_a, d_r, d_m,
-                      best_a=None, best_r=None, best_m=None, best_img=None, optimize_part: str = "arm", jac16: bool = False) -> None:
+                      best_a=None, best_r=None, best_m=None, best_img=None, optimize_part: str = "arm", jac16: bool = False,
+                      th: Optional[torch.Tensor] = None, d_x: Optional[torch.Tensor] = None) -> None:
     lib = _lib.load()
     pa = _dev(pa, "pa", (3,))
     B, H, W = _bhw(pa)
+    flags = part_mask(optimize_part) | (FLAG_JAC16 if jac16 else 0)
     with torch.cuda.device(pa.device), _timed("shade_bwd"):
-        code = lib.matpbr_brdf_loss_bwd_jac(_ptr(pa), _ptr(pr), _ptr(pm), _ptr(jac), _ptr(pred), _ptr(gt_srgb), _ptr(stats), _ptr(a0), _ptr(r0),
-                                            _ptr(m0), float(scale_delta), _ptr(d_a), _ptr(d_r), _ptr(d_m), _ptr(best_a), _ptr(best_r),
-                                            _ptr(best_m), _ptr(best_img), H, W, B, part_mask(optimize_part) | (FLAG_JAC16 if jac16 else 0), _stream(pa))
+        if th is not None or d_x is not None:
+            code = lib.matpbr_brdf_loss_bwd_jac_head(_ptr(pa), _ptr(pr), _ptr(pm), _ptr(jac), _ptr(pred), _ptr(gt_srgb), _ptr(stats), _ptr(a0), _ptr(r0),
+                                                     _ptr(m0), float(scale_delta), _ptr(d_a), _ptr(d_r), _ptr(d_m), _ptr(best_a), _ptr(best_r),
+                                                     _ptr(best_m), _ptr(best_img), _ptr(th), _ptr(d_x), H, W, B, flags, _stream(pa))
+        else:
+            code = lib.matpbr_brdf_loss_bwd_jac(_ptr(pa), _ptr(pr), _ptr(pm), _ptr(jac), _ptr(pred), _ptr(gt_srgb), _ptr(stats), _ptr(a0), _ptr(r0),
+                                                _ptr(m0), float(scale_delta), _ptr(d_a), _ptr(d_r), _ptr(d_m), _ptr(best_a), _ptr(best_r),
+                                                _ptr(best_m), _ptr(best_img), H, W, B, flags, _stream(pa))
     _lib.check(code, "matpbr_brdf_loss_bwd_jac")
 
 
@@ -837,6 +844,14 @@
     return int(_lib.load().matpbr_mlp_set_wgrad_kernel(int(kernel)))
 
 
+def mlp_reduce_jobs_adamw(jobs, n: int, p: torch.Tensor, g: torch.Tensor, m: torch.Tensor, v: torch.Tensor, hyper: torch.Tensor, stats: torch.Tensor,
+                          best: Optional[torch.Tensor] = None, beta1: float = 0.9, beta2: float = 0.999, eps: float = 1e-8, weight_decay: float = 0.01) -> None:
+    with torch.cuda.device(p.device):
+        code = _lib.load().matpbr_mlp_reduce_jobs_adamw(ctypes.byref(jobs), int(n), _ptr(p), _ptr(g), _ptr(m), _ptr(v), p.numel(), _ptr(hyper), float(beta1),
+                                                        float(beta2), float(eps), float(weight_decay), _ptr(best), _ptr(stats), _stream(p))
+    _lib.check(code, "matpbr_mlp_reduce_jobs_adamw")
+
+
 def mlp_reduce_jobs(jobs, n: int, like: torch.Tensor) -> None:
     with torch.cuda.device(like.device):
         code = _lib.load().matpbr_mlp_reduce_jobs(ctypes.byref(jobs), int(n), _stream(like))
```
